# charlesknipp/sequential_monte_carlo

Hardware: AMD Instinct MI355X
Metric: particle-steps/sec (higher is better)
Workload: dtype f64; 1 GPU; LinearGaussian1D bootstrap filter Nx=2^20 T=1000 (BASELINE configs[1]); n_theta_per_gpu=1, n_x=1048576, T=1000, seg=2048, resident_kernel=False, resampler=multinomial

## Files before the change

### include/smc_hip.h

```cpp
#ifndef SMC_HIP_H
#define SMC_HIP_H
#include <stdint.h>

#ifdef __cplusplus
extern "C" {
#endif

#define SMC_MODEL_LG1D 1
#define SMC_MODEL_SV1D 2
#define SMC_MODEL_UCSV3D 3
#define SMC_MODEL_UCSV_RB 4

#define SMC_OK 0
#define SMC_EINVAL (-1)
#define SMC_EHIP (-2)
#define SMC_ESTATE (-3)
#define SMC_ENOMEM (-4)

#define SMC_FLAG_ANCESTORS 1u
#define SMC_FLAG_NO_RESIDENT 2u
#define SMC_FLAG_SYSTEMATIC 4u

typedef struct smc_filter_s* smc_handle;

int smc_create(int model_id, int64_t n_theta, int64_t n_x, int seg, uint64_t seed, int device, uint32_t flags,
               smc_handle* out);
int smc_destroy(smc_handle h);

int smc_set_params(smc_handle h, const double* raw );
int smc_set_streams(smc_handle h, const uint32_t* stream );
int smc_reseed(smc_handle h, uint64_t seed);

#define SMC_PROP_NONE 0
#define SMC_PROP_AFFINE 1
#define SMC_PROP_OPTIMAL 2
#define SMC_PROP_NPAR 4
int smc_set_proposal(smc_handle h, int kind, const double* par );
int smc_host_optimal_proposal(int model_id, const double* raw, double* par );
int smc_host_guided_step(int model_id, const double* raw, int kind, const double* par, const double* xp ,
                         const double* z , double y, double* x , double* logw);
int smc_device_guided_step(int model_id, const double* raw, int kind, const double* par, const double* xp,
                           const double* z, double y, int64_t n, double* x, double* logw, int device);

int smc_host_rb_step(const double* raw , const double* sp , const double* z , double y, int first,
                     double* s , double* logw);
int smc_device_rb_step(const double* raw, const double* sp, const double* z, double y, int first, int64_t n, double* s,
                       double* logw, int device);

int smc_init(smc_handle h, double y1, double* logmu );
int smc_step(smc_handle h, double y_t, double* logmu , double* ess );
int smc_step_window(smc_handle h, const double* y , int k, double* logmu , double* ess );
int smc_step_commit(smc_handle h, int j);
int smc_log_likelihood(smc_handle h, const double* y, int64_t T, double* logZ ,
                       double* logmu_trace, double* ess_trace);
int smc_set_summaries(smc_handle h, int component, const double* p , int np, int moments);
int smc_get_summaries(smc_handle h, int64_t T, double* q , double* mean , double* var );
#define SMC_SUMM_WEIGHTED 0
#define SMC_SUMM_UNWEIGHTED 1
int smc_set_summary_mode(smc_handle h, int mode);
int smc_get_state(smc_handle h, double* x , double* w ,
                  int32_t* anc );
int smc_get_logZ(smc_handle h, double* logZ , double* ess );
int smc_permute(smc_handle h, const int32_t* a );
int smc_copy_from(smc_handle dst, smc_handle src, const uint8_t* mask );

int smc_set_skip(smc_handle h, const uint8_t* skip );

#define SMC_PRIOR_UNIFORM 1
#define SMC_PRIOR_NORMAL 2
#define SMC_PRIOR_TRUNCNORMAL 3
#define SMC_PRIOR_LOGNORMAL 4
#define SMC_PRIOR_NPAR 5
#define SMC_MAX_DTHETA 8
int smc_pmmh_configure(smc_handle prop, int d_theta, const int32_t* prior_family ,
                       const double* prior_par , const int32_t* raw_from ,
                       const double* raw_const );
int smc_pmmh_rejuvenate(smc_handle prop, smc_handle main , const double* y, int64_t T, double xi,
                        const double* chol , const double* scales , int chain,
                        const uint64_t* filter_seeds , uint64_t move_seed, double* theta ,
                        double* logZ , uint8_t* accepted , int64_t* filters_run );
#define SMC_OUTER_SEG 8
int smc_outer_seg(void);
int smc_host_reweight(const double* logw, int64_t n, double* w, double* logmu, double* ess);
int smc_host_outer_records(const double* logw_local, int64_t n_local, uint64_t* rec);
int smc_host_outer_combine(const uint64_t* rec, int64_t nseg, int64_t n_total, double* logmu, double* ess);
int smc_host_outer_window(const double* logw_local, const double* lik , int k, int64_t n_local, uint64_t* rec);
int smc_host_outer_walk(const uint64_t* rec, int k, int64_t nseg, int64_t n_total, double ess_min, double* ess_out , int* j_out);
int smc_host_outer_advance(double* logw, double* logZ, const double* lik , int j, int64_t n);
int smc_host_outer_temper(const double* logZ, int64_t n, double xi, double ess_min, double* xi_new, double* ess, int* resample_flag,
                          double* logw_out);
int smc_host_outer_resample(const double* logw, int64_t n, int64_t m, uint64_t seed, int32_t* a );
int smc_host_rw_factor(const double* theta, int64_t n, int d, double* L , int* univariate);
int smc_host_rw_factor_cov(const double* cov , int d, double* L , int* univariate);
int smc_host_pmmh_propose(int d_theta, uint64_t move_seed, uint32_t stream, uint32_t c, const double* theta,
                          const double* chol, double scale, double* prop);
double smc_host_pmmh_log_uniform(uint64_t move_seed, uint32_t stream, uint32_t c);
double smc_host_prior_logpdf(int family, const double* par , double x);

int smc_slot_bytes(smc_handle h, int64_t* bytes);
int smc_pack_slots(smc_handle h, const int32_t* idx, int64_t k, void* device_buf);
int smc_unpack_slots(smc_handle h, const int32_t* idx, int64_t k, const void* device_buf);

#define SMC_COMM_ID_BYTES 128
typedef struct smc_comm_s* smc_comm;
int smc_comm_unique_id(void* id );
int smc_comm_create(const void* id, int rank, int world, int device, smc_comm* out);
int smc_comm_destroy(smc_comm c);
int smc_comm_rank(smc_comm c, int* rank, int* world);
int smc_comm_all_gather(smc_comm c, const double* local , int64_t n, double* all );
int smc_outer_reweight(smc_comm c, const double* logw_local , int64_t n_local, double* logw_all ,
                       double* w_all , double* logmu, double* ess);
int smc_comm_exchange_slots(smc_comm c, smc_handle h, const int32_t* a , int64_t M);
int smc_comm_plan_exchange(const int32_t* a , int64_t M, int rank, int world, int32_t* send_idx, int64_t* send_cnt ,
                           int64_t* n_send, int32_t* dest_idx, int64_t* recv_cnt );

int smc_get_weights_raw(smc_handle h, uint64_t* C, double* m, uint64_t* S, uint64_t* S2hi, uint64_t* S2lo);
int smc_get_geometry(smc_handle h, int* seg, int* nseg, int* d, int* resident);
int smc_last_elapsed_ms(smc_handle h, double* ms);
int smc_synchronize(smc_handle h);
int smc_time_step_kernel(smc_handle h, const double* y, int64_t T, int nsample, double* avg_ms, double* min_ms);
int smc_event_overhead_ms(smc_handle h, int nsample, double* avg_ms);

int smc_normalize(const double* logw, int64_t n, double* w, double* logmu, double* ess, int device);
int smc_resample(const double* w, int64_t n, int64_t ndraw, uint64_t seed, uint32_t stream, uint32_t t, int32_t* a,
                 int device);

int smc_kalman_log_likelihood(const double* raw, int64_t n_theta, const double* y, int64_t T, int predict_first,
                              double* out , int device);
int smc_ibis_create(int64_t n_theta, uint64_t seed, int device, int predict_first, void* out);
int smc_ibis_destroy(void* h);
int smc_ibis_configure(void* h, int d_theta, const int32_t* prior_family , const double* prior_par ,
                       const int32_t* raw_from , const double* raw_const );
int smc_ibis_set_theta(void* h, const double* theta );
int smc_ibis_window(void* h, const double* y , int k, double* lik , uint64_t* rec );
int smc_ibis_commit(void* h, int j);
int smc_ibis_filter(void* h, const double* y, int64_t T);
int smc_ibis_permute(void* h, const int32_t* a );
int smc_ibis_set_logw(void* h, const double* logw );
int smc_ibis_rejuvenate(void* h, const double* y, int64_t T, double xi, const double* chol ,
                        const double* scales , int chain, uint64_t move_seed, int64_t* accepted ,
                        uint8_t* moved );
int smc_ibis_get(void* h, double* theta, double* x, double* S, double* logZ, double* logw);
int smc_ibis_summary(void* h, int ahead, double* out );
int smc_ibis_set_summaries(void* h, int on, int ahead);
int smc_ibis_get_summaries(void* h, int j, double* out );
int smc_host_ibis_summary(const double* rows, const double* x, const double* S, const double* logw, int64_t M, int ahead, double* out );
int smc_ibis_window_ess(void* h, const double* y , int k, double ess_min, double* ess_out , int* j_out);
int smc_ibis_resample(void* h, uint64_t seed, int32_t* a_out );
int smc_ibis_theta_moments(void* h, int weighted, double* mean , double* cov );
int smc_host_theta_moments(const double* theta, const double* logw, int64_t M, int d, int weighted, double* mean, double* cov);
int smc_ibis_get_moved(void* h, uint8_t* moved );
int smc_get_moments(smc_handle h, double* mean, double* var);

int smc_get_quantiles(smc_handle h, int component, const double* p, int np, double* out);

int smc_simulate(int model_id, const double* raw, int64_t T, uint64_t seed, double* x , double* y );
int smc_simulate_dim(int model_id);
int smc_model_dim(int model_id);
int smc_model_nraw(int model_id);
int smc_auto_seg(int model_id, int64_t n_x);
int smc_device_count(void);
int smc_host_quantile7(const double* x, int64_t n, const double* p, int np, double* out);
int smc_host_sample_moments(const double* x, int64_t n, double* mean, double* var);
double smc_host_exp(double x);
double smc_host_log(double x);
void smc_host_philox4x32_10(const uint32_t ctr[4], const uint32_t key[2], uint32_t out[4]);
void smc_host_box_muller(const uint32_t w[4], double* z0, double* z1);
int smc_sys_targets(uint64_t Dtot, uint32_t n, uint64_t u, uint64_t j0, int nk, uint64_t* out, int device);
int smc_device_math(int which , const double* a, const double* b,
                    int64_t n, double* out, int device);

const char* smc_last_error(void);
const char* smc_version(void);

#ifdef __cplusplus
}
#endif
#endif
```

### sequential_monte_carlo_amd/_lib.py

```python
import ctypes as C
import os

import numpy as np

_HERE = os.path.dirname(os.path.abspath(__file__))
LIB_PATH = os.environ.get("SMC_LIB") or os.path.join(_HERE, "lib", "libsmchip.so")

MODEL_LG1D, MODEL_SV1D, MODEL_UCSV3D, MODEL_UCSV_RB = 1, 2, 3, 4
FLAG_ANCESTORS, FLAG_NO_RESIDENT, FLAG_SYSTEMATIC = 1, 2, 4

EXPORTS = [
    "smc_create", "smc_destroy", "smc_set_params", "smc_set_streams", "smc_reseed", "smc_init", "smc_step",
    "smc_log_likelihood", "smc_get_state", "smc_get_logZ", "smc_permute", "smc_copy_from", "smc_slot_bytes", "smc_pack_slots", "smc_unpack_slots", "smc_get_weights_raw", "smc_get_geometry",
    "smc_last_elapsed_ms", "smc_synchronize", "smc_time_step_kernel", "smc_event_overhead_ms", "smc_normalize", "smc_resample", "smc_kalman_log_likelihood", "smc_get_moments", "smc_get_quantiles", "smc_simulate", "smc_simulate_dim", "smc_model_dim",
    "smc_model_nraw", "smc_auto_seg", "smc_device_count", "smc_host_exp", "smc_host_log", "smc_host_philox4x32_10",
    "smc_host_box_muller", "smc_sys_targets", "smc_device_math", "smc_last_error", "smc_version",
    "smc_set_skip", "smc_pmmh_configure", "smc_pmmh_rejuvenate", "smc_host_pmmh_propose", "smc_host_pmmh_log_uniform",
    "smc_host_prior_logpdf", "smc_step_window", "smc_step_commit",
    "smc_comm_unique_id", "smc_comm_create", "smc_comm_destroy", "smc_comm_rank", "smc_comm_all_gather", "smc_outer_reweight",
    "smc_comm_exchange_slots", "smc_host_reweight", "smc_comm_plan_exchange",
    "smc_outer_seg", "smc_host_outer_records", "smc_host_outer_combine", "smc_host_outer_window", "smc_host_outer_walk",
    "smc_host_outer_advance", "smc_host_outer_temper", "smc_host_outer_resample", "smc_host_rw_factor",
    "smc_set_summaries", "smc_get_summaries", "smc_set_summary_mode", "smc_host_quantile7", "smc_host_sample_moments",
    "smc_set_proposal", "smc_host_optimal_proposal", "smc_host_guided_step", "smc_device_guided_step",
    "smc_host_rb_step", "smc_device_rb_step",
    "smc_ibis_create", "smc_ibis_destroy", "smc_ibis_configure", "smc_ibis_set_theta", "smc_ibis_window", "smc_ibis_commit",
    "smc_ibis_filter", "smc_ibis_permute", "smc_ibis_set_logw", "smc_ibis_rejuvenate", "smc_ibis_get",
    "smc_ibis_summary", "smc_ibis_set_summaries", "smc_ibis_get_summaries", "smc_host_ibis_summary",
    "smc_ibis_window_ess", "smc_ibis_resample", "smc_ibis_theta_moments", "smc_ibis_get_moved", "smc_host_theta_moments",
    "smc_host_rw_factor_cov",
]
PROP_NONE, PROP_AFFINE, PROP_OPTIMAL, PROP_NPAR = 0, 1, 2, 4
SUMM_WEIGHTED, SUMM_UNWEIGHTED = 0, 1
_SUMM_MODES = {"weighted": SUMM_WEIGHTED, "unweighted": SUMM_UNWEIGHTED}
COMM_ID_BYTES = 128
PRIOR_UNIFORM, PRIOR_NORMAL, PRIOR_TRUNCNORMAL, PRIOR_LOGNORMAL, PRIOR_NPAR, MAX_DTHETA = 1, 2, 3, 4, 5, 8

_dp = C.POINTER(C.c_double)
_u64p = C.POINTER(C.c_uint64)
_u32p = C.POINTER(C.c_uint32)
_i32p = C.POINTER(C.c_int32)
_ip = C.POINTER(C.c_int)


class SmcError(RuntimeError):
    pass


_lib = None


def _share_hip_runtime_with_torch():
    if os.environ.get("SMC_HIP_RUNTIME", "") == "system":
        return
    try:
        import importlib.util
        spec = importlib.util.find_spec("torch")
        if spec is None or not spec.submodule_search_locations:
            return
        cand = os.path.join(list(spec.submodule_search_locations)[0], "lib", "libamdhip64.so")
        if os.path.exists(cand):
            C.CDLL(cand, mode=C.RTLD_GLOBAL)
    except Exception:
        pass


def lib():
    global _lib
    if _lib is not None:
        return _lib
    if not os.path.exists(LIB_PATH):
        raise SmcError("HIP extension %s not built: run `python -c 'import __graft_entry__ as g; g.build()'` "
                       "(hipcc --offload-arch=gfx950). There is no CPU fallback." % LIB_PATH)
    _share_hip_runtime_with_torch()
    L = C.CDLL(LIB_PATH)
    h = C.c_void_p
    L.smc_create.argtypes = [C.c_int, C.c_int64, C.c_int64, C.c_int, C.c_uint64, C.c_int, C.c_uint32, C.POINTER(h)]
    L.smc_destroy.argtypes = [h]
    L.smc_set_params.argtypes = [h, _dp]
    L.smc_set_streams.argtypes = [h, _u32p]
    L.smc_reseed.argtypes = [h, C.c_uint64]
    L.smc_init.argtypes = [h, C.c_double, _dp]
    L.smc_step.argtypes = [h, C.c_double, _dp, _dp]
    L.smc_log_likelihood.argtypes = [h, _dp, C.c_int64, _dp, _dp, _dp]
    L.smc_get_state.argtypes = [h, _dp, _dp, _i32p]
    L.smc_get_logZ.argtypes = [h, _dp, _dp]
    L.smc_permute.argtypes = [h, _i32p]
    L.smc_copy_from.argtypes = [h, h, C.POINTER(C.c_uint8)]
    L.smc_slot_bytes.argtypes = [h, C.POINTER(C.c_int64)]
    L.smc_pack_slots.argtypes = [h, _i32p, C.c_int64, C.c_void_p]
    L.smc_unpack_slots.argtypes = [h, _i32p, C.c_int64, C.c_void_p]
    L.smc_get_weights_raw.argtypes = [h, _u64p, _dp, _u64p, _u64p, _u64p]
    L.smc_get_geometry.argtypes = [h, _ip, _ip, _ip, _ip]
    L.smc_last_elapsed_ms.argtypes = [h, _dp]
    L.smc_synchronize.argtypes = [h]
    L.smc_time_step_kernel.argtypes = [h, _dp, C.c_int64, C.c_int, _dp, _dp]
    L.smc_event_overhead_ms.argtypes = [h, C.c_int, _dp]
    L.smc_normalize.argtypes = [_dp, C.c_int64, _dp, _dp, _dp, C.c_int]
    L.smc_resample.argtypes = [_dp, C.c_int64, C.c_int64, C.c_uint64, C.c_uint32, C.c_uint32, _i32p, C.c_int]
    L.smc_kalman_log_likelihood.argtypes = [_dp, C.c_int64, _dp, C.c_int64, C.c_int, _dp, C.c_int]
    L.smc_get_moments.argtypes = [h, _dp, _dp]
    L.smc_get_quantiles.argtypes = [h, C.c_int, _dp, C.c_int, _dp]
    L.smc_set_summaries.argtypes = [h, C.c_int, _dp, C.c_int, C.c_int]
    L.smc_set_summary_mode.argtypes = [h, C.c_int]
    L.smc_host_quantile7.argtypes = [_dp, C.c_int64, _dp, C.c_int, _dp]
    L.smc_host_sample_moments.argtypes = [_dp, C.c_int64, _dp, _dp]
    L.smc_set_proposal.argtypes = [h, C.c_int, _dp]
    L.smc_host_optimal_proposal.argtypes = [C.c_int, _dp, _dp]
    L.smc_host_guided_step.argtypes = [C.c_int, _dp, C.c_int, _dp, _dp, _dp, C.c_double, _dp, _dp]
    L.smc_device_guided_step.argtypes = [C.c_int, _dp, C.c_int, _dp, _dp, _dp, C.c_double, C.c_int64, _dp, _dp, C.c_int]
    L.smc_host_rb_step.argtypes = [_dp, _dp, _dp, C.c_double, C.c_int, _dp, _dp]
    L.smc_device_rb_step.argtypes = [_dp, _dp, _dp, C.c_double, C.c_int, C.c_int64, _dp, _dp, C.c_int]
    L.smc_get_summaries.argtypes = [h, C.c_int64, _dp, _dp, _dp]
    L.smc_sys_targets.argtypes = [C.c_uint64, C.c_uint32, C.c_uint64, C.c_uint64, C.c_int, C.POINTER(C.c_uint64), C.c_int]
    L.smc_simulate.argtypes = [C.c_int, _dp, C.c_int64, C.c_uint64, _dp, _dp]
    L.smc_model_dim.argtypes = [C.c_int]
    L.smc_simulate_dim.argtypes = [C.c_int]
    L.smc_model_nraw.argtypes = [C.c_int]
    L.smc_auto_seg.argtypes = [C.c_int, C.c_int64]
    L.smc_host_exp.restype = C.c_double
    L.smc_host_exp.argtypes = [C.c_double]
    L.smc_host_log.restype = C.c_double
    L.smc_host_log.argtypes = [C.c_double]
    L.smc_host_philox4x32_10.restype = None
    L.smc_host_philox4x32_10.argtypes = [_u32p, _u32p, _u32p]
    L.smc_host_box_muller.restype = None
    L.smc_host_box_muller.argtypes = [_u32p, _dp, _dp]
    L.smc_device_math.argtypes = [C.c_int, _dp, _dp, C.c_int64, _dp, C.c_int]
    L.smc_step_window.argtypes = [h, _dp, C.c_int, _dp, _dp]
    L.smc_step_commit.argtypes = [h, C.c_int]
    L.smc_set_skip.argtypes = [h, C.POINTER(C.c_uint8)]
    L.smc_pmmh_configure.argtypes = [h, C.c_int, _i32p, _dp, _i32p, _dp]
    L.smc_pmmh_rejuvenate.argtypes = [h, h, _dp, C.c_int64, C.c_double, _dp, _dp, C.c_int, _u64p, C.c_uint64, _dp, _dp,
                                      C.POINTER(C.c_uint8), C.POINTER(C.c_int64)]
    L.smc_host_pmmh_propose.argtypes = [C.c_int, C.c_uint64, C.c_uint32, C.c_uint32, _dp, _dp, C.c_double, _dp]
    L.smc_host_pmmh_log_uniform.restype = C.c_double
    L.smc_host_pmmh_log_uniform.argtypes = [C.c_uint64, C.c_uint32, C.c_uint32]
    L.smc_host_prior_logpdf.restype = C.c_double
    L.smc_host_prior_logpdf.argtypes = [C.c_int, _dp, C.c_double]
    L.smc_host_reweight.argtypes = [_dp, C.c_int64, _dp, _dp, _dp]
    L.smc_host_outer_records.argtypes = [_dp, C.c_int64, _u64p]
    L.smc_host_outer_combine.argtypes = [_u64p, C.c_int64, C.c_int64, _dp, _dp]
    L.smc_host_outer_window.argtypes = [_dp, _dp, C.c_int, C.c_int64, _u64p]
    L.smc_host_outer_walk.argtypes = [_u64p, C.c_int, C.c_int64, C.c_int64, C.c_double, _dp, _ip]
    L.smc_host_outer_advance.argtypes = [_dp, _dp, _dp, C.c_int, C.c_int64]
    L.smc_host_outer_temper.argtypes = [_dp, C.c_int64, C.c_double, C.c_double, _dp, _dp, _ip, _dp]
    L.smc_host_outer_resample.argtypes = [_dp, C.c_int64, C.c_int64, C.c_uint64, _i32p]
    L.smc_host_rw_factor.argtypes = [_dp, C.c_int64, C.c_int, _dp, _ip]
    L.smc_comm_unique_id.argtypes = [C.c_void_p]
    L.smc_comm_create.argtypes = [C.c_void_p, C.c_int, C.c_int, C.c_int, C.POINTER(h)]
    L.smc_comm_destroy.argtypes = [h]
    L.smc_comm_rank.argtypes = [h, _ip, _ip]
    L.smc_comm_all_gather.argtypes = [h, _dp, C.c_int64, _dp]
    L.smc_outer_reweight.argtypes = [h, _dp, C.c_int64, _dp, _dp, _dp, _dp]
    L.smc_comm_exchange_slots.argtypes = [h, h, _i32p, C.c_int64]
    L.smc_comm_plan_exchange.argtypes = [_i32p, C.c_int64, C.c_int, C.c_int, _i32p, C.POINTER(C.c_int64), C.POINTER(C.c_int64), _i32p,
                                         C.POINTER(C.c_int64)]
    L.smc_ibis_create.argtypes = [C.c_int64, C.c_uint64, C.c_int, C.c_int, C.POINTER(h)]
    L.smc_ibis_destroy.argtypes = [h]
    L.smc_ibis_configure.argtypes = [h, C.c_int, _i32p, _dp, _i32p, _dp]
    L.smc_ibis_set_theta.argtypes = [h, _dp]
    L.smc_ibis_window.argtypes = [h, _dp, C.c_int, _dp, _u64p]
    L.smc_ibis_commit.argtypes = [h, C.c_int]
    L.smc_ibis_filter.argtypes = [h, _dp, C.c_int64]
    L.smc_ibis_permute.argtypes = [h, _i32p]
    L.smc_ibis_set_logw.argtypes = [h, _dp]
    L.smc_ibis_rejuvenate.argtypes = [h, _dp, C.c_int64, C.c_double, _dp, _dp, C.c_int, C.c_uint64, C.POINTER(C.c_int64),
                                      C.POINTER(C.c_uint8)]
    L.smc_ibis_get.argtypes = [h, _dp, _dp, _dp, _dp, _dp]
    L.smc_ibis_summary.argtypes = [h, C.c_int, _dp]
    L.smc_ibis_set_summaries.argtypes = [h, C.c_int, C.c_int]
    L.smc_ibis_get_summaries.argtypes = [h, C.c_int, _dp]
    L.smc_host_ibis_summary.argtypes = [_dp, _dp, _dp, _dp, C.c_int64, C.c_int, _dp]
    L.smc_ibis_window_ess.argtypes = [h, _dp, C.c_int, C.c_double, _dp, _ip]
    L.smc_ibis_resample.argtypes = [h, C.c_uint64, _i32p]
    L.smc_ibis_theta_moments.argtypes = [h, C.c_int, _dp, _dp]
    L.smc_ibis_get_moved.argtypes = [h, C.POINTER(C.c_uint8)]
    L.smc_host_theta_moments.argtypes = [_dp, _dp, C.c_int64, C.c_int, C.c_int, _dp, _dp]
    L.smc_host_rw_factor_cov.argtypes = [_dp, C.c_int, _dp, _ip]
    L.smc_last_error.restype = C.c_char_p
    L.smc_version.restype = C.c_char_p
    _lib = L
    return L


def check(rc):
    if rc != 0:
        raise SmcError("libsmchip error %d: %s" % (rc, lib().smc_last_error().decode()))


def _d(a):
    return a.ctypes.data_as(_dp) if a is not None else None


def device_count():
    return lib().smc_device_count()


def sys_targets(Dtot, n, u, j0, nk, device=-1):
    out = np.zeros(nk, dtype=np.uint64)
    check(lib().smc_sys_targets(int(Dtot), int(n), int(u), int(j0), int(nk), out.ctypes.data_as(C.POINTER(C.c_uint64)), device))
    return out


def simulate(model_id, raw, T, seed):
    raw = np.ascontiguousarray(raw, dtype=np.float64)
    d = lib().smc_simulate_dim(model_id)
    x = np.zeros((d, T))
    y = np.zeros(T)
    check(lib().smc_simulate(model_id, _d(raw), T, seed, _d(x), _d(y)))
    return x, y


def normalize(logw, device=0):
    logw = np.ascontiguousarray(logw, dtype=np.float64)
    w = np.zeros_like(logw)
    lm, ess = C.c_double(), C.c_double()
    check(lib().smc_normalize(_d(logw), logw.size, _d(w), C.byref(lm), C.byref(ess), device))
    return lm.value, w, ess.value


def resample(w, ndraw=None, seed=0, stream=0, t=0, device=0):
    w = np.ascontiguousarray(w, dtype=np.float64)
    ndraw = w.size if ndraw is None else int(ndraw)
    a = np.zeros(ndraw, dtype=np.int32)
    check(lib().smc_resample(_d(w), w.size, ndraw, seed, stream, t, a.ctypes.data_as(_i32p), device))
    return a


def kalman_log_likelihood(raw, y, predict_first=False, device=0):
    raw = np.ascontiguousarray(raw, dtype=np.float64).reshape(-1, 6)
    y = np.ascontiguousarray(y, dtype=np.float64)
    out = np.zeros((raw.shape[0], 3))
    check(lib().smc_kalman_log_likelihood(_d(raw), raw.shape[0], _d(y), y.size, int(predict_first), _d(out), device))
# ... 124 lines not shown
    k, nseg = rec.shape[0], rec.shape[1]
    ess = np.zeros(k)
    j = C.c_int()
    check(lib().smc_host_outer_walk(rec.ctypes.data_as(_u64p), k, nseg, int(n_total), float(ess_min), _d(ess), C.byref(j)))
    return ess[:j.value], j.value


def host_outer_advance(logw, logZ, lik, j):
    lik = np.ascontiguousarray(lik, dtype=np.float64)
    logw = np.array(logw, dtype=np.float64, order="C")
    logZ = np.array(logZ, dtype=np.float64, order="C")
    assert lik.shape[1] == logw.size == logZ.size and 0 <= j <= lik.shape[0]
    check(lib().smc_host_outer_advance(_d(logw), _d(logZ), _d(lik), int(j), logw.size))
    return logw, logZ


def host_outer_temper(logZ, xi, ess_min):
    logZ = np.ascontiguousarray(logZ, dtype=np.float64)
    lw = np.empty_like(logZ)
    nx, e, flag = C.c_double(), C.c_double(), C.c_int()
    check(lib().smc_host_outer_temper(_d(logZ), logZ.size, float(xi), float(ess_min), C.byref(nx), C.byref(e), C.byref(flag), _d(lw)))
    return nx.value, e.value, bool(flag.value), lw


def host_outer_resample(logw, m, seed):
    logw = np.ascontiguousarray(logw, dtype=np.float64)
    a = np.empty(int(m), dtype=np.int32)
    check(lib().smc_host_outer_resample(_d(logw), logw.size, int(m), int(seed), a.ctypes.data_as(_i32p)))
    return a


def host_rw_factor(theta):
    theta = np.ascontiguousarray(theta, dtype=np.float64)
    n, d = theta.shape
    L = np.zeros((d, d))
    uni = C.c_int()
    check(lib().smc_host_rw_factor(_d(theta), n, d, _d(L), C.byref(uni)))
    return L, bool(uni.value)


def host_rw_factor_cov(cov):
    cov = np.ascontiguousarray(cov, dtype=np.float64)
    d = cov.shape[0]
    assert cov.shape == (d, d)
    L = np.zeros((d, d))
    uni = C.c_int()
    check(lib().smc_host_rw_factor_cov(_d(cov), d, _d(L), C.byref(uni)))
    return L, bool(uni.value)


def host_theta_moments(theta, logw=None, weighted=False):
    theta = np.ascontiguousarray(theta, dtype=np.float64)
    M, d = theta.shape
    if weighted:
        logw = np.ascontiguousarray(logw, dtype=np.float64)
        assert logw.size == M
    mean, cov = np.zeros(d), np.zeros((d, d))
    check(lib().smc_host_theta_moments(_d(theta), _d(logw) if weighted else None, M, d, int(bool(weighted)), _d(mean), _d(cov)))
    return mean, cov


def comm_unique_id():
    buf = C.create_string_buffer(COMM_ID_BYTES)
    check(lib().smc_comm_unique_id(buf))
    return buf.raw


class Comm:

    def __init__(self, unique_id, rank, world, device=0):
        self._c = C.c_void_p()
        self.rank, self.world = int(rank), int(world)
        check(lib().smc_comm_create(C.c_char_p(bytes(unique_id)), self.rank, self.world, int(device), C.byref(self._c)))

    def close(self):
        if getattr(self, "_c", None):
            lib().smc_comm_destroy(self._c)
            self._c = None

    def slice(self, M):
        if M % self.world:
            raise ValueError("n_theta (%d) must be a multiple of the number of ranks (%d)" % (M, self.world))
        per = M // self.world
        return self.rank * per, (self.rank + 1) * per

    def all_gather(self, local):
        local = np.ascontiguousarray(local, dtype=np.float64).ravel()
        out = np.zeros(local.size * self.world)
        check(lib().smc_comm_all_gather(self._c, _d(local), local.size, _d(out)))
        return out

    def outer_reweight(self, logw_local, want_w=True):
        lw = np.ascontiguousarray(logw_local, dtype=np.float64).ravel()
        allw, w = (np.zeros(lw.size * self.world), np.zeros(lw.size * self.world)) if want_w else (None, None)
        lm, ess = C.c_double(), C.c_double()
        check(lib().smc_outer_reweight(self._c, _d(lw), lw.size, _d(allw), _d(w), C.byref(lm), C.byref(ess)))
        return lm.value, w, ess.value, allw

    def exchange_slots(self, h, a, M):
        a = np.ascontiguousarray(a, dtype=np.int32)
        check(lib().smc_comm_exchange_slots(self._c, h._h, a.ctypes.data_as(_i32p), int(M)))


class Handle:

    def __init__(self, model_id, n_theta, n_x, seg=0, seed=1, device=0, flags=0):
        self._h = C.c_void_p()
        self.summary_mode = "weighted"
        self.model_id, self.n_theta, self.n_x = model_id, int(n_theta), int(n_x)
        check(lib().smc_create(model_id, self.n_theta, self.n_x, seg, seed, device, flags, C.byref(self._h)))
        seg_, nseg, d, res = C.c_int(), C.c_int(), C.c_int(), C.c_int()
        check(lib().smc_get_geometry(self._h, C.byref(seg_), C.byref(nseg), C.byref(d), C.byref(res)))
        self.seg, self.nseg, self.d, self.resident = seg_.value, nseg.value, d.value, bool(res.value)
        self.flags = flags

    def close(self):
        if getattr(self, "_h", None):
            lib().smc_destroy(self._h)
            self._h = None

    def __del__(self):
        try:
            self.close()
        except Exception:
            pass

    def set_params(self, raw):
        raw = np.ascontiguousarray(raw, dtype=np.float64).reshape(self.n_theta, -1)
        assert raw.shape[1] == lib().smc_model_nraw(self.model_id)
        check(lib().smc_set_params(self._h, _d(raw)))

    def set_proposal(self, kind, par=None):
        if par is not None:
            par = np.ascontiguousarray(par, dtype=np.float64)
            if par.size == PROP_NPAR and self.n_theta > 1:
                par = np.tile(par.reshape(1, PROP_NPAR), (self.n_theta, 1))
            if par.size != self.n_theta * PROP_NPAR:
                raise ValueError("proposal rows must be [n_theta][4]")
            par = np.ascontiguousarray(par)
        check(lib().smc_set_proposal(self._h, int(kind), _d(par)))
        self.proposal_kind = int(kind)

    def set_streams(self, streams):
        s = np.ascontiguousarray(streams, dtype=np.uint32)
        assert s.size == self.n_theta
        if getattr(self, "_streams_set", None) is not None and np.array_equal(self._streams_set, s):
            return
        check(lib().smc_set_streams(self._h, s.ctypes.data_as(_u32p)))
        self._streams_set = s.copy()

    def reseed(self, seed):
        check(lib().smc_reseed(self._h, seed))

    def init(self, y1):
        lm = np.zeros(self.n_theta)
        check(lib().smc_init(self._h, float(y1), _d(lm)))
        return lm

    def step(self, y):
        lm = np.zeros(self.n_theta)
        ess = np.zeros(self.n_theta)
        check(lib().smc_step(self._h, float(y), _d(lm), _d(ess)))
        return lm, ess

    def step_window(self, y):
        y = np.ascontiguousarray(y, dtype=np.float64)
        lm = np.zeros((y.size, self.n_theta))
        ess = np.zeros((y.size, self.n_theta))
        check(lib().smc_step_window(self._h, _d(y), y.size, _d(lm), _d(ess)))
        return lm, ess

    def step_commit(self, j):
        check(lib().smc_step_commit(self._h, int(j)))

    @property
    def can_window(self):
        return self.nseg == 1 and self.resident

    def log_likelihood(self, y, trace=False):
        y = np.ascontiguousarray(y, dtype=np.float64)
        logZ = np.zeros(self.n_theta)
        if trace:
            lm = np.zeros((y.size, self.n_theta))
            es = np.zeros((y.size, self.n_theta))
            check(lib().smc_log_likelihood(self._h, _d(y), y.size, _d(logZ), _d(lm), _d(es)))
            return logZ, lm, es
        check(lib().smc_log_likelihood(self._h, _d(y), y.size, _d(logZ), None, None))
        return logZ

    def state(self, want_w=True, want_anc=None):
        x = np.zeros((self.d, self.n_theta, self.n_x))
        w = np.zeros((self.n_theta, self.n_x)) if want_w else None
        if want_anc is None:
            want_anc = bool(self.flags & FLAG_ANCESTORS)
        a = np.zeros((self.n_theta, self.n_x), dtype=np.int32) if want_anc else None
        check(lib().smc_get_state(self._h, _d(x), _d(w), a.ctypes.data_as(_i32p) if a is not None else None))
        return x, w, a

    def logZ(self):
        z = np.zeros(self.n_theta)
        e = np.zeros(self.n_theta)
        check(lib().smc_get_logZ(self._h, _d(z), _d(e)))
        return z, e

    def permute(self, a):
        a = np.ascontiguousarray(a, dtype=np.int32)
        assert a.size == self.n_theta
        check(lib().smc_permute(self._h, a.ctypes.data_as(_i32p)))

    def set_summary_mode(self, mode):
        if mode not in _SUMM_MODES:
            raise ValueError("summary mode must be 'weighted' or 'unweighted'")
        check(lib().smc_set_summary_mode(self._h, _SUMM_MODES[mode]))
        self.summary_mode = mode

    def moments(self):
        m = np.zeros((self.d, self.n_theta))
        v = np.zeros((self.d, self.n_theta))
        check(lib().smc_get_moments(self._h, _d(m), _d(v)))
        return m, v

    def quantiles(self, p, component=0):
        p = np.ascontiguousarray(p, dtype=np.float64).ravel()
        out = np.zeros((self.n_theta, p.size))
        check(lib().smc_get_quantiles(self._h, int(component), _d(p), p.size, _d(out)))
        return out

    def set_summaries(self, p=None, component=0, moments=False):
        p = np.ascontiguousarray([] if p is None else p, dtype=np.float64).ravel()
        check(lib().smc_set_summaries(self._h, int(component), _d(p) if p.size else None, p.size, int(bool(moments))))
        self._sum_np, self._sum_mom = int(p.size), bool(moments)

    def get_summaries(self, T):
        nq, mom = getattr(self, "_sum_np", 0), getattr(self, "_sum_mom", False)
        q = np.zeros((T, self.n_theta, nq)) if nq else None
        mean = np.zeros((T, self.d, self.n_theta)) if mom else None
        var = np.zeros((T, self.d, self.n_theta)) if mom else None
        check(lib().smc_get_summaries(self._h, int(T), _d(q), _d(mean), _d(var)))
        return q, mean, var

    def copy_from(self, src, mask):
        m = np.ascontiguousarray(mask, dtype=np.uint8)
        assert m.size == self.n_theta
        check(lib().smc_copy_from(self._h, src._h, m.ctypes.data_as(C.POINTER(C.c_uint8))))

    def set_skip(self, skip):
        if skip is None:
            check(lib().smc_set_skip(self._h, None))
            return
        m = np.ascontiguousarray(skip, dtype=np.uint8)
        assert m.size == self.n_theta
        check(lib().smc_set_skip(self._h, m.ctypes.data_as(C.POINTER(C.c_uint8))))

    def pmmh_configure(self, families, pars, raw_from, raw_const):
        fam = np.ascontiguousarray(families, dtype=np.int32)
        par = np.ascontiguousarray(pars, dtype=np.float64).reshape(fam.size, PRIOR_NPAR)
        rf = np.ascontiguousarray(raw_from, dtype=np.int32)
        rc = np.ascontiguousarray(raw_const, dtype=np.float64)
        assert rf.size == rc.size == lib().smc_model_nraw(self.model_id)
        check(lib().smc_pmmh_configure(self._h, fam.size, fam.ctypes.data_as(_i32p), _d(par), rf.ctypes.data_as(_i32p), _d(rc)))
        self._pmmh_d = int(fam.size)

    def pmmh_rejuvenate(self, main, y, xi, chol, scales, filter_seeds, move_seed, theta, logZ):
        y = np.ascontiguousarray(y, dtype=np.float64)
        d = self._pmmh_d
        theta = np.array(theta, dtype=np.float64, order="C").reshape(self.n_theta, d)
        logZ = np.array(logZ, dtype=np.float64, order="C").reshape(self.n_theta)
        chol = np.ascontiguousarray(chol, dtype=np.float64).reshape(d, d)
        scales = np.ascontiguousarray(scales, dtype=np.float64)
        seeds = np.ascontiguousarray(filter_seeds, dtype=np.uint64)
        assert seeds.size == scales.size
        acc = np.zeros(self.n_theta, dtype=np.uint8)
        nrun = C.c_int64()
        check(lib().smc_pmmh_rejuvenate(self._h, main._h if main is not None else None, _d(y), y.size, float(xi), _d(chol),
                                        _d(scales), scales.size, seeds.ctypes.data_as(_u64p), int(move_seed), _d(theta), _d(logZ),
                                        acc.ctypes.data_as(C.POINTER(C.c_uint8)), C.byref(nrun)))
        return theta, logZ, acc.astype(bool), int(nrun.value)

    def slot_bytes(self):
        b = C.c_int64()
        check(lib().smc_slot_bytes(self._h, C.byref(b)))
        return b.value

    def pack_slots(self, idx, device_ptr):
        idx = np.ascontiguousarray(idx, dtype=np.int32)
        check(lib().smc_pack_slots(self._h, idx.ctypes.data_as(_i32p), idx.size, C.c_void_p(int(device_ptr))))

    def unpack_slots(self, idx, device_ptr):
        idx = np.ascontiguousarray(idx, dtype=np.int32)
        check(lib().smc_unpack_slots(self._h, idx.ctypes.data_as(_i32p), idx.size, C.c_void_p(int(device_ptr))))

    def weights_raw(self):
        npad = self.nseg * self.seg
        Cc = np.zeros((self.n_theta, npad), dtype=np.uint64)
        m = np.zeros((self.n_theta, self.nseg))
        S = np.zeros((self.n_theta, self.nseg), dtype=np.uint64)
        hi = np.zeros_like(S)
        lo = np.zeros_like(S)
        check(lib().smc_get_weights_raw(self._h, Cc.ctypes.data_as(_u64p), _d(m), S.ctypes.data_as(_u64p),
                                        hi.ctypes.data_as(_u64p), lo.ctypes.data_as(_u64p)))
        return Cc, m, S, hi, lo

    def elapsed_ms(self):
        ms = C.c_double()
        check(lib().smc_last_elapsed_ms(self._h, C.byref(ms)))
        return ms.value
# ... 133 lines not shown
```

### sequential_monte_carlo_amd/csrc/smc_capi.hip

```cpp
#include "smc_host.h"
#include "smc_aux_kernels.h"

#include <atomic>
#include <chrono>
#include <cstdlib>
#include <cstring>
#include <mutex>
#include <string>
#include <vector>
#ifdef SMC_ABLATE
#include <algorithm>
#include <cstdio>
#include <map>
#endif

using namespace smc;

static thread_local std::string g_err;
#ifdef SMC_ABLATE
static int h_abl_tmp = 0;
static void abl_report(smc_filter_s* h);
#endif
int fail(int code, const std::string& msg) {
    g_err = msg;
    return code;
}

namespace smc {
bool geo_valid(int seg, int np, Geo& g) {
    if (np != 1 && np != 2 && np != 4) return false;
    const int th = seg / (2 * np);
    if (th * 2 * np != seg) return false;
    if (!(th == 128 || th == 256 || th == 512 || th == 1024 || (th == 64 && np == 2))) return false;
    g = {th, np};
    return true;
}
bool geo_default(int seg, Geo& g) {
    switch (seg) {
    case 256: g = {128, 1}; return true;
    case 512: g = {256, 1}; return true;
    case 1024: g = {512, 1}; return true;
    case 2048: g = {512, 2}; return true;
    case 4096: g = {1024, 2}; return true;
    case 8192: g = {1024, 4}; return true;
    }
    return false;
}
}

constexpr int MAX_NSEG = 16384;
extern "C" int smc_auto_seg(int model_id, int64_t n) {
    const int dm = model_dim_rt(model_id);
    const bool d3 = dm >= 3;
    if (n > (int64_t)MAX_NSEG * 4096) return 8192;
    if (n > (int64_t)MAX_NSEG * 2048) return 4096;
    if (n > (int64_t)MAX_NSEG * 1024) return 2048;
    if (n > ((int64_t)1 << 19)) return d3 ? 1024 : 2048;
    if (n > ((int64_t)1 << 17)) return 1024;
    if (n > ((int64_t)1 << 15)) return 512;
    if (n > (dm > 3 ? 2048 : d3 ? 4096 : MAX_SEG)) return 256;
    int s = 256;
    while (s < n) s <<= 1;
    return s;
}
extern "C" int smc_model_dim(int id) { return model_dim_rt(id); }
extern "C" int smc_model_nraw(int id) { return model_nraw_rt(id); }
extern "C" const char* smc_last_error(void) { return g_err.c_str(); }
extern "C" const char* smc_version(void) { return "smchip 0.1 (gfx950)"; }
extern "C" int smc_device_count(void) {
    int n = 0;
    if (hipGetDeviceCount(&n) != hipSuccess) return 0;
    return n;
}

hipError_t do_init(smc_filter_s* h, double y) {
    return by_model(h->model, [&](auto M) { return launch_init<decltype(M)::value>(h->v, h->geo, h->cur, y, h->stream); });
}
static hipError_t do_table(smc_filter_s* h, int emit, int first_emit, uint32_t t_emit) {
    constexpr int TH = 1024;
    hipLaunchKernelGGL((k_table<TH>), dim3(h->v.ntheta), dim3(TH), 0, h->stream, h->v, h->cur, emit, first_emit, t_emit);
    return hipGetLastError();
}
hipError_t do_step(smc_filter_s* h, uint32_t t, int emit_prev, double y) {
    if (h->v.tabD) {
        hipError_t e = do_table(h, emit_prev, t == 1u ? 1 : 0, t - 1u);
        if (e != hipSuccess) return e;
        emit_prev = 0;
    }
    if (h->v.prop_kind)
        return by_guided_model(h->model, [&](auto M) { return launch_step_g<decltype(M)::value>(h->v, h->geo, h->cur, t, emit_prev, y, h->stream); });
    return by_model(h->model, [&](auto M) { return launch_step<decltype(M)::value>(h->v, h->geo, h->cur, t, emit_prev, y, h->stream); });
}
hipError_t ensure_breaks(smc_filter_s* h, uint32_t t, uint32_t t_end) {
    FilterView& v = h->v;
    if (v.nseg <= 1 || v.systematic) return hipSuccess;
    if (h->brk_count && t >= v.brk_t0 && t < v.brk_t0 + h->brk_count) return hipSuccess;
    const size_t per_step = (size_t)v.ntheta * ((size_t)v.nseg + 1);
    if (!h->d_brk) {
        size_t steps = ((size_t)32 << 20) / (per_step * 8);
        steps = steps < 1 ? 1 : (steps > 1024 ? 1024 : steps);
        hipError_t e = hipMalloc((void**)&h->d_brk, steps * per_step * 8);
        if (e != hipSuccess) return e;
        h->brk_cap = (uint32_t)steps;
        v.brk = h->d_brk;
    }
    uint32_t cnt = t_end > t ? t_end - t : 1;
    cnt = cnt > h->brk_cap ? h->brk_cap : cnt;
    constexpr int TH = 256;
    const size_t lds = ((size_t)v.nseg + 1 + TH / WAVE) * 8;
    static bool raised[16] = {};
    hipError_t e = raise_lds_limit(k_breaks<TH>, lds, raised);
    if (e != hipSuccess) return e;
    hipLaunchKernelGGL((k_breaks<TH>), dim3(cnt, v.ntheta), dim3(TH), lds, h->stream, v, t, h->d_brk);
    v.brk_t0 = t;
    h->brk_count = cnt;
    return hipGetLastError();
}
static hipError_t do_window(smc_filter_s* h, int k, int bout) {
    if (h->v.prop_kind)
        return by_guided_model(h->model, [&](auto M) {
            return launch_window_g<decltype(M)::value>(h->v, k, h->d_recs, (int)h->t, h->cur, bout, h->win.h_out, h->stream);
        });
    return by_model(h->model, [&](auto M) {
        return launch_window<decltype(M)::value>(h->v, k, h->d_recs, (int)h->t, h->cur, bout, h->win.h_out, h->stream);
    });
}

hipError_t do_finalize(smc_filter_s* h, int first_emit, uint32_t t_emit) {
    if (h->v.tabD) return do_table(h, 1, first_emit, t_emit);
    constexpr int TH = 256;
    const size_t lds = table_lds_bytes(h->v.nseg_p2, TH, 1);
    hipLaunchKernelGGL((k_finalize<TH>), dim3(h->v.ntheta), dim3(TH), lds, h->stream, h->v, h->cur, first_emit, t_emit);
    return hipGetLastError();
}

namespace {
struct Bundle {
    int device = -1;
    char* slab = nullptr; size_t slab_bytes = 0;
    double* pin = nullptr; size_t pin_bytes = 0;
    hipStream_t stream = nullptr;
    hipEvent_t ev0 = nullptr, ev1 = nullptr;
    double* d_y = nullptr; int64_t ycap = 0;
    void* d_recs = nullptr; size_t rec_bytes = 0;
    void* h_params = nullptr; size_t params_bytes = 0;
};
struct BundleCache {
    std::mutex mu;
    std::vector<Bundle> free_list;
    size_t bytes = 0;
    static constexpr size_t MAX_BYTES = (size_t)512 << 20, MAX_COUNT = 8;
    bool take(int device, size_t slab_bytes, size_t pin_bytes, Bundle& out) {
        std::lock_guard<std::mutex> g(mu);
        for (size_t i = 0; i < free_list.size(); ++i) {
            const Bundle& b = free_list[i];
            if (b.device == device && b.slab_bytes >= slab_bytes && b.slab_bytes <= 2 * slab_bytes + 4096 && b.pin_bytes >= pin_bytes) {
                out = b;
                bytes -= b.slab_bytes;
                free_list.erase(free_list.begin() + (long)i);
                return true;
            }
        }
        return false;
    }
    bool give(const Bundle& b) {
        std::lock_guard<std::mutex> g(mu);
        if (free_list.size() >= MAX_COUNT || bytes + b.slab_bytes > MAX_BYTES) return false;
        free_list.push_back(b);
        bytes += b.slab_bytes;
        return true;
    }
};
BundleCache& bundle_cache() { static BundleCache* c = new BundleCache(); return *c; }
}

extern "C" int smc_create(int model_id, int64_t n_theta, int64_t n_x, int seg, uint64_t seed, int device, uint32_t flags,
                          smc_handle* out) {
    if (!out) return fail(SMC_EINVAL, "smc_create: out is NULL");
    *out = nullptr;
    const int d = model_dim_rt(model_id);
    if (d < 0) return fail(SMC_EINVAL, "smc_create: unknown model_id " + std::to_string(model_id));
    if (n_theta <= 0 || n_x <= 0) return fail(SMC_EINVAL, "smc_create: n_theta and n_x must be positive");
    if (n_theta > 65535) return fail(SMC_EINVAL, "smc_create: n_theta > 65535 (grid.y limit); shard theta");
    if (seg == 0) seg = smc_auto_seg(model_id, n_x);
    Geo g;
    if (!geo_default(seg, g)) return fail(SMC_EINVAL, "smc_create: seg must be a power of two in [256,8192]");
#ifdef SMC_ABLATE
    if (const char* e = getenv("SMC_ABL")) h_abl_tmp = atoi(e);
#endif
    if (const char* e = getenv("SMC_NP")) {
        Geo g2;
        if (geo_valid(seg, atoi(e), g2)) g = g2;
    }
    const int64_t nseg = (n_x + seg - 1) / seg;
    if (nseg > MAX_NSEG) return fail(SMC_EINVAL, "smc_create: more than 16384 segments; use a larger seg");
    if (n_x > ((int64_t)1 << 31)) return fail(SMC_EINVAL, "smc_create: n_x > 2^31");
    int ndev = 0;
    HIPCHK(hipGetDeviceCount(&ndev));
    if (ndev == 0) return fail(SMC_EHIP, "smc_create: no HIP device; this library has no CPU fallback");
    if (device < 0 || device >= ndev) return fail(SMC_EINVAL, "smc_create: bad device index");
    HIPCHK(hipSetDevice(device));

    smc_filter_s* h = new smc_filter_s();
    h->model = model_id; h->d = d; h->device = device; h->flags = flags;
    h->geo = g;
    FilterView& v = h->v;
    v.n = n_x; v.seg = seg; v.nseg = (int)nseg; v.npad = nseg * seg; v.ntheta = (int)n_theta; v.seed = seed;
    int p2 = 1;
    while (p2 < v.nseg) p2 <<= 1;
    v.nseg_p2 = p2;
    v.SH = table_shift_extra(v.npad);
    v.want_s2 = 1;
#ifdef SMC_ABLATE
    v.abl = h_abl_tmp;
    if (getenv("SMC_DBG")) {
        if (hipMalloc((void**)&v.dbg, (size_t)v.ntheta * v.nseg * 128) != hipSuccess) v.dbg = nullptr;
        else (void)hipMemset(v.dbg, 0, (size_t)v.ntheta * v.nseg * 128);
    }
#endif
    h->resident_ok = (v.nseg == 1) && !(flags & SMC_FLAG_NO_RESIDENT);
    v.systematic = (flags & SMC_FLAG_SYSTEMATIC) ? 1 : 0;
    v.inv_n = 1.0 / (double)n_x;

    const size_t np = (size_t)v.ntheta * (size_t)v.npad, ns = (size_t)v.ntheta * (size_t)v.nseg, nt = (size_t)v.ntheta;
#define TRY(expr)                                       \
    do {                                                \
        hipError_t _e = (expr);                         \
        if (_e != hipSuccess) {                         \
            std::string m = hipGetErrorString(_e);      \
            smc_destroy(h);                             \
            return fail(SMC_ENOMEM, "smc_create: " #expr ": " + m); \
        }                                               \
    } while (0)
    Bundle bun;
    {
        const bool gtab = v.nseg_p2 > 2 * g.threads;
        size_t off = 0;
        auto take = [&](size_t bytes) { const size_t o = off; off += (bytes + 255) & ~(size_t)255; return o; };
        const size_t o_params = take(nt * sizeof(*h->d_params)), o_stream = take(nt * sizeof(*h->d_stream)), o_perm = take(nt * sizeof(*h->d_perm)),
                     o_ztmp = take(nt * 8);
        size_t o_x[2], o_C[2], o_k[2], o_S[2], o_hi[2], o_lo[2];
        for (int b = 0; b < 2; ++b) {
            o_x[b] = take(np * (size_t)d * 8); o_C[b] = take(np * 8);
            o_k[b] = take(ns * 8); o_S[b] = take(ns * 8); o_hi[b] = take(ns * 8); o_lo[b] = take(ns * 8);
        }
        const size_t o_anc = (flags & SMC_FLAG_ANCESTORS) ? take(np * 4) : 0;
        const size_t o_logZ = take(nt * 8), o_lm = take(nt * 8), o_es = take(nt * 8), o_K = take(nt * 8), o_D = take(nt * 8);
        const size_t o_tD = gtab ? take(nt * (size_t)v.nseg_p2 * 8) : 0, o_tsh = gtab ? take(nt * (size_t)v.nseg_p2 * 4) : 0;
        h->slab_bytes = off;
        if (bundle_cache().take(device, off, 4 * nt * 8, bun)) {
            h->d_slab = bun.slab; h->slab_bytes = bun.slab_bytes; h->stream = bun.stream; h->ev0 = bun.ev0; h->ev1 = bun.ev1;
            h->h_pin = bun.pin; h->pin_bytes = bun.pin_bytes;
            h->d_y = bun.d_y; h->ycap = bun.ycap;
            h->d_recs = (decltype(h->d_recs))bun.d_recs; h->reccap = (int64_t)(bun.rec_bytes / (nt * sizeof(*h->d_recs)));
            if (bun.params_bytes >= nt * sizeof(Params)) h->h_params = (Params*)bun.h_params;
            else if (bun.h_params) (void)hipHostFree(bun.h_params);
        } else {
            TRY(hipStreamCreateWithFlags(&h->stream, hipStreamNonBlocking));
            TRY(hipEventCreate(&h->ev0));
            TRY(hipEventCreate(&h->ev1));
            TRY(hipMalloc((void**)&h->d_slab, off));
        }
        TRY(hipMemsetAsync(h->d_slab, 0, off, h->stream));
        char* base = h->d_slab;
        h->d_params = (decltype(h->d_params))(base + o_params); h->d_stream = (decltype(h->d_stream))(base + o_stream);
        h->d_perm = (decltype(h->d_perm))(base + o_perm); h->d_logZ_tmp = (double*)(base + o_ztmp);
        for (int b = 0; b < 2; ++b) {
            v.x[b] = (double*)(base + o_x[b]); v.C[b] = (uint64_t*)(base + o_C[b]);
            v.segk[b] = (double*)(base + o_k[b]); v.segS[b] = (uint64_t*)(base + o_S[b]);
            v.segS2hi[b] = (uint64_t*)(base + o_hi[b]); v.segS2lo[b] = (uint64_t*)(base + o_lo[b]);
        }
        if (flags & SMC_FLAG_ANCESTORS) v.anc = (decltype(v.anc))(base + o_anc);
        v.logZ = (double*)(base + o_logZ); v.last_logmu = (double*)(base + o_lm); v.last_ess = (double*)(base + o_es);
        v.last_K = (double*)(base + o_K); v.last_D = (uint64_t*)(base + o_D);
        if (gtab) { v.tabD = (uint64_t*)(base + o_tD); v.tabsh = (int*)(base + o_tsh); }
    }
    if (!h->h_pin) {
        TRY(hipHostMalloc((void**)&h->h_pin, 4 * nt * 8, hipHostMallocDefault));
        h->pin_bytes = 4 * nt * 8;
    }
    memset(h->h_pin, 0, 4 * nt * 8);
    v.host_out = h->h_pin;
    std::vector<uint32_t> st(nt);
    for (size_t m = 0; m < nt; ++m) st[m] = (uint32_t)m;
    TRY(hipMemcpyAsync(h->d_stream, st.data(), nt * 4, hipMemcpyHostToDevice, h->stream));
    TRY(hipStreamSynchronize(h->stream));
#undef TRY
    v.params = h->d_params;
    v.stream = h->d_stream;
    *out = h;
    return SMC_OK;
}

extern "C" int smc_destroy(smc_handle h) {
    if (!h) return SMC_OK;
    (void)hipSetDevice(h->device);
    if (h->stream) (void)hipStreamSynchronize(h->stream);
#ifdef SMC_ABLATE
    abl_report(h);
#endif
    Bundle bun;
    bun.device = h->device; bun.slab = h->d_slab; bun.slab_bytes = h->slab_bytes; bun.pin = h->h_pin; bun.pin_bytes = h->pin_bytes;
    bun.stream = h->stream; bun.ev0 = h->ev0; bun.ev1 = h->ev1;
    bun.d_y = h->d_y; bun.ycap = h->ycap; bun.d_recs = h->d_recs; bun.rec_bytes = (size_t)h->reccap * (size_t)h->v.ntheta * sizeof(*h->d_recs);
    bun.h_params = h->h_params; bun.params_bytes = h->h_params ? (size_t)h->v.ntheta * sizeof(Params) : 0;
    const bool kept = h->d_slab && h->h_pin && h->stream && h->ev0 && h->ev1 && bundle_cache().give(bun);
    if (!kept) {
        (void)hipFree(h->d_slab);
        if (h->h_pin) (void)hipHostFree(h->h_pin);
    }
    if (h->pm.h_out) (void)hipHostFree(h->pm.h_out);
    if (h->pm.h_in) (void)hipHostFree(h->pm.h_in);
    if (h->h_perm) (void)hipHostFree(h->h_perm);
    if (h->h_params && !kept) (void)hipHostFree(h->h_params);
    if (h->d_prop) (void)hipFree(h->d_prop);
    if (h->h_prop) (void)hipHostFree(h->h_prop);
    (void)hipFree(h->skip.d_mask); (void)hipFree(h->skip.d_order);
    if (h->win.h_out) (void)hipHostFree(h->win.h_out);
    if (h->summ.h_once) (void)hipHostFree(h->summ.h_once);
    (void)hipFree(h->pm.dev.order);
    (void)hipFree(h->pm.d_in);
    (void)hipFree(h->pm.dev.prop); (void)hipFree(h->pm.dev.lp); (void)hipFree(h->pm.dev.skip); (void)hipFree(h->pm.dev.mask);
    if (h->d_brk) (void)hipFree(h->d_brk);
    if (h->summ.d_ms) (void)hipFree(h->summ.d_ms);
    if (!kept) (void)hipFree(h->d_y);
    (void)hipFree(h->d_tr_logmu); (void)hipFree(h->d_tr_ess); (void)hipFree(h->d_wdense); if (!kept) (void)hipFree(h->d_recs);
    (void)hipFree(h->summ.d_q); (void)hipFree(h->summ.d_m); (void)hipFree(h->persist.d_flags);
    if (h->persist.h_err) (void)hipHostFree(h->persist.h_err);
    if (!kept) {
        if (h->ev0) (void)hipEventDestroy(h->ev0);
        if (h->ev1) (void)hipEventDestroy(h->ev1);
        if (h->stream) (void)hipStreamDestroy(h->stream);
    }
    delete h;
    return SMC_OK;
}

static void fill_proposal(smc_handle h, int m) {
    const Params& P = h->h_params[m];
    double* q = h->h_prop[m].p;
    for (int k = 0; k < NPARAM; ++k) q[k] = 0.0;
    if (h->v.prop_kind == PROP_AFFINE)
        for (int k = 0; k < PROP_NPAR; ++k) q[k] = h->prop_par[(size_t)m * PROP_NPAR + k];
    derive_proposal(h->model, h->v.prop_kind, P.raw, P.der, q);
}

extern "C" int smc_set_params(smc_handle h, const double* raw) {
    if (!h || !raw) return fail(SMC_EINVAL, "smc_set_params: NULL argument");
    HIPCHK(hipSetDevice(h->device));
    const int nraw = model_nraw_rt(h->model);
    if (!h->h_params) HIPCHK(hipHostMalloc((void**)&h->h_params, (size_t)h->v.ntheta * sizeof(Params), hipHostMallocDefault));
    else HIPCHK(hipStreamSynchronize(h->stream));
    Params* P = h->h_params;
    for (int m = 0; m < h->v.ntheta; ++m) {
        for (int k = 0; k < NPARAM; ++k) P[m].raw[k] = k < nraw ? raw[(size_t)m * nraw + k] : 0.0;
        derive_params(h->model, P[m].raw, P[m].der);
        if (h->v.prop_kind) fill_proposal(h, m);
    }
    HIPCHK(hipMemcpyAsync(h->d_params, P, (size_t)h->v.ntheta * sizeof(Params), hipMemcpyHostToDevice, h->stream));
    if (h->v.prop_kind)
        HIPCHK(hipMemcpyAsync(h->d_prop, h->h_prop, (size_t)h->v.ntheta * sizeof(PropRow), hipMemcpyHostToDevice, h->stream));
    h->have_params = true;
    return SMC_OK;
}

extern "C" int smc_set_proposal(smc_handle h, int kind, const double* par) {
    if (!h) return fail(SMC_EINVAL, "smc_set_proposal: NULL handle");
    if (kind != PROP_NONE && kind != PROP_AFFINE && kind != PROP_OPTIMAL) return fail(SMC_EINVAL, "smc_set_proposal: unknown kind");
    if (h->model == MODEL_UCSV_RB && kind != PROP_NONE)
        return fail(SMC_EINVAL, "smc_set_proposal: SMC_MODEL_UCSV_RB takes no proposal (its step already conditions on y: the trend is integrated out)");
    if (!proposal_supported(h->model, kind)) return fail(SMC_EINVAL, "smc_set_proposal: this model family has no proposal of that kind");
    if ((kind == PROP_AFFINE) != (par != nullptr)) return fail(SMC_EINVAL, "smc_set_proposal: rows are given with SMC_PROP_AFFINE and only then");
    if (kind == PROP_AFFINE)
        for (int m = 0; m < h->v.ntheta; ++m)
            if (!affine_row_ok(par + (size_t)m * PROP_NPAR)) return fail(SMC_EINVAL, "smc_set_proposal: rows must be finite with s2 > 0");
    HIPCHK(hipSetDevice(h->device));
    HIPCHK(hipStreamSynchronize(h->stream));
    const size_t nt = (size_t)h->v.ntheta;
    if (kind != PROP_NONE && !h->d_prop) {
        HIPCHK(hipMalloc((void**)&h->d_prop, nt * sizeof(PropRow)));
        HIPCHK(hipHostMalloc((void**)&h->h_prop, nt * sizeof(PropRow), hipHostMallocDefault));
    }
    if (kind == PROP_AFFINE) h->prop_par.assign(par, par + nt * PROP_NPAR);
    else h->prop_par.clear();
    h->v.prop_kind = kind;
    h->v.prop = kind != PROP_NONE ? h->d_prop : nullptr;
    h->win.k = 0;
    if (kind == PROP_NONE) return SMC_OK;
    if (!h->h_params) {
        HIPCHK(hipHostMalloc((void**)&h->h_params, nt * sizeof(Params), hipHostMallocDefault));
        memset(h->h_params, 0, nt * sizeof(Params));
    }
    if (h->have_params) HIPCHK(hipMemcpy(h->h_params, h->d_params, nt * sizeof(Params), hipMemcpyDeviceToHost));
    for (int m = 0; m < h->v.ntheta; ++m) fill_proposal(h, m);
    HIPCHK(hipMemcpyAsync(h->d_prop, h->h_prop, nt * sizeof(PropRow), hipMemcpyHostToDevice, h->stream));
    return SMC_OK;
}

extern "C" int smc_set_streams(smc_handle h, const uint32_t* s) {
    if (!h || !s) return fail(SMC_EINVAL, "smc_set_streams: NULL argument");
    HIPCHK(hipSetDevice(h->device));
    HIPCHK(hipMemcpyAsync(h->d_stream, s, (size_t)h->v.ntheta * 4, hipMemcpyHostToDevice, h->stream));
    HIPCHK(hipStreamSynchronize(h->stream));
    h->brk_count = 0;
    return SMC_OK;
}

extern "C" int smc_reseed(smc_handle h, uint64_t seed) {
    if (!h) return fail(SMC_EINVAL, "smc_reseed: NULL handle");
    h->v.seed = seed;
    h->brk_count = 0;
    return SMC_OK;
}

int ensure_y(smc_handle h, int64_t T) {
    if (T > h->ycap) {
        HIPCHK(hipStreamSynchronize(h->stream));
        (void)hipFree(h->d_y);
        h->d_y = nullptr;
        HIPCHK(dalloc(&h->d_y, (size_t)T));
        h->ycap = T;
    }
    return SMC_OK;
}

int ensure_recs(smc_handle h, int64_t T) {
    if (T > h->reccap) {
        HIPCHK(hipStreamSynchronize(h->stream));
        (void)hipFree(h->d_recs);
        h->d_recs = nullptr;
        HIPCHK(dalloc(&h->d_recs, (size_t)T * h->v.ntheta));
        h->reccap = T;
    }
    return SMC_OK;
}

int finish_elapsed(smc_handle h, double* logZ, double* logmu, double* ess) {
    const size_t nt = (size_t)h->v.ntheta;
    HIPCHK(hipEventRecord(h->ev1, h->stream));
    HIPCHK(hipStreamSynchronize(h->stream));
    float ms = 0.f;
    HIPCHK(hipEventElapsedTime(&ms, h->ev0, h->ev1));
    h->last_ms = ms;
    if (logZ) memcpy(logZ, h->h_pin, nt * 8);
    if (logmu) memcpy(logmu, h->h_pin + nt, nt * 8);
    if (ess) memcpy(ess, h->h_pin + 2 * nt, nt * 8);
    return SMC_OK;
}

static int wait_ticket(smc_handle h, uint32_t seq, double* logmu, double* ess) {
    const size_t nt = (size_t)h->v.ntheta;
    const volatile double* tk = h->h_pin + 3 * nt;
    const double want = (double)seq;
    const auto t0 = std::chrono::steady_clock::now();
    bool synced = false;
    unsigned spins = 0;
    for (size_t th = 0; th < nt;) {
        if (tk[th] == want) { ++th; continue; }
        if ((++spins & 0x3ffu) == 0 && std::chrono::steady_clock::now() - t0 > std::chrono::milliseconds(50)) {
            if (synced) return fail(SMC_EHIP, "step API: the launch completed without its result ticket");
            HIPCHK(hipStreamSynchronize(h->stream));
            synced = true;
        }
        __builtin_ia32_pause();
    }
    std::atomic_thread_fence(std::memory_order_acquire);
    if (logmu) memcpy(logmu, h->h_pin + nt, nt * 8);
    if (ess) memcpy(ess, h->h_pin + 2 * nt, nt * 8);
    h->last_ms = std::chrono::duration<float, std::milli>(std::chrono::steady_clock::now() - t0).count();
    return SMC_OK;
}

static uint32_t step_ticket(smc_handle h) {
    if (h->v.ntheta > 64) return 0;
    return ++h->seq ? h->seq : ++h->seq;
}
int emit_if_needed(smc_handle h) {
    if (!h->emitted) {
        HIPCHK(do_finalize(h, h->t == 1 ? 1 : 0, h->t - 1));
        h->emitted = true;
    }
    return SMC_OK;
}

extern "C" int smc_init(smc_handle h, double y1, double* logmu) {
    if (!h) return fail(SMC_EINVAL, "smc_init: NULL handle");
    if (!h->have_params) return fail(SMC_ESTATE, "smc_init: smc_set_params has not been called");
    h->win.k = 0;
    HIPCHK(hipSetDevice(h->device));
    h->v.y = nullptr; h->v.trace_logmu = nullptr; h->v.trace_ess = nullptr;
    h->cur = 0;
    const bool own = h->v.nseg == 1;
    const uint32_t seq = step_ticket(h);
    if (!seq) HIPCHK(hipEventRecord(h->ev0, h->stream));
    h->v.emit_now = own ? 1 : 0;
    h->v.host_seq = seq;
    hipError_t le = do_init(h, y1);
    h->v.emit_now = 0;
    if (le == hipSuccess) { h->t = 1; h->inited = true; h->emitted = own; }
    const int rc = le == hipSuccess ? emit_if_needed(h) : SMC_OK;
    h->v.host_seq = 0;
    HIPCHK(le);
    if (rc) return rc;
    return seq ? wait_ticket(h, seq, logmu, nullptr) : finish_elapsed(h, nullptr, logmu, nullptr);
}

extern "C" int smc_step(smc_handle h, double y_t, double* logmu, double* ess) {
    if (!h) return fail(SMC_EINVAL, "smc_step: NULL handle");
    if (!h->inited) return fail(SMC_ESTATE, "smc_step: call smc_init (bootstrap_filter) first");
    h->win.k = 0;
    HIPCHK(hipSetDevice(h->device));
    h->v.y = nullptr; h->v.trace_logmu = nullptr; h->v.trace_ess = nullptr;
    int rc = emit_if_needed(h);
    if (rc) return rc;
    HIPCHK(ensure_breaks(h, h->t, h->t + 64));
    const bool own = h->v.nseg == 1;
    const uint32_t seq = step_ticket(h);
    if (!seq) HIPCHK(hipEventRecord(h->ev0, h->stream));
    h->v.emit_now = own ? 1 : 0;
    h->v.host_seq = seq;
    hipError_t le = do_step(h, h->t, 0, y_t);
    h->v.emit_now = 0;
    if (le == hipSuccess) { h->cur ^= 1; h->t += 1; h->emitted = own; rc = emit_if_needed(h); }
    h->v.host_seq = 0;
    HIPCHK(le);
    if (rc) return rc;
    return seq ? wait_ticket(h, seq, logmu, ess) : finish_elapsed(h, nullptr, logmu, ess);
}

constexpr int WIN_MAX = 64;
static int launch_window_steps(smc_handle h, int k) {
    HIPCHK(hipEventRecord(h->ev0, h->stream));
    HIPCHK(do_window(h, k, h->cur ^ 1));
    return SMC_OK;
}
extern "C" int smc_step_window(smc_handle h, const double* y, int k, double* logmu, double* ess) {
    if (!h || !y) return fail(SMC_EINVAL, "smc_step_window: NULL argument");
    if (!h->inited) return fail(SMC_ESTATE, "smc_step_window: call smc_init (bootstrap_filter) first");
    if (k < 1 || k > WIN_MAX) return fail(SMC_EINVAL, "smc_step_window: 1 <= k <= 64");
    if (h->v.nseg != 1 || !resident_supported(h->model, h->v.seg))
        return fail(SMC_EINVAL, "smc_step_window: needs filters that fit the LDS-resident kernel (one segment); use smc_step");
    HIPCHK(hipSetDevice(h->device));
    int rc = emit_if_needed(h);
    if (rc) return rc;
    if ((rc = ensure_y(h, WIN_MAX))) return rc;
    if ((rc = ensure_recs(h, WIN_MAX))) return rc;
    const size_t nt = (size_t)h->v.ntheta;
    if (!h->win.h_out) HIPCHK(hipHostMalloc((void**)&h->win.h_out, 2 * (size_t)WIN_MAX * nt * 8, hipHostMallocDefault));
    const bool summ = summaries_on(h);
    if (summ && h->v.systematic) return fail(SMC_EINVAL, "smc_step_window: per-step summaries need the default (multinomial) resampler");
    if (summ && !summaries_fit_lds(h)) return fail(SMC_EINVAL, "smc_step_window: no LDS left for the summaries of filters this long; fewer levels, or smc_step");
    if (summ && (rc = ensure_summaries(h, WIN_MAX))) return rc;
    h->summ.T = 0;
    h->summ.skip.clear();
    HIPCHK(hipMemcpyAsync(h->d_y, y, (size_t)k * 8, hipMemcpyHostToDevice, h->stream));
    h->v.y = h->d_y;
    if (summ) view_summaries(h);
    rc = launch_window_steps(h, k);
    h->v.y = nullptr;
    h->v.sum_np = h->v.sum_mom = 0; h->v.sum_q = h->v.sum_m = nullptr;
    if (rc) return rc;
    if (summ) h->summ.T = k;
    if ((rc = finish_elapsed(h))) return rc;
    if (logmu) memcpy(logmu, h->win.h_out, (size_t)k * nt * 8);
    if (ess) memcpy(ess, h->win.h_out + (size_t)k * nt, (size_t)k * nt * 8);
    h->win.k = k;
    return SMC_OK;
}
extern "C" int smc_step_commit(smc_handle h, int j) {
    if (!h) return fail(SMC_EINVAL, "smc_step_commit: NULL handle");
    if (h->win.k == 0) return fail(SMC_ESTATE, "smc_step_commit: no window pending (smc_step_window)");
    if (j < 0 || j > h->win.k) return fail(SMC_EINVAL, "smc_step_commit: 0 <= j <= steps of the window");
    HIPCHK(hipSetDevice(h->device));
    const int k = h->win.k;
    h->win.k = 0;
    if (j == 0) return SMC_OK;
    if (j < k) {
        h->v.y = h->d_y;
        int rc = launch_window_steps(h, j);
        h->v.y = nullptr;
        if (rc) return rc;
    }
    hipLaunchKernelGGL(k_commit, dim3((unsigned)((h->v.ntheta + 127) / 128)), dim3(128), 0, h->stream, h->v, j, h->d_recs);
    HIPCHK(hipGetLastError());
    h->cur ^= 1; h->t += (uint32_t)j; h->emitted = true;
    return SMC_OK;
}

extern "C" int smc_set_skip(smc_handle h, const uint8_t* skip) {
    if (!h) return fail(SMC_EINVAL, "smc_set_skip: NULL handle");
    HIPCHK(hipSetDevice(h->device));
    if (!skip) { h->skip.on = false; h->skip.h_mask.clear(); return SMC_OK; }
    const int nt = h->v.ntheta;
    if (!h->skip.d_mask) HIPCHK(dalloc(&h->skip.d_mask, (size_t)nt));
    if (!h->skip.d_order) HIPCHK(dalloc(&h->skip.d_order, (size_t)nt + 1));
    std::vector<int32_t> ord((size_t)nt + 1);
    int na = 0, ns = 0;
    for (int m = 0; m < nt; ++m) {
        if (skip[m]) ord[(size_t)nt - 1 - ns++] = m;
        else ord[(size_t)na++] = m;
    }
    ord[(size_t)nt] = na;
    HIPCHK(hipMemcpyAsync(h->skip.d_mask, skip, (size_t)nt, hipMemcpyHostToDevice, h->stream));
    HIPCHK(hipMemcpyAsync(h->skip.d_order, ord.data(), ord.size() * 4, hipMemcpyHostToDevice, h->stream));
    HIPCHK(hipStreamSynchronize(h->stream));
    h->skip.h_mask.assign(skip, skip + nt);
    h->skip.on = true;
    return SMC_OK;
}

extern "C" int smc_get_logZ(smc_handle h, double* logZ, double* ess) {
    if (!h) return fail(SMC_EINVAL, "smc_get_logZ: NULL handle");
    if (!h->inited) return fail(SMC_ESTATE, "smc_get_logZ: filter not initialised");
    HIPCHK(hipSetDevice(h->device));
    int rc = emit_if_needed(h);
    if (rc) return rc;
    HIPCHK(hipStreamSynchronize(h->stream));
    if (logZ) HIPCHK(hipMemcpy(logZ, h->v.logZ, (size_t)h->v.ntheta * 8, hipMemcpyDeviceToHost));
    if (ess) HIPCHK(hipMemcpy(ess, h->v.last_ess, (size_t)h->v.ntheta * 8, hipMemcpyDeviceToHost));
    return SMC_OK;
}

extern "C" int smc_get_geometry(smc_handle h, int* seg, int* nseg, int* d, int* resident) {
    if (!h) return fail(SMC_EINVAL, "smc_get_geometry: NULL handle");
    if (seg) *seg = h->v.seg;
    if (nseg) *nseg = h->v.nseg;
    if (d) *d = h->d;
    if (resident) *resident = (h->resident_ok && resident_supported(h->model, h->v.seg)) ? 1 : 0;
    return SMC_OK;
}

extern "C" int smc_last_elapsed_ms(smc_handle h, double* ms) {
    if (!h || !ms) return fail(SMC_EINVAL, "smc_last_elapsed_ms: NULL argument");
    *ms = h->last_ms;
    return SMC_OK;
}

extern "C" int smc_synchronize(smc_handle h) {
    if (!h) return fail(SMC_EINVAL, "smc_synchronize: NULL handle");
    HIPCHK(hipSetDevice(h->device));
    HIPCHK(hipStreamSynchronize(h->stream));
    return SMC_OK;
}

#ifdef SMC_ABLATE
static void abl_report(smc_filter_s* h) {
    if (h->v.dbg && h->v.nseg == 1) {
        const size_t nwg = (size_t)h->v.ntheta;
        std::vector<unsigned long long> st(nwg * 8);
        (void)hipMemcpy(st.data(), h->v.dbg, nwg * 64, hipMemcpyDeviceToHost);
        unsigned long long t0 = ~0ull, t1 = 0;
        std::map<unsigned long long, std::vector<size_t>> bycu;
        size_t nact = 0;
        for (size_t w = 0; w < nwg; ++w) {
            if (!st[w * 8 + 1]) continue;
            ++nact;
            if (st[w * 8] < t0) t0 = st[w * 8];
            if (st[w * 8 + 1] > t1) t1 = st[w * 8 + 1];
            const unsigned long long hw = st[w * 8 + 2];
            const unsigned long long key = ((hw >> 32) & 0xf) << 16 | ((hw >> 8) & 0xff);
            bycu[key].push_back(w);
        }
        int hist[9] = {0};
        double life[9] = {0};
        for (auto& kv : bycu) {
            const size_t c = kv.second.size() < 8 ? kv.second.size() : 8;
            hist[c]++;
            for (size_t w : kv.second) life[c] += (double)(st[w * 8 + 1] - st[w * 8]) * 0.01;
        }
        fprintf(stderr, "[dbg] k_resident: %zu workgroups ran on %zu CUs, span %.1f us;", nact, bycu.size(), (double)(t1 - t0) * 0.01);
        for (int c = 1; c <= 8; ++c)
            if (hist[c]) fprintf(stderr, "  %d CUs with %d workgroups (mean life %.1f us)", hist[c], c, life[c] / (hist[c] * c));
        fprintf(stderr, "\n");
        {
            int shown = 0;
            for (auto& kv : bycu) {
                if (shown++ >= 4) break;
                fprintf(stderr, "[dbg]   cu %05llx:", kv.first);
                for (size_t w : kv.second) fprintf(stderr, " wg %zu [%.1f, %.1f]", w, (double)(st[w * 8] - t0) * 0.01, (double)(st[w * 8 + 1] - t0) * 0.01);
                fprintf(stderr, "\n");
            }
        }
        (void)hipFree(h->v.dbg);
        h->v.dbg = nullptr;
    }
    if (h->v.dbg) {
        const size_t nwg = (size_t)h->v.ntheta * h->v.nseg;
        std::vector<unsigned long long> st(nwg * 8);
        (void)hipMemcpy(st.data(), h->v.dbg + nwg * 8, nwg * 64, hipMemcpyDeviceToHost);
        if (st[7] == 0x5045525349535421ull) {
            double wait = 0, body = 0, pub = 0, mx_wait = 0;
            for (size_t w = 0; w < nwg; ++w) {
                const double steps = (double)st[w * 8];
                wait += st[w * 8 + 1] * 0.01 / steps; body += st[w * 8 + 2] * 0.01 / steps; pub += st[w * 8 + 3] * 0.01 / steps;
                mx_wait = std::max(mx_wait, st[w * 8 + 1] * 0.01 / steps);
            }
            fprintf(stderr, "[dbg] k_persist, mean over %zu workgroups, us per step: wait (poll + acquire + barrier) %.2f (max %.2f), step body %.2f, "
                            "drain + barrier + publish %.2f\n", nwg, wait / nwg, mx_wait, body / nwg, pub / nwg);
        }
    }
    if (h->v.dbg) {
        const size_t nwg = (size_t)h->v.ntheta * h->v.nseg;
        std::vector<unsigned long long> st(nwg * 8);
        (void)hipMemcpy(st.data(), h->v.dbg, nwg * 64, hipMemcpyDeviceToHost);
        unsigned long long t0 = ~0ull, t7 = 0;
        double ph[8] = {0};
        for (size_t w = 0; w < nwg; ++w) {
            if (st[w * 8] < t0) t0 = st[w * 8];
            if (st[w * 8 + 7] > t7) t7 = st[w * 8 + 7];
            for (int k = 1; k < 8; ++k) ph[k] += (double)(st[w * 8 + k] - st[w * 8 + k - 1]) * 0.01;
        }
        double start_spread = 0, life = 0;
        for (size_t w = 0; w < nwg; ++w) { start_spread += (double)(st[w * 8] - t0) * 0.01; life += (double)(st[w * 8 + 7] - st[w * 8]) * 0.01; }
        fprintf(stderr, "[dbg] k_step span %.2f us; mean start offset %.2f us; mean WG life %.2f us; phases(us):", (double)(t7 - t0) * 0.01,
                start_spread / nwg, life / nwg);
        const char* nm[8] = {"", "table+picks", "targets+range+lookup", "normals", "T2+stage-write+barrier", "search", "gather+model+store", "epilogue"};
        for (int k = 1; k < 8; ++k) fprintf(stderr, " %s=%.2f", nm[k], ph[k] / nwg);
        fprintf(stderr, "\n");
        {
            std::vector<size_t> idx(nwg);
            for (size_t w = 0; w < nwg; ++w) idx[w] = w;
            std::sort(idx.begin(), idx.end(), [&](size_t a, size_t b) { return st[a * 8 + 7] > st[b * 8 + 7]; });
            for (size_t r = 0; r < 6 && r < nwg; ++r) {
                const size_t w = idx[r];
                fprintf(stderr, "[dbg]   late #%zu wg %zu xcd %zu: start %.2f end %.2f phases", r, w, w % 8, (double)(st[w * 8] - t0) * 0.01,
                        (double)(st[w * 8 + 7] - t0) * 0.01);
                for (int k = 1; k < 8; ++k) fprintf(stderr, " %.2f", (double)(st[w * 8 + k] - st[w * 8 + k - 1]) * 0.01);
                fprintf(stderr, "\n");
            }
            double endq[5];
            std::vector<double> ends(nwg);
            for (size_t w = 0; w < nwg; ++w) ends[w] = (double)(st[w * 8 + 7] - t0) * 0.01;
            std::sort(ends.begin(), ends.end());
            const double qs[5] = {0.1, 0.5, 0.9, 0.99, 1.0};
            for (int k = 0; k < 5; ++k) endq[k] = ends[(size_t)((nwg - 1) * qs[k])];
            fprintf(stderr, "[dbg]   end-time quantiles (us) 10%%=%.2f 50%%=%.2f 90%%=%.2f 99%%=%.2f max=%.2f\n", endq[0], endq[1], endq[2], endq[3], endq[4]);
        }
        (void)hipFree(h->v.dbg);
    }
}
#endif
```

### sequential_monte_carlo_amd/csrc/smc_capi_pmmh.hip

```cpp
#include "smc_host.h"
#include "smc_pmmh_kernels.h"

#include <cmath>
#include <cstring>

using namespace smc;

extern "C" int smc_pmmh_configure(smc_handle h, int d_theta, const int32_t* prior_family, const double* prior_par,
                                  const int32_t* raw_from, const double* raw_const) {
    if (!h || !prior_family || !prior_par || !raw_from || !raw_const) return fail(SMC_EINVAL, "smc_pmmh_configure: NULL argument");
    if (d_theta < 1 || d_theta > MAX_DTHETA) return fail(SMC_EINVAL, "smc_pmmh_configure: 1 <= d_theta <= 8");
    PmmhSpec sp{};
    sp.d = d_theta;
    for (int i = 0; i < d_theta; ++i) {
        if (prior_family[i] < PRIOR_UNIFORM || prior_family[i] > PRIOR_LOGNORMAL)
            return fail(SMC_EINVAL, "smc_pmmh_configure: unknown prior family " + std::to_string(prior_family[i]));
        sp.family[i] = prior_family[i];
        for (int k = 0; k < PRIOR_NPAR; ++k) sp.par[i][k] = prior_par[(size_t)i * PRIOR_NPAR + k];
    }
    sp.nraw = model_nraw_rt(h->model);
    for (int k = 0; k < sp.nraw; ++k) {
        if (raw_from[k] >= d_theta) return fail(SMC_EINVAL, "smc_pmmh_configure: raw_from index out of range");
        sp.raw_from[k] = raw_from[k];
        sp.raw_const[k] = raw_const[k];
    }
    HIPCHK(hipSetDevice(h->device));
    const size_t nt = (size_t)h->v.ntheta;
    if (!h->pm.d_in) {
        const size_t w_theta = nt * MAX_DTHETA, w_chol = (size_t)MAX_DTHETA * MAX_DTHETA, w_any = (nt + 7) / 8;
        h->pm.in_words = w_theta + nt + w_chol + 2 + w_any;
        HIPCHK(dalloc(&h->pm.d_in, h->pm.in_words));
        HIPCHK(hipHostMalloc((void**)&h->pm.h_in, h->pm.in_words * 8, hipHostMallocDefault));
        h->pm.dev.theta = h->pm.d_in;
        h->pm.dev.logZ = h->pm.dev.theta + w_theta;
        h->pm.dev.chol = h->pm.dev.logZ + nt;
        h->pm.dev.nrun = (unsigned long long*)(h->pm.dev.chol + w_chol);
        h->pm.dev.counts = (int32_t*)(h->pm.dev.nrun + 1);
        h->pm.dev.any = (unsigned char*)(h->pm.dev.nrun + 2);
        HIPCHK(dalloc(&h->pm.dev.prop, nt * MAX_DTHETA));
        HIPCHK(dalloc(&h->pm.dev.lp, nt * 2));
        HIPCHK(dalloc(&h->pm.dev.skip, nt));
        HIPCHK(dalloc(&h->pm.dev.mask, nt));
        HIPCHK(dalloc(&h->pm.dev.order, nt));
        HIPCHK(hipHostMalloc((void**)&h->pm.h_out, (nt * (MAX_DTHETA + 2) + 1) * 8, hipHostMallocDefault));
    }
    h->pm.spec = sp;
    h->pm.cfg = true;
    return SMC_OK;
}

__global__ void k_pmmh_export(int ntheta, int d, PmmhDev p, double* out) {
    const int m = blockIdx.x * blockDim.x + threadIdx.x;
    if (m >= ntheta) return;
    for (int i = 0; i < d; ++i) out[(size_t)m * d + i] = p.theta[(size_t)m * MAX_DTHETA + i];
    out[(size_t)ntheta * d + m] = p.logZ[m];
    out[(size_t)ntheta * (d + 1) + m] = p.any[m] ? 1.0 : 0.0;
    if (m == 0) out[(size_t)ntheta * (d + 2)] = (double)*p.nrun;
}

extern "C" int smc_pmmh_rejuvenate(smc_handle h, smc_handle main, const double* y, int64_t T, double xi, const double* chol,
                                   const double* scales, int chain, const uint64_t* filter_seeds, uint64_t move_seed,
                                   double* theta, double* logZ, uint8_t* accepted, int64_t* filters_run) {
    if (!h || !y || !chol || !scales || !filter_seeds || !theta || !logZ) return fail(SMC_EINVAL, "smc_pmmh_rejuvenate: NULL argument");
    if (!h->pm.cfg) return fail(SMC_ESTATE, "smc_pmmh_rejuvenate: smc_pmmh_configure has not been called");
    if (T <= 0 || chain < 0) return fail(SMC_EINVAL, "smc_pmmh_rejuvenate: bad T or chain");
    if (main) {
        if (main == h) return fail(SMC_EINVAL, "smc_pmmh_rejuvenate: main and proposal handles are the same");
        const FilterView &a = main->v, &b = h->v;
        if (main->model != h->model || a.n != b.n || a.seg != b.seg || a.ntheta != b.ntheta || main->device != h->device)
            return fail(SMC_EINVAL, "smc_pmmh_rejuvenate: handles differ in model, geometry or device");
        if (!main->inited) return fail(SMC_ESTATE, "smc_pmmh_rejuvenate: main filters not initialised");
        main->win.k = 0;
    }
    h->win.k = 0;
    HIPCHK(hipSetDevice(h->device));
    const PmmhSpec& sp = h->pm.spec;
    const int nt = h->v.ntheta, d = sp.d;
    int rc = ensure_y(h, T);
    if (rc) return rc;
    const bool resident = h->resident_ok && resident_supported(h->model, h->v.seg);
    if (resident && (rc = ensure_recs(h, T))) return rc;
    if (main) {
        if ((rc = emit_if_needed(main))) return rc;
        HIPCHK(hipStreamSynchronize(main->stream));
    }
    {
        double* in = h->pm.h_in;
        memset(in, 0, h->pm.in_words * 8);
        for (int m = 0; m < nt; ++m)
            for (int i = 0; i < d; ++i) in[(size_t)m * MAX_DTHETA + i] = theta[(size_t)m * d + i];
        double* in_logZ = in + (size_t)nt * MAX_DTHETA;
        memcpy(in_logZ, logZ, (size_t)nt * 8);
        double* in_chol = in_logZ + nt;
        for (int i = 0; i < d * d; ++i) in_chol[i] = chol[i];
    }
    HIPCHK(hipEventRecord(h->ev0, h->stream));
    HIPCHK(hipMemcpyAsync(h->d_y, y, (size_t)T * 8, hipMemcpyHostToDevice, h->stream));
    HIPCHK(hipMemcpyAsync(h->pm.d_in, h->pm.h_in, h->pm.in_words * 8, hipMemcpyHostToDevice, h->stream));
    const dim3 grid((unsigned)((nt + 127) / 128)), block(128);
    for (int c = 0; c < chain; ++c) {
        hipLaunchKernelGGL(k_pmmh_propose, grid, block, 0, h->stream, h->v, sp, h->pm.dev, h->model, move_seed, (uint32_t)c,
                           sqrt(scales[c]), h->d_params);
        HIPCHK(hipGetLastError());
        h->have_params = true;
        h->v.seed = filter_seeds[c];
        h->brk_count = 0;
        h->v.skip = h->pm.dev.skip; h->v.order = h->pm.dev.order; h->v.n_active = h->pm.dev.counts;
        rc = enqueue_log_likelihood(h, y[0], T, false);
        h->v.skip = nullptr; h->v.order = nullptr; h->v.n_active = nullptr;
        if (rc) return rc;
        hipLaunchKernelGGL(k_pmmh_accept, grid, block, 0, h->stream, h->v, h->pm.dev, d, move_seed, (uint32_t)c, xi);
        HIPCHK(hipGetLastError());
        if (main) HIPCHK(copy_slots(main->v, main->cur, h->v, h->cur, main->d, h->pm.dev.mask, h->stream));
    }
    hipLaunchKernelGGL(k_pmmh_export, grid, block, 0, h->stream, nt, d, h->pm.dev, h->pm.h_out);
    HIPCHK(hipGetLastError());
    if ((rc = finish_elapsed(h))) return rc;
    if (main && chain > 0) main->t = h->t;
    memcpy(theta, h->pm.h_out, (size_t)nt * d * 8);
    memcpy(logZ, h->pm.h_out + (size_t)nt * d, (size_t)nt * 8);
    if (accepted)
        for (int m = 0; m < nt; ++m) accepted[m] = h->pm.h_out[(size_t)nt * (d + 1) + m] != 0.0 ? 1 : 0;
    if (filters_run) *filters_run = (int64_t)h->pm.h_out[(size_t)nt * (d + 2)];
    return SMC_OK;
}
```

### sequential_monte_carlo_amd/csrc/smc_capi_series.hip

```cpp
#include "smc_host.h"

#include <cstdlib>
#include <cstring>
#include <limits>
#include <vector>

using namespace smc;

static int ensure_trace(smc_handle h, int64_t T) {
    if (T > h->trcap) {
        HIPCHK(hipStreamSynchronize(h->stream));
        (void)hipFree(h->d_tr_logmu); (void)hipFree(h->d_tr_ess);
        h->d_tr_logmu = h->d_tr_ess = nullptr;
        HIPCHK(dalloc(&h->d_tr_logmu, (size_t)T * h->v.ntheta));
        HIPCHK(dalloc(&h->d_tr_ess, (size_t)T * h->v.ntheta));
        h->trcap = T;
    }
    return SMC_OK;
}

struct SeriesScope {
    FilterView& v;
    explicit SeriesScope(FilterView& view) : v(view) {}
    ~SeriesScope() { v.want_s2 = 1; v.y = nullptr; v.trace_logmu = nullptr; v.trace_ess = nullptr; v.sum_np = v.sum_mom = 0; v.sum_q = v.sum_m = nullptr; }
};

static hipError_t do_persist(smc_filter_s* h, uint32_t t0, uint32_t t1, PersistCtl pc) {
    return by_model(h->model, [&](auto M) {
        if constexpr (decltype(M)::value == MODEL_UCSV_RB) return hipErrorCooperativeLaunchTooLarge;
        else return launch_persist<decltype(M)::value>(h->v, h->geo, h->cur, t0, t1, pc, h->stream);
    });
}
static hipError_t do_resident(smc_filter_s* h, int T) {
    if (h->v.prop_kind)
        return by_guided_model(h->model, [&](auto M) { return launch_resident_g<decltype(M)::value>(h->v, T, h->d_recs, h->stream); });
    return by_model(h->model, [&](auto M) { return launch_resident<decltype(M)::value>(h->v, T, h->d_recs, h->stream); });
}
int enqueue_log_likelihood(smc_handle h, double y0, int64_t T, bool want_trace, bool summ) {
    const bool resident = h->resident_ok && resident_supported(h->model, h->v.seg) && !(summ && (h->v.systematic || !summaries_fit_lds(h)));
    SeriesScope scope(h->v);
    h->v.y = h->d_y;
    h->v.trace_logmu = want_trace ? h->d_tr_logmu : nullptr;
    h->v.trace_ess = want_trace ? h->d_tr_ess : nullptr;
    h->cur = 0;
    h->v.want_s2 = want_trace ? 1 : 0;
    int rc = SMC_OK;
    if (summ && resident) view_summaries(h);
    if (summ && !resident) {
        h->v.want_s2 = 1;
        HIPCHK(do_init(h, y0));
        h->t = 1; h->inited = true; h->emitted = false;
        if ((rc = emit_if_needed(h))) return rc;
        if ((rc = enqueue_step_summaries(h, 0))) return rc;
        for (int64_t t = 1; t < T; ++t) {
            HIPCHK(ensure_breaks(h, (uint32_t)t, (uint32_t)T));
            HIPCHK(do_step(h, (uint32_t)t, 0, 0.0));
            h->cur ^= 1; h->t += 1; h->emitted = false;
            if ((rc = emit_if_needed(h))) return rc;
            if ((rc = enqueue_step_summaries(h, t))) return rc;
        }
        return SMC_OK;
    }
    if (resident) {
        HIPCHK(do_resident(h, (int)T));
        h->cur = 0; h->t = (uint32_t)T; h->inited = true; h->emitted = true;
    } else {
        if (T == 1) h->v.want_s2 = 1;
        HIPCHK(do_init(h, y0));
        h->t = 1; h->inited = true; h->emitted = false;
        int64_t t_first = 1;
        if (h->persist.on < 0) { const char* e = getenv("SMC_PERSIST"); h->persist.on = (e && atoi(e) == 1) ? 1 : 0; }
        if (h->persist.on == 1 && !h->v.prop_kind && !want_trace && h->v.nseg > 1 && !h->v.skip && !h->v.anc && T > 3) {
            const size_t nfl = (size_t)h->v.ntheta * h->v.nseg;
            if (!h->persist.d_flags) {
                HIPCHK(dalloc(&h->persist.d_flags, 2 * nfl));
                HIPCHK(hipHostMalloc((void**)&h->persist.h_err, 16, hipHostMallocDefault));
            }
            *h->persist.h_err = 0;
            while (t_first < T - 1) {
                HIPCHK(ensure_breaks(h, (uint32_t)t_first, (uint32_t)T));
                int64_t t_end = (int64_t)h->v.brk_t0 + h->brk_count;
                t_end = t_end > T - 1 ? T - 1 : t_end;
                HIPCHK(hipMemsetAsync(h->persist.d_flags, 0, 2 * nfl * 4, h->stream));
                PersistCtl pc{{h->persist.d_flags, h->persist.d_flags + nfl}, h->persist.h_err};
                const hipError_t pe = do_persist(h, (uint32_t)t_first, (uint32_t)t_end, pc);
                if (pe == hipErrorCooperativeLaunchTooLarge) { h->persist.on = 0; break; }
                HIPCHK(pe);
                if ((t_end - t_first) & 1) h->cur ^= 1;
                h->t += (uint32_t)(t_end - t_first);
                t_first = t_end;
            }
        }
        for (int64_t t = t_first; t < T; ++t) {
            const int emit = h->v.want_s2 ? 1 : 2;
            if (t == T - 1) h->v.want_s2 = 1;
            HIPCHK(ensure_breaks(h, (uint32_t)t, (uint32_t)T));
            HIPCHK(do_step(h, (uint32_t)t, emit, 0.0));
            h->cur ^= 1; h->t += 1;
        }
        h->v.want_s2 = 1;
        rc = emit_if_needed(h);
    }
    return rc;
}

extern "C" int smc_log_likelihood(smc_handle h, const double* y, int64_t T, double* logZ, double* logmu_trace,
                                  double* ess_trace) {
    if (!h || !y) return fail(SMC_EINVAL, "smc_log_likelihood: NULL argument");
    if (T <= 0) return fail(SMC_EINVAL, "smc_log_likelihood: T must be positive");
    if (!h->have_params) return fail(SMC_ESTATE, "smc_log_likelihood: smc_set_params has not been called");
    h->win.k = 0;
    HIPCHK(hipSetDevice(h->device));
    int rc = ensure_y(h, T);
    if (rc) return rc;
    const bool want_trace = logmu_trace || ess_trace;
    if (want_trace && (rc = ensure_trace(h, T))) return rc;
    const bool resident = h->resident_ok && resident_supported(h->model, h->v.seg);
    if (resident && (rc = ensure_recs(h, T))) return rc;
    const bool summ = summaries_on(h);
    if (summ && (rc = ensure_summaries(h, T))) return rc;
    h->summ.T = 0;
    h->summ.skip.clear();
    HIPCHK(hipMemcpyAsync(h->d_y, y, (size_t)T * 8, hipMemcpyHostToDevice, h->stream));
    if (h->skip.on) { h->v.skip = h->skip.d_mask; h->v.order = h->skip.d_order; h->v.n_active = h->skip.d_order + h->v.ntheta; }
    const int cur0 = h->cur;
    HIPCHK(hipEventRecord(h->ev0, h->stream));
    rc = enqueue_log_likelihood(h, y[0], T, want_trace, summ);
    h->v.skip = nullptr; h->v.order = nullptr; h->v.n_active = nullptr;
    if (rc) return rc;
    if (h->skip.on && h->cur != cur0) HIPCHK(copy_slots(h->v, h->cur, h->v, cur0, h->d, h->skip.d_mask, h->stream));
    if (summ) {
        h->summ.T = T;
        if (h->skip.on) h->summ.skip = h->skip.h_mask;
    }
    rc = finish_elapsed(h, logZ);
    if (rc) return rc;
    if (h->persist.h_err && *h->persist.h_err) {
        *h->persist.h_err = 0;
        h->persist.on = 0;
        h->inited = false;
        return fail(SMC_EHIP, "smc_log_likelihood: the persistent step kernel gave up (a workgroup waited 100 ms for the previous step: "
                              "not every workgroup resident?); the handle falls back to one launch per step - call again");
    }
    if (logmu_trace) HIPCHK(hipMemcpy(logmu_trace, h->d_tr_logmu, (size_t)T * h->v.ntheta * 8, hipMemcpyDeviceToHost));
    if (ess_trace) HIPCHK(hipMemcpy(ess_trace, h->d_tr_ess, (size_t)T * h->v.ntheta * 8, hipMemcpyDeviceToHost));
    if (h->skip.on && want_trace) {
        const double nan = std::numeric_limits<double>::quiet_NaN();
        const size_t nt = (size_t)h->v.ntheta;
        for (size_t m = 0; m < nt; ++m) {
            if (!h->skip.h_mask[m]) continue;
            for (int64_t t = 0; t < T; ++t) {
                if (logmu_trace) logmu_trace[(size_t)t * nt + m] = nan;
                if (ess_trace) ess_trace[(size_t)t * nt + m] = nan;
            }
        }
    }
    return SMC_OK;
}

extern "C" int smc_time_step_kernel(smc_handle h, const double* y, int64_t T, int nsample, double* avg_ms,
                                    double* min_ms) {
    if (!h || !y || T < 2 || nsample < 1) return fail(SMC_EINVAL, "smc_time_step_kernel: bad argument");
    if (!h->have_params) return fail(SMC_ESTATE, "smc_time_step_kernel: smc_set_params has not been called");
    HIPCHK(hipSetDevice(h->device));
    int rc = ensure_y(h, T);
    if (rc) return rc;
    const int G = T - 1 >= 512 ? 32 : (T - 1 >= 64 ? 8 : 1);
    if ((int64_t)nsample * G > T - 1) nsample = (int)((T - 1) / G);
    std::vector<hipEvent_t> e0((size_t)nsample), e1((size_t)nsample);
    for (int i = 0; i < nsample; ++i) { HIPCHK(hipEventCreate(&e0[i])); HIPCHK(hipEventCreate(&e1[i])); }
    HIPCHK(hipMemcpyAsync(h->d_y, y, (size_t)T * 8, hipMemcpyHostToDevice, h->stream));
    SeriesScope scope(h->v);
    h->v.y = h->d_y; h->v.trace_logmu = nullptr; h->v.trace_ess = nullptr;
    h->cur = 0;
    h->v.want_s2 = 0;
    HIPCHK(do_init(h, y[0]));
    h->t = 1; h->inited = true; h->emitted = false;
    const int64_t stride = (T - 1) / nsample;
    int k = 0, open_left = 0;
    for (int64_t t = 1; t < T; ++t) {
        const int emit = h->v.want_s2 ? 1 : 2;
        if (t == T - 1) h->v.want_s2 = 1;
        HIPCHK(ensure_breaks(h, (uint32_t)t, (uint32_t)T));
        if (!open_left && k < nsample && ((t - 1) % stride) == (stride - G) / 2) {
            HIPCHK(hipEventRecord(e0[k], h->stream));
            open_left = G;
        }
        HIPCHK(do_step(h, (uint32_t)t, emit, 0.0));
        if (open_left && --open_left == 0) { HIPCHK(hipEventRecord(e1[k], h->stream)); ++k; }
        h->cur ^= 1; h->t += 1;
    }
    if (open_left) { HIPCHK(hipEventRecord(e1[k], h->stream)); }
    h->v.want_s2 = 1;
    rc = emit_if_needed(h);
    if (rc) return rc;
    HIPCHK(hipStreamSynchronize(h->stream));
    double sum = 0.0, mn = 1e30;
    for (int i = 0; i < k; ++i) {
        float ms = 0.f;
        HIPCHK(hipEventElapsedTime(&ms, e0[i], e1[i]));
        sum += ms / G;
        mn = ms / G < mn ? ms / G : mn;
    }
    for (int i = 0; i < nsample; ++i) { (void)hipEventDestroy(e0[i]); (void)hipEventDestroy(e1[i]); }
    if (avg_ms) *avg_ms = k ? sum / k : 0.0;
    if (min_ms) *min_ms = k ? mn : 0.0;
    return SMC_OK;
}

__global__ void k_nop() {}

extern "C" int smc_event_overhead_ms(smc_handle h, int nsample, double* avg_ms) {
    if (!h || !avg_ms || nsample < 1) return fail(SMC_EINVAL, "smc_event_overhead_ms: bad argument");
    HIPCHK(hipSetDevice(h->device));
    std::vector<hipEvent_t> e0((size_t)nsample), e1((size_t)nsample);
    for (int i = 0; i < nsample; ++i) { HIPCHK(hipEventCreate(&e0[i])); HIPCHK(hipEventCreate(&e1[i])); }
    for (int i = 0; i < nsample; ++i) {
        hipLaunchKernelGGL(k_nop, dim3(1), dim3(64), 0, h->stream);
        HIPCHK(hipEventRecord(e0[i], h->stream));
        HIPCHK(hipEventRecord(e1[i], h->stream));
    }
    HIPCHK(hipStreamSynchronize(h->stream));
    double sum = 0.0;
    for (int i = 0; i < nsample; ++i) {
        float ms = 0.f;
        HIPCHK(hipEventElapsedTime(&ms, e0[i], e1[i]));
        sum += ms;
        (void)hipEventDestroy(e0[i]); (void)hipEventDestroy(e1[i]);
    }
    *avg_ms = sum / nsample;
    return SMC_OK;
}
```

### sequential_monte_carlo_amd/csrc/smc_capi_slots.hip

```cpp
#include "smc_host.h"
#include "smc_slot_kernels.h"

#include <cstring>

using namespace smc;

hipError_t copy_slots(const FilterView& dst, int dcur, const FilterView& src, int scur, int d, const unsigned char* mask, hipStream_t s) {
    hipLaunchKernelGGL(k_copy_slots, dim3((unsigned)((dst.npad + 255) / 256), dst.ntheta), dim3(256), 0, s, dst, dcur, src, scur, d, mask);
    return hipGetLastError();
}

extern "C" int smc_get_state(smc_handle h, double* x, double* w, int32_t* anc) {
    if (!h) return fail(SMC_EINVAL, "smc_get_state: NULL handle");
    if (!h->inited) return fail(SMC_ESTATE, "smc_get_state: filter not initialised");
    HIPCHK(hipSetDevice(h->device));
    const FilterView& v = h->v;
    HIPCHK(hipStreamSynchronize(h->stream));
    const size_t rows = (size_t)h->d * v.ntheta;
    if (x)
        HIPCHK(hipMemcpy2D(x, (size_t)v.n * 8, v.x[h->cur], (size_t)v.npad * 8, (size_t)v.n * 8, rows,
                           hipMemcpyDeviceToHost));
    if (anc) {
        if (!v.anc) return fail(SMC_ESTATE, "smc_get_state: handle created without SMC_FLAG_ANCESTORS");
        HIPCHK(hipMemcpy2D(anc, (size_t)v.n * 4, v.anc, (size_t)v.npad * 4, (size_t)v.n * 4, (size_t)v.ntheta,
                           hipMemcpyDeviceToHost));
    }
    if (w) {
        int rc = emit_if_needed(h);
        if (rc) return rc;
        if (!h->d_wdense) HIPCHK(dalloc(&h->d_wdense, (size_t)v.ntheta * v.n + 2 * (size_t)h->d * v.ntheta));
        hipLaunchKernelGGL(k_dense_weights, dim3((unsigned)((v.n + 255) / 256), v.ntheta), dim3(256), 0, h->stream, v,
                           h->cur, h->d_wdense);
        HIPCHK(hipGetLastError());
        HIPCHK(hipStreamSynchronize(h->stream));
        HIPCHK(hipMemcpy(w, h->d_wdense, (size_t)v.ntheta * v.n * 8, hipMemcpyDeviceToHost));
    }
    return SMC_OK;
}

extern "C" int smc_permute(smc_handle h, const int32_t* a) {
    if (!h || !a) return fail(SMC_EINVAL, "smc_permute: NULL argument");
    if (!h->inited) return fail(SMC_ESTATE, "smc_permute: filter not initialised");
    h->win.k = 0;
    for (int m = 0; m < h->v.ntheta; ++m)
        if (a[m] < 0 || a[m] >= h->v.ntheta) return fail(SMC_EINVAL, "smc_permute: index out of range");
    HIPCHK(hipSetDevice(h->device));
    int rc = emit_if_needed(h);
    if (rc) return rc;
    const FilterView& v = h->v;
    if (!h->h_perm) HIPCHK(hipHostMalloc((void**)&h->h_perm, (size_t)v.ntheta * 4, hipHostMallocDefault));
    else HIPCHK(hipStreamSynchronize(h->stream));
    memcpy(h->h_perm, a, (size_t)v.ntheta * 4);
    HIPCHK(hipMemcpyAsync(h->d_perm, h->h_perm, (size_t)v.ntheta * 4, hipMemcpyHostToDevice, h->stream));
    HIPCHK(hipMemcpyAsync(h->d_logZ_tmp, v.logZ, (size_t)v.ntheta * 8, hipMemcpyDeviceToDevice, h->stream));
    hipLaunchKernelGGL(k_permute, dim3((unsigned)((v.npad + 255) / 256), v.ntheta), dim3(256), 0, h->stream, v, h->cur, h->d,
                       h->d_perm, h->d_logZ_tmp);
    HIPCHK(hipGetLastError());
    h->cur ^= 1;
    HIPCHK(hipMemcpyAsync(h->d_logZ_tmp, v.logZ, (size_t)v.ntheta * 8, hipMemcpyDeviceToDevice, h->stream));
    HIPCHK(do_finalize(h, 0, h->t - 1));
    HIPCHK(hipMemcpyAsync(v.logZ, h->d_logZ_tmp, (size_t)v.ntheta * 8, hipMemcpyDeviceToDevice, h->stream));
    return SMC_OK;
}

extern "C" int smc_copy_from(smc_handle dst, smc_handle src, const uint8_t* mask) {
    if (!dst || !src || !mask) return fail(SMC_EINVAL, "smc_copy_from: NULL argument");
    if (dst == src) return fail(SMC_EINVAL, "smc_copy_from: dst and src are the same handle");
    if (!dst->inited || !src->inited) return fail(SMC_ESTATE, "smc_copy_from: filter not initialised");
    dst->win.k = 0;
    const FilterView &a = dst->v, &b = src->v;
    if (dst->model != src->model || a.n != b.n || a.seg != b.seg || a.ntheta != b.ntheta || dst->device != src->device)
        return fail(SMC_EINVAL, "smc_copy_from: handles differ in model, geometry or device");
    HIPCHK(hipSetDevice(dst->device));
    int rc = emit_if_needed(dst);
    if (rc) return rc;
    rc = emit_if_needed(src);
    if (rc) return rc;
    HIPCHK(hipStreamSynchronize(src->stream));
    unsigned char* d_mask = reinterpret_cast<unsigned char*>(dst->d_perm);
    HIPCHK(hipMemcpyAsync(d_mask, mask, (size_t)a.ntheta, hipMemcpyHostToDevice, dst->stream));
    HIPCHK(copy_slots(a, dst->cur, b, src->cur, dst->d, d_mask, dst->stream));
    HIPCHK(hipStreamSynchronize(dst->stream));
    dst->t = src->t;
    return SMC_OK;
}

extern "C" int smc_slot_bytes(smc_handle h, int64_t* bytes) {
    if (!h || !bytes) return fail(SMC_EINVAL, "smc_slot_bytes: NULL argument");
    *bytes = slot_words(h->d, h->v.npad, h->v.nseg) * 8;
    return SMC_OK;
}

static int pack_unpack(smc_handle h, const int32_t* idx, int64_t k, void* buf, bool pack) {
    if (!h || k < 0 || (k > 0 && (!idx || !buf))) return fail(SMC_EINVAL, "smc_pack/unpack_slots: bad argument");
    if (!h->inited) return fail(SMC_ESTATE, "smc_pack/unpack_slots: filter not initialised");
    if (!pack) h->win.k = 0;
    if (k == 0) return SMC_OK;
    for (int64_t i = 0; i < k; ++i)
        if (idx[i] < 0 || idx[i] >= h->v.ntheta) return fail(SMC_EINVAL, "smc_pack/unpack_slots: index out of range");
    HIPCHK(hipSetDevice(h->device));
    int rc = emit_if_needed(h);
    if (rc) return rc;
    const FilterView& v = h->v;
    const int64_t W = slot_words(h->d, v.npad, v.nseg);
    const int64_t span = v.npad > v.nseg ? v.npad : v.nseg;
    for (int64_t k0 = 0; k0 < k; k0 += v.ntheta) {
        const int64_t kc = k - k0 < v.ntheta ? k - k0 : v.ntheta;
        HIPCHK(hipMemcpyAsync(h->d_perm, idx + k0, (size_t)kc * 4, hipMemcpyHostToDevice, h->stream));
        const dim3 grid((unsigned)((span + 255) / 256), (unsigned)kc);
        uint64_t* b = (uint64_t*)buf + (size_t)k0 * W;
        if (pack)
            hipLaunchKernelGGL((k_pack_slots<true>), grid, dim3(256), 0, h->stream, v, h->cur, h->d, h->d_perm, b);
        else
            hipLaunchKernelGGL((k_pack_slots<false>), grid, dim3(256), 0, h->stream, v, h->cur, h->d, h->d_perm, b);
        HIPCHK(hipGetLastError());
        HIPCHK(hipStreamSynchronize(h->stream));
    }
    return SMC_OK;
}
extern "C" int smc_pack_slots(smc_handle h, const int32_t* idx, int64_t k, void* device_buf) {
    return pack_unpack(h, idx, k, device_buf, true);
}
extern "C" int smc_unpack_slots(smc_handle h, const int32_t* idx, int64_t k, const void* device_buf) {
    return pack_unpack(h, idx, k, const_cast<void*>(device_buf), false);
}

extern "C" int smc_get_weights_raw(smc_handle h, uint64_t* C, double* m, uint64_t* S, uint64_t* S2hi, uint64_t* S2lo) {
    if (!h) return fail(SMC_EINVAL, "smc_get_weights_raw: NULL handle");
    if (!h->inited) return fail(SMC_ESTATE, "smc_get_weights_raw: filter not initialised");
    HIPCHK(hipSetDevice(h->device));
    HIPCHK(hipStreamSynchronize(h->stream));
    const FilterView& v = h->v;
    const size_t np = (size_t)v.ntheta * v.npad * 8, ns = (size_t)v.ntheta * v.nseg * 8;
    const int c = h->cur;
    if (C) HIPCHK(hipMemcpy(C, v.C[c], np, hipMemcpyDeviceToHost));
    if (m) HIPCHK(hipMemcpy(m, v.segk[c], ns, hipMemcpyDeviceToHost));
    if (S) HIPCHK(hipMemcpy(S, v.segS[c], ns, hipMemcpyDeviceToHost));
    if (S2hi) HIPCHK(hipMemcpy(S2hi, v.segS2hi[c], ns, hipMemcpyDeviceToHost));
    if (S2lo) HIPCHK(hipMemcpy(S2lo, v.segS2lo[c], ns, hipMemcpyDeviceToHost));
    return SMC_OK;
}
```

### sequential_monte_carlo_amd/csrc/smc_host.h

```cpp
#pragma once
#include "../../include/smc_hip.h"
#include "smc_launch.h"

#include <string>
#include <vector>

#pragma GCC visibility push(hidden)

int fail(int code, const std::string& msg);
#define HIPCHK(expr)                                                                                          \
    do {                                                                                                      \
        hipError_t _e = (expr);                                                                               \
        if (_e != hipSuccess)                                                                                 \
            return fail(SMC_EHIP, std::string(#expr) + ": " + hipGetErrorString(_e) + " (" __FILE__ ":" +      \
                                      std::to_string(__LINE__) + ")");                                        \
    } while (0)

template <class T>
inline hipError_t dalloc(T** p, size_t count) {
    return hipMalloc((void**)p, count * sizeof(T) > 0 ? count * sizeof(T) : 16);
}

namespace smc {
struct PmmhDev {
    double* theta;
    double* prop;
    double* logZ;
    double* lp;
    unsigned char* skip;
    unsigned char* mask;
    unsigned char* any;
    unsigned long long* nrun;
    double* chol;
    int32_t* order;
    int32_t* counts;
};
}

struct smc_filter_s {
    int model = 0, d = 0, device = 0;
    uint32_t flags = 0;
    smc::FilterView v{};
    smc::Params* d_params = nullptr;
    uint32_t* d_stream = nullptr;
    int32_t* d_perm = nullptr;
    double* d_logZ_tmp = nullptr;
    double* d_y = nullptr;
    int64_t ycap = 0;
    double *d_tr_logmu = nullptr, *d_tr_ess = nullptr;
    int64_t trcap = 0;
    double* d_wdense = nullptr;
    smc::StepRec* d_recs = nullptr;
    int64_t reccap = 0;
    double* h_pin = nullptr;
    uint32_t seq = 0;
    size_t slab_bytes = 0, pin_bytes = 0;
    char* d_slab = nullptr;
    uint64_t* d_brk = nullptr;
    uint32_t brk_cap = 0, brk_count = 0;
    int32_t* h_perm = nullptr;
    std::vector<double> prop_par;
    smc::PropRow *d_prop = nullptr, *h_prop = nullptr;
    smc::Params* h_params = nullptr;
    hipStream_t stream = nullptr;
    hipEvent_t ev0 = nullptr, ev1 = nullptr;
    int cur = 0;
    uint32_t t = 0;
    bool inited = false;
    bool emitted = false;
    bool have_params = false;
    bool resident_ok = false;
    smc::Geo geo{0, 0};
    double last_ms = 0.0;

    struct {
        unsigned char* d_mask = nullptr;
        int32_t* d_order = nullptr;
        bool on = false;
        std::vector<uint8_t> h_mask;
    } skip;
    struct {
        int np = 0, comp = 0, mom = 0;
        uint64_t p64[smc::QMAX] = {};
        double p[smc::QMAX] = {};
        int mode = SMC_SUMM_WEIGHTED;
        double *d_q = nullptr, *d_m = nullptr;
        int64_t cap = 0, T = 0;
        std::vector<uint8_t> skip;
        uint64_t* d_ms = nullptr;
        double* h_once = nullptr;
    } summ;
    struct {
        unsigned* d_flags = nullptr;
        int* h_err = nullptr;
        int on = -1;
    } persist;
    struct {
        double* h_out = nullptr;
        int k = 0;
    } win;
    struct {
        smc::PmmhSpec spec{};
        bool cfg = false;
        smc::PmmhDev dev{};
        double* h_out = nullptr;
        double* d_in = nullptr;
        double* h_in = nullptr;
        size_t in_words = 0;
    } pm;
};

inline bool affine_row_ok(const double* par) {
    for (int k = 0; k < smc::PROP_NPAR; ++k)
        if (!smc::finite_d(par[k])) return false;
    return par[3] > 0.0;
}

hipError_t do_init(smc_filter_s* h, double y);
hipError_t do_step(smc_filter_s* h, uint32_t t, int emit_prev, double y);
hipError_t do_finalize(smc_filter_s* h, int first_emit, uint32_t t_emit);
hipError_t ensure_breaks(smc_filter_s* h, uint32_t t, uint32_t t_end);
int ensure_y(smc_handle h, int64_t T);
int ensure_recs(smc_handle h, int64_t T);
int emit_if_needed(smc_handle h);
int finish_elapsed(smc_handle h, double* logZ = nullptr, double* logmu = nullptr, double* ess = nullptr);
int enqueue_log_likelihood(smc_handle h, double y0, int64_t T, bool want_trace, bool summ = false);
inline bool summaries_on(const smc_filter_s* h) { return h->summ.np > 0 || h->summ.mom != 0; }
bool summaries_fit_lds(const smc_filter_s* h);
int ensure_summaries(smc_handle h, int64_t T);
void view_summaries(smc_handle h);
int enqueue_step_summaries(smc_handle h, int64_t row);
hipError_t copy_slots(const smc::FilterView& dst, int dcur, const smc::FilterView& src, int scur, int d, const unsigned char* mask, hipStream_t s);

#pragma GCC visibility pop
```

### sequential_monte_carlo_amd/csrc/smc_kernels.h

```cpp
#pragma once
#include "smc_spec.h"

namespace smc {

constexpr int WAVE = 64;
__host__ __device__ constexpr int lds_pad(int i) { return i + ((i >> 5) << 1); }
__host__ __device__ constexpr int lds_probe_off(int s) { return s >= 32 ? lds_pad(s - 32) + 31 : s - 1; }
__host__ __device__ constexpr int lds_step_inc(int s) { return s >= 32 ? lds_pad(s) : s; }
__host__ __device__ constexpr int lds_unpad(int pp) { return pp - 2 * (pp / 34); }
__host__ __device__ constexpr int lds_padded_len(int n) { return n + (n >> 4) + 8; }

typedef __attribute__((address_space(3))) const char lds_byte;
typedef __attribute__((address_space(3))) const uint64_t lds_u64;
typedef __attribute__((address_space(3))) const double lds_f64;
__device__ __forceinline__ lds_byte* lds_ptr(const void* p) { return (lds_byte*)p; }
__device__ __forceinline__ uint64_t lds_load_u64(lds_byte* p) { return *(lds_u64*)p; }

typedef unsigned long long nt_v2u64 __attribute__((ext_vector_type(2)));
template <bool WT = false, class T>
__device__ __forceinline__ void store_out(T* p, const T& val) {
    static_assert(sizeof(T) == 16, "16-byte stores");
    if (WT) {
        const nt_v2u64 v2 = *reinterpret_cast<const nt_v2u64*>(&val);
        asm volatile("global_store_dwordx4 %0, %1, off sc1\n\ts_nop 1" : : "v"(p), "v"(v2) : "memory");
    } else {
        __builtin_nontemporal_store(*reinterpret_cast<const nt_v2u64*>(&val), reinterpret_cast<nt_v2u64*>(p));
    }
}
template <bool WT, class T>
__device__ __forceinline__ void store_word(T* p, T val) {
    static_assert(sizeof(T) == 8, "8-byte words");
    if (WT) __hip_atomic_store(reinterpret_cast<unsigned long long*>(p), __builtin_bit_cast(unsigned long long, val), __ATOMIC_RELAXED, __HIP_MEMORY_SCOPE_AGENT);
    else *p = val;
}

struct FilterView {
    int64_t n;
    int64_t npad;
    int seg, nseg, nseg_p2, SH;
    int ntheta;
    uint64_t seed;
    const Params* params;
    const uint32_t* stream;
    double* x[2];
    uint64_t* C[2];
    double* segk[2];
    uint64_t* segS[2];
    uint64_t* segS2hi[2];
    uint64_t* segS2lo[2];
    const uint64_t* brk;
    uint32_t brk_t0;
    int32_t* anc;
    double* logZ;
    double* last_logmu;
    double* last_ess;
    double* last_K;
    uint64_t* last_D;
    double* trace_logmu;
    double* trace_ess;
    const double* y;
    uint64_t* tabD;
    int* tabsh;
    uint32_t host_seq;
    double* host_out;
    int systematic;
    double inv_n;
    int emit_now;
    int want_s2;
    const unsigned char* skip;
    const int32_t* order;
    const int32_t* n_active;
    int sum_np, sum_comp, sum_mom, sum_unw;
    uint64_t sum_p64[8];
    double* sum_q;
    double* sum_m;
    int abl;
    int prop_kind;
    unsigned long long* dbg;
    PropRow* prop;
};

#ifdef SMC_ABLATE
#define SMC_ABL(v, bit) (((v).abl >> (bit)) & 1)
#define SMC_STAMP(v, k)                                                                                   \
    do {                                                                                                  \
        if ((v).dbg && threadIdx.x == 0)                                                                  \
            (v).dbg[((size_t)blockIdx.y * gridDim.x + blockIdx.x) * 8 + (k)] = __builtin_amdgcn_s_memrealtime(); \
    } while (0)
#else
#define SMC_ABL(v, bit) 0
#define SMC_STAMP(v, k) do { } while (0)
#endif
template <class VIEW>
__device__ __forceinline__ void host_emit(const VIEW& v, int th, double z, double logmu, double ess) {
    if (!v.host_out) return;
    v.host_out[th] = z;
    v.host_out[(size_t)v.ntheta + th] = logmu;
    v.host_out[2 * (size_t)v.ntheta + th] = ess;
    if (v.host_seq) {
        __threadfence_system();
        __hip_atomic_store(&v.host_out[3 * (size_t)v.ntheta + th], (double)v.host_seq, __ATOMIC_RELEASE, __HIP_MEMORY_SCOPE_SYSTEM);
    }
}
constexpr int QMAX = 8;
__host__ __device__ inline uint64_t order_key(double x) {
    const uint64_t b = d2bits(x);
    return (b >> 63) ? ~b : (b | 0x8000000000000000ULL);
}
__host__ __device__ inline double key_value(uint64_t k) { return bits2d((k >> 63) ? (k & 0x7fffffffffffffffULL) : ~k); }
__host__ __device__ inline uint64_t prob_to_u64(double p) {
    if (!(p > 0.0)) return 0;
    if (p >= 1.0) return ~(uint64_t)0;
    return (uint64_t)(p * TWO_P64);
}
struct Q7Rank { int64_t j; double g; };
__host__ __device__ inline Q7Rank q7_rank(int64_t n, double p) {
    const double h = (double)n * p + (1.0 - p);
    int64_t j = (int64_t)h;
    j = j > n - 1 ? n - 1 : (j < 1 ? 1 : j);
    double g = h - (double)j;
    g = g > 1.0 ? 1.0 : (g < 0.0 ? 0.0 : g);
    Q7Rank r; r.j = j; r.g = g;
    return r;
}
__host__ __device__ inline double q7_interp(double a, double b, double g) {
    const bool fin = (a - a == 0.0) && (b - b == 0.0);
    return fin ? a + g * (b - a) : (1.0 - g) * a + g * b;
}
__host__ __device__ inline double q7_level(double p) { return p > 0.0 ? (p < 1.0 ? p : 1.0) : 0.0; }


#ifndef SMC_NORMALS_EARLY
#define SMC_NORMALS_EARLY 0
#endif
#define SMC_PRIO(ph) __builtin_amdgcn_s_setprio((short)(3 - (ph)))

__device__ __forceinline__ int smc_tid() {
    int t = (int)threadIdx.x;
#if defined(SMC_TID_OPAQUE)
    asm volatile("" : "+v"(t));
#endif
    return t;
}

template <int CTRL, int ROW_MASK>
__device__ __forceinline__ uint32_t dpp_u32(uint32_t old, uint32_t v) {
    return (uint32_t)__builtin_amdgcn_update_dpp((int)old, (int)v, CTRL, ROW_MASK, 0xf, false);
}
template <int CTRL>
__device__ __forceinline__ uint64_t dpp_add_u64(uint64_t v) {
    uint32_t lo = (uint32_t)v, hi = (uint32_t)(v >> 32);
#define SMC_DPP_ADD64(MOD)                                                                                  \
    asm volatile("s_nop 1\n\tv_add_co_u32_dpp %0, vcc, %0, %0 " MOD "\n\ts_nop 1\n\tv_addc_co_u32_dpp %1, vcc, %1, %1, vcc " MOD \
                 : "+v"(lo), "+v"(hi) : : "vcc")
    static_assert(CTRL == 0x111 || CTRL == 0x112 || CTRL == 0x114 || CTRL == 0x118 || CTRL == 0x142 || CTRL == 0x143, "DPP control");
    if (CTRL == 0x111) SMC_DPP_ADD64("row_shr:1 row_mask:0xf bank_mask:0xf bound_ctrl:1");
    if (CTRL == 0x112) SMC_DPP_ADD64("row_shr:2 row_mask:0xf bank_mask:0xf bound_ctrl:1");
    if (CTRL == 0x114) SMC_DPP_ADD64("row_shr:4 row_mask:0xf bank_mask:0xf bound_ctrl:1");
    if (CTRL == 0x118) SMC_DPP_ADD64("row_shr:8 row_mask:0xf bank_mask:0xf bound_ctrl:1");
    if (CTRL == 0x142) SMC_DPP_ADD64("row_bcast:15 row_mask:0xa bank_mask:0xf");
    if (CTRL == 0x143) SMC_DPP_ADD64("row_bcast:31 row_mask:0xc bank_mask:0xf");
#undef SMC_DPP_ADD64
    return ((uint64_t)hi << 32) | lo;
}
__device__ __forceinline__ uint64_t wave_incl_scan(uint64_t v, int ) {
    v = dpp_add_u64<0x111>(v);
    v = dpp_add_u64<0x112>(v);
    v = dpp_add_u64<0x114>(v);
    v = dpp_add_u64<0x118>(v);
    v = dpp_add_u64<0x142>(v);
    v = dpp_add_u64<0x143>(v);
    return v;
}
__device__ __forceinline__ uint32_t wave_incl_scan_u32(uint32_t v) {
    v += dpp_u32<0x111, 0xf>(0u, v);
    v += dpp_u32<0x112, 0xf>(0u, v);
    v += dpp_u32<0x114, 0xf>(0u, v);
    v += dpp_u32<0x118, 0xf>(0u, v);
    v += dpp_u32<0x142, 0xa>(0u, v);
    v += dpp_u32<0x143, 0xc>(0u, v);
    return v;
}
__device__ __forceinline__ uint64_t wave_incl_scan_52(uint64_t v) {
    const uint32_t lo = wave_incl_scan_u32((uint32_t)v & 0x3ffffffu);
    const uint32_t hi = wave_incl_scan_u32((uint32_t)(v >> 26));
    return ((uint64_t)hi << 26) + lo;
}
__device__ __forceinline__ uint64_t readlane_u64(uint64_t v, int l) {
    const uint32_t lo = (uint32_t)__builtin_amdgcn_readlane((int)(uint32_t)v, l);
    const uint32_t hi = (uint32_t)__builtin_amdgcn_readlane((int)(uint32_t)(v >> 32), l);
    return ((uint64_t)hi << 32) | lo;
}
__device__ __forceinline__ uint64_t wave_sum(uint64_t v) { return readlane_u64(wave_incl_scan(v, 0), WAVE - 1); }
template <int NW>
__device__ __forceinline__ void wave_totals(const uint64_t* tot, int lane, int wave, uint64_t& off, uint64_t& all) {
    static_assert(NW >= 1 && NW <= 16 && (NW & (NW - 1)) == 0, "wave count");
    uint64_t t = tot[lane & (NW - 1)];
    if (NW > 1) t = dpp_add_u64<0x111>(t);
    if (NW > 2) t = dpp_add_u64<0x112>(t);
    if (NW > 4) t = dpp_add_u64<0x114>(t);
    if (NW > 8) t = dpp_add_u64<0x118>(t);
    const int ws = __builtin_amdgcn_readfirstlane(wave);
    all = readlane_u64(t, NW - 1);
    const uint64_t prev = readlane_u64(t, ws > 0 ? ws - 1 : 0);
    off = ws > 0 ? prev : 0;
}

struct U128 {
    uint64_t lo, hi;
};
__device__ __forceinline__ U128 add128(U128 a, U128 b) {
    U128 r;
    r.lo = a.lo + b.lo;
    r.hi = a.hi + b.hi + (r.lo < a.lo ? 1u : 0u);
    return r;
}
__device__ __forceinline__ U128 sq128(uint64_t q) {
    U128 r;
    r.hi = __umul64hi(q, q);
    r.lo = q * q;
    return r;
}
template <int CTRL>
__device__ __forceinline__ U128 dpp_add_u128(U128 v) {
    uint32_t w0 = (uint32_t)v.lo, w1 = (uint32_t)(v.lo >> 32), w2 = (uint32_t)v.hi, w3 = (uint32_t)(v.hi >> 32);
#define SMC_DPP_ADD128(MOD)                                                                                       \
    asm volatile("s_nop 1\n\tv_add_co_u32_dpp %0, vcc, %0, %0 " MOD "\n\ts_nop 1\n\tv_addc_co_u32_dpp %1, vcc, %1, %1, vcc " MOD \
                 "\n\ts_nop 1\n\tv_addc_co_u32_dpp %2, vcc, %2, %2, vcc " MOD "\n\ts_nop 1\n\tv_addc_co_u32_dpp %3, vcc, %3, %3, vcc " MOD \
                 : "+v"(w0), "+v"(w1), "+v"(w2), "+v"(w3) : : "vcc")
    static_assert(CTRL == 0x111 || CTRL == 0x112 || CTRL == 0x114 || CTRL == 0x118 || CTRL == 0x142 || CTRL == 0x143, "DPP control");
    if (CTRL == 0x111) SMC_DPP_ADD128("row_shr:1 row_mask:0xf bank_mask:0xf bound_ctrl:1");
    if (CTRL == 0x112) SMC_DPP_ADD128("row_shr:2 row_mask:0xf bank_mask:0xf bound_ctrl:1");
    if (CTRL == 0x114) SMC_DPP_ADD128("row_shr:4 row_mask:0xf bank_mask:0xf bound_ctrl:1");
    if (CTRL == 0x118) SMC_DPP_ADD128("row_shr:8 row_mask:0xf bank_mask:0xf bound_ctrl:1");
    if (CTRL == 0x142) SMC_DPP_ADD128("row_bcast:15 row_mask:0xa bank_mask:0xf");
    if (CTRL == 0x143) SMC_DPP_ADD128("row_bcast:31 row_mask:0xc bank_mask:0xf");
#undef SMC_DPP_ADD128
    return U128{((uint64_t)w1 << 32) | w0, ((uint64_t)w3 << 32) | w2};
}
__device__ __forceinline__ U128 wave_sum128(U128 v) {
    v = dpp_add_u128<0x111>(v);
    v = dpp_add_u128<0x112>(v);
    v = dpp_add_u128<0x114>(v);
    v = dpp_add_u128<0x118>(v);
// ... 334 lines not shown
    uint64_t basek = 0;
    constexpr bool MERGED = NP > 1 && NP * NW <= 16;
    uint64_t tt = 0;
    if (MERGED) {
        tt = wtot[lane & (NP * NW - 1)];
        tt = dpp_add_u64<0x111>(tt);
        if (NP * NW > 2) tt = dpp_add_u64<0x112>(tt);
        if (NP * NW > 4) tt = dpp_add_u64<0x114>(tt);
        if (NP * NW > 8) tt = dpp_add_u64<0x118>(tt);
    }
#pragma unroll
    for (int k = 0; k < NP; ++k) {
        uint64_t off, ktot;
        if (MERGED) {
            const int j = __builtin_amdgcn_readfirstlane(k * NW + wave);
            off = j > 0 ? readlane_u64(tt, j > 0 ? j - 1 : 0) : 0;
            ktot = 0;
        } else {
            wave_totals<NW>(wtot + k * NW, lane, wave, off, ktot);
        }
        const uint64_t excl = basek + off + incl[k] - ps[k];
        ulonglong2 cc;
        cc.x = excl + q[k][0];
        cc.y = cc.x + q[k][1];
        if (PADDED) *reinterpret_cast<ulonglong2*>(Cout + lds_pad(2 * (tid + k * THREADS))) = cc;
        else store_out<WT>(reinterpret_cast<ulonglong2*>(Cout + 2 * (tid + k * THREADS)), cc);
        basek += ktot;
    }
    if (MERGED) basek = readlane_u64(tt, NP * NW - 1);
    SegRec rec;
    rec.kb = kb;
    rec.S = basek;
    rec.hi = rec.lo = 0;
    if (tid == 0) {
        U128 t{0, 0};
#pragma unroll
        for (int w = 0; w < NW; ++w) t = add128(t, U128{w2[w], w2[NW + w]});
        rec.hi = t.hi;
        rec.lo = t.lo;
    }
    return rec;
}

template <int THREADS, int NP, bool WT = false, class VIEW>
__device__ __forceinline__ SegRec segment_epilogue(const VIEW& v, int nxt, int th, int sb, double (&lw)[NP][2],
                                                   uint64_t* scr) {
    uint64_t* Cout = v.C[nxt] + (size_t)th * v.npad + (size_t)sb * v.seg;
    const SegRec rec = segment_normalize<THREADS, NP, false, WT>(lw, scr, Cout, v.want_s2 != 0);
    if (smc_tid() == 0) {
        const size_t r = (size_t)th * v.nseg + sb;
        store_word<WT>(&v.segk[nxt][r], rec.kb);
        store_word<WT>(&v.segS[nxt][r], rec.S);
        store_word<WT>(&v.segS2hi[nxt][r], rec.hi);
        store_word<WT>(&v.segS2lo[nxt][r], rec.lo);
    }
    return rec;
}

template <class VIEW>
__device__ __forceinline__ void emit_own(const VIEW& v, int th, const SegRec& rec, uint32_t t_emit, bool first_emit) {
    const int sh = seg_shift(rec.kb, rec.kb, v.SH);
    const uint64_t D = seg_Q(rec.S, sh), R = seg_R(rec.hi, rec.lo, sh, v.SH);
    double logmu, ess;
    combine_outputs(rec.kb, D, R, v.SH, v.n, logmu, ess);
    v.last_logmu[th] = logmu;
    v.last_ess[th] = ess;
    v.last_K[th] = rec.kb;
    v.last_D[th] = D;
    if (v.trace_logmu) v.trace_logmu[(size_t)t_emit * v.ntheta + th] = logmu;
    if (v.trace_ess) v.trace_ess[(size_t)t_emit * v.ntheta + th] = ess;
    const double z = first_emit ? logmu : v.logZ[th] + logmu;
    v.logZ[th] = z;
    host_emit(v, th, z, logmu, ess);
}

template <class VIEW>
__device__ __forceinline__ void emit_from_totals(const VIEW& v, int th, double K, uint64_t Dtot, bool first_emit, uint32_t t_emit) {
    double logmu, ess;
    combine_outputs(K, Dtot, 0, v.SH, v.n, logmu, ess);
    v.last_logmu[th] = logmu;
    v.last_ess[th] = ess;
    v.last_K[th] = K;
    v.last_D[th] = Dtot;
    if (v.trace_logmu) v.trace_logmu[(size_t)t_emit * v.ntheta + th] = logmu;
    if (v.trace_ess) v.trace_ess[(size_t)t_emit * v.ntheta + th] = ess;
    const double z = first_emit ? logmu : v.logZ[th] + logmu;
    v.logZ[th] = z;
    host_emit(v, th, z, logmu, ess);
}

__device__ __forceinline__ double nan_mask() { return bits2d(0x7ff8000000000000ULL); }

__device__ __forceinline__ int logical_segment(int bid, int nseg) {
    return (nseg & 7) ? bid : (bid & 7) * (nseg >> 3) + (bid >> 3);
}

template <int MODEL, int THREADS, int NP>
__global__ __launch_bounds__(THREADS) void k_init(FilterView v, int nxt, double y) {
    constexpr int D = model_dim<MODEL>::value, NZ = model_nz<MODEL>::value;
    extern __shared__ __attribute__((aligned(16))) char smem[];
    uint64_t* scr = (uint64_t*)smem;
    const int sb = logical_segment(blockIdx.x, v.nseg), th = blockIdx.y, tid = smc_tid();
    if (v.skip && v.skip[th]) return;
    const Params prm = v.params[th];
    const uint32_t stream = v.stream[th];
    const int64_t seg0 = (int64_t)sb * v.seg;
    double lw[NP][2];
#pragma unroll
    for (int k = 0; k < NP; ++k) {
        const int pl = tid + k * THREADS;
        const int64_t i0 = seg0 + 2 * pl;
        const uint32_t pg = (uint32_t)(i0 >> 1);
        double z[NZ][2], xn[2][D];
#pragma unroll
        for (int c = 0; c < NZ; ++c) box_muller(draw(v.seed, pg, stream, 0u, SLOT_NORMAL0 + c), z[c][0], z[c][1]);
#pragma unroll
        for (int j = 0; j < 2; ++j) {
            double zz[NZ];
#pragma unroll
            for (int c = 0; c < NZ; ++c) zz[c] = z[c][j];
            const bool valid = (i0 + j) < v.n;
            if constexpr (model_marginal<MODEL>::value) {
                const double l = model_marginal_step<MODEL>(prm, true, xn[j], zz, y, xn[j]);
                lw[k][j] = valid ? l : nan_mask();
            } else {
                model_initial<MODEL>(prm, zz, xn[j]);
                lw[k][j] = valid ? model_logobs<MODEL>(prm, xn[j], y) : nan_mask();
            }
        }
#pragma unroll
        for (int c = 0; c < D; ++c) {
            double2 o;
            o.x = (i0 < v.n) ? xn[0][c] : 0.0;
            o.y = (i0 + 1 < v.n) ? xn[1][c] : 0.0;
            store_out(reinterpret_cast<double2*>(v.x[nxt] + ((size_t)c * v.ntheta + th) * v.npad + i0), o);
        }
        if (v.anc) {
            int2 o;
            o.x = (int)i0;
            o.y = (int)i0 + 1;
            *reinterpret_cast<int2*>(v.anc + (size_t)th * v.npad + i0) = o;
        }
    }
    const SegRec rec = segment_epilogue<THREADS, NP>(v, nxt, th, sb, lw, scr);
    if (v.emit_now && v.nseg == 1 && tid == 0) emit_own(v, th, rec, 0u, true);
}

__host__ __device__ constexpr int nstage_for(int seg) { return seg >= 8192 ? 1 : (seg >= 4096 ? 2 : 3); }
__host__ __device__ inline size_t step_lds_bytes(int nseg_p2, int threads, int np, bool multi) {
    const size_t base = (size_t)nseg_p2 * 16 + scr_words(threads, np) * 8;
    return base + (size_t)(multi ? nstage_for(2 * np * threads) : 1) * lds_padded_len(2 * np * threads) * 8;
}

template <int MODEL, int THREADS, int NP, bool MULTI, bool SYS, bool PERSIST, class VIEW, bool GTAB = false, int RPT = 1, bool GUIDED = false>
__device__ __forceinline__ void step_body(const VIEW& v, int cur, uint32_t t, int emit_prev, double yval, char* smem) {
    static_assert(!GTAB || (MULTI && !PERSIST), "global table: multi-segment launches");
    static_assert(RPT == 1 || (RPT == 2 && MULTI && !GTAB && !PERSIST), "two records per thread: multi-segment launches");
    constexpr int D = model_dim<MODEL>::value, NZ = model_nz<MODEL>::value;
    static_assert(!(GUIDED && model_marginal<MODEL>::value), "marginal families have no proposals");
    constexpr int SEG = 2 * NP * THREADS;
    constexpr int NQ = 2 * NP;
    constexpr int NSTAGE = nstage_for(SEG);
    constexpr int SEGP = lds_padded_len(SEG);
    int sb_ = logical_segment(blockIdx.x, v.nseg), th_ = blockIdx.y, tid_ = smc_tid();
    if (PERSIST) {
        asm volatile("" : "+v"(tid_));
    }
    const int sb = sb_, th = th_, tid = tid_;
    if (!PERSIST && v.skip && v.skip[th]) return;
    const int nxt = cur ^ 1;
    const Params prm = v.params[th];
    PropRow prw;
    if constexpr (GUIDED) prw = v.prop[th];
    const uint32_t stream = v.stream[th];
    const double y = v.y ? v.y[t] : yval;
    const uint32_t seg0 = (uint32_t)sb * (uint32_t)SEG, n32 = (uint32_t)v.n;
    const uint64_t* Cprev = v.C[cur] + (size_t)th * v.npad;
    const double* xprev = v.x[cur];
    uint64_t* scr;
#ifdef SMC_ABLATE
    if (SMC_ABL(v, 8) && (blockIdx.x & 8)) {
        __builtin_amdgcn_s_sleep(127);
        __builtin_amdgcn_s_sleep(127);
    }
#endif
    SMC_STAMP(v, 0);
    SMC_PRIO(0);

    uint64_t F0 = 0, F1 = 0;
    if (MULTI && !SYS) {
        const uint64_t* Fb = v.brk + ((size_t)(t - v.brk_t0) * v.ntheta + th) * ((size_t)v.nseg + 1) + sb;
        F0 = Fb[0];
        F1 = Fb[1];
    }
    const TablePre tpre = (MULTI && !GTAB) ? table_preload<THREADS, VIEW, RPT>(v, cur, th, emit_prev && sb == 0) : TablePre{-inf(), 0, 0, 0, -inf(), 0};
    uint64_t rr[NQ];
#pragma unroll
    for (int k = 0; k < NP; ++k) {
        if (SYS) { rr[2 * k] = rr[2 * k + 1] = 0; continue; }
        const uint32_t pg = (uint32_t)((seg0 >> 1) + tid + k * THREADS);
        const u32x4 rw = SMC_ABL(v, 3) ? u32x4{{pg * 2654435761u, pg ^ t, pg * 40503u, ~pg}} : draw(v.seed, pg, stream, t, SLOT_RESAMPLE);
        rr[2 * k] = ((uint64_t)rw.v[1] << 32) | rw.v[0];
        rr[2 * k + 1] = ((uint64_t)rw.v[3] << 32) | rw.v[2];
    }
    const uint32_t m_blk = (seg0 + SEG < n32 ? seg0 + SEG : n32) - seg0;
    const bool ragged = seg0 + SEG > n32;
    uint32_t kk[NQ];
#pragma unroll
    for (int i = 0; i < NQ; ++i) kk[i] = 2 * (tid + (i >> 1) * THREADS) + (i & 1);
    if (ragged) {
        asm volatile("; ragged");
#pragma unroll
        for (int i = 0; i < NQ; ++i) kk[i] = (seg0 + kk[i] < n32 ? seg0 + kk[i] : n32 - 1) - seg0;
    }
    uint64_t Tg[NQ];

    constexpr bool SPEC = MULTI && NSTAGE == 3;
    ulonglong2 stg[NSTAGE][NP];
    int spec_lo = 0;
    if (SPEC) {
        spec_lo = sb - 1 < 0 ? 0 : sb - 1;
        spec_lo = spec_lo + NSTAGE > v.nseg ? (v.nseg - NSTAGE < 0 ? 0 : v.nseg - NSTAGE) : spec_lo;
#pragma unroll
        for (int sg = 0; sg < NSTAGE; ++sg) {
#pragma unroll
            for (int k = 0; k < NP; ++k) stg[sg][k] = ulonglong2{0, 0};
            if (spec_lo + sg < v.nseg) {
                const ulonglong2* src = reinterpret_cast<const ulonglong2*>(Cprev + (size_t)(spec_lo + sg) * SEG);
#pragma unroll
                for (int k = 0; k < NP; ++k) stg[sg][k] = src[tid + k * THREADS];
            }
        }
    }

    ulonglong2 stg1[NP];
    constexpr bool EARLY1 = D == 1;
#pragma unroll
    for (int k = 0; k < NP; ++k)
        stg1[k] = (!MULTI && EARLY1) ? reinterpret_cast<const ulonglong2*>(Cprev)[tid + k * THREADS] : ulonglong2{0, 0};

    constexpr bool LATE_Z = D >= 3 && NP >= 2 && !SYS;
    double z[NP][NZ][2];
#pragma unroll
    for (int k = 0; k < NP; ++k) {
        if (LATE_Z) break;
        const uint32_t pg = (uint32_t)((seg0 >> 1) + tid + k * THREADS);
#pragma unroll
        for (int c = 0; c < NZ; ++c) {
            if (SMC_ABL(v, 2)) { z[k][c][0] = 1e-3 * (double)(pg & 1023); z[k][c][1] = -z[k][c][0]; }
            else if (SMC_ABL(v, 6)) { const u32x4 w4 = draw(v.seed, pg, stream, t, SLOT_NORMAL0 + c); z[k][c][0] = 1e-9 * (double)w4.v[0]; z[k][c][1] = 1e-9 * (double)w4.v[2]; }
            else box_muller(draw(v.seed, pg, stream, t, SLOT_NORMAL0 + c), z[k][c][0], z[k][c][1]);
            if (SYS || SMC_NORMALS_EARLY) asm volatile("" : "+v"(z[k][c][0]), "+v"(z[k][c][1]));
        }
    }


    uint64_t alive;
    uint64_t Sseg[NQ];
    int bseg[NQ];
    uint64_t* Cst = nullptr;
    int blo = 0;
    const int tab_p2 = GTAB ? 0 : v.nseg_p2;
    if (MULTI) {
        TableLds L = carve(smem, tab_p2);
        if (GTAB) {
            L.Dcum = v.tabD + (size_t)th * v.nseg_p2;
            L.sh = v.tabsh + (size_t)th * v.nseg_p2;
        }
        scr = L.scr;
        uint64_t* sysw = L.scr + scr_words(THREADS, NP) - 8;
        if (SYS && tid == 0) {
            const u32x4 uw = draw(v.seed, 0u, stream, t, SLOT_SYS);
            sysw[0] = ((uint64_t)uw.v[1] << 32) | uw.v[0];
        }
        const bool emitter = emit_prev && sb == 0;
        const bool emit_totals = emitter && emit_prev == 2;
        const int s_hi = spec_lo + NSTAGE - 1 < v.nseg - 1 ? spec_lo + NSTAGE - 1 : v.nseg - 1;
        const bool use_fast = SPEC && (GTAB || ((!emitter || emit_totals) && v.nseg_p2 <= RPT * THREADS));
        uint64_t P0 = 0, Dc[NSTAGE];
        int shw[NSTAGE];
        if (GTAB) {
            alive = L.Dcum[v.nseg - 1];
            if (SPEC) {
                P0 = spec_lo ? L.Dcum[spec_lo - 1] : 0;
#pragma unroll
                for (int i = 0; i < NSTAGE; ++i) { Dc[i] = L.Dcum[spec_lo + i]; shw[i] = L.sh[spec_lo + i]; }
            }
            if (SYS) __syncthreads();
        } else if (use_fast) {
            double Kw;
            alive = window_prologue<THREADS, NSTAGE, VIEW, RPT>(v, L.scr, tpre, spec_lo, P0, Dc, shw, Kw);
            if (emit_totals && tid == 0) emit_from_totals(v, th, Kw, alive, t == 1u, t - 1u);
        } else {
            alive = table_prologue<THREADS>(v, cur, th, L, emitter, t == 1u, t - 1u, RPT == 1 ? &tpre : nullptr);
        }
        SMC_STAMP(v, 1);
        SMC_PRIO(1);
        SysBase sbase{};
        uint64_t Tfirst, Tlast, lo_ = 0;
        if (SYS) {
            sbase = sys_base(alive, n32, v.inv_n, sysw[0], (uint64_t)seg0);
            Tfirst = sys_target(sbase, 0u);
            Tlast = sys_target(sbase, m_blk - 1);
        } else {
            mul64wide(F0, alive, Tfirst, lo_);
            mul64wide(F1, alive, Tlast, lo_);
        }
        bool fast = false;
        if (use_fast) {
            fast = (spec_lo == 0 || P0 <= Tfirst) && Tlast < Dc[s_hi - spec_lo];
            if (!fast && !GTAB) alive = table_prologue<THREADS>(v, cur, th, L, false, false, 0u, RPT == 1 ? &tpre : nullptr);
        }
        int b_lo = 0, b_hi = 0;
        if (fast || (SPEC && !use_fast && (spec_lo == 0 || L.Dcum[spec_lo - 1] <= Tfirst) && Tlast < L.Dcum[s_hi])) {
            b_lo = spec_lo;
            b_hi = s_hi;
        } else {
            for (int s = v.nseg_p2 >> 1; s >= 1; s >>= 1) {
                b_lo += (L.Dcum[b_lo + s - 1] <= Tfirst) ? s : 0;
                b_hi += (L.Dcum[b_hi + s - 1] <= Tlast) ? s : 0;
            }
            b_lo = b_lo < v.nseg ? b_lo : v.nseg - 1;
            b_hi = b_hi < v.nseg ? b_hi : v.nseg - 1;
            b_hi = b_hi < b_lo ? b_lo : b_hi;
        }
        int w0 = 1;
        while (w0 < b_hi - b_lo + 1) w0 <<= 1;
        Cst = (uint64_t*)(smem + (size_t)tab_p2 * 16 + scr_words(THREADS, NP) * 8);
        const bool spec_ok = SPEC && b_lo >= spec_lo && b_hi < spec_lo + NSTAGE;
        int st_lo = spec_lo;
        if (!spec_ok) {
            st_lo = b_lo;
            const int nst = (b_hi - b_lo + 1) < NSTAGE ? (b_hi - b_lo + 1) : NSTAGE;
#pragma unroll
            for (int sg = 0; sg < NSTAGE; ++sg) {
#pragma unroll
                for (int k = 0; k < NP; ++k) stg[sg][k] = ulonglong2{0, 0};
                if (sg < nst) {
                    const ulonglong2* src = reinterpret_cast<const ulonglong2*>(Cprev + (size_t)(b_lo + sg) * SEG);
#pragma unroll
                    for (int k = 0; k < NP; ++k) stg[sg][k] = src[tid + k * THREADS];
                }
            }
        }
        blo = st_lo;
        int pos[NQ];
#pragma unroll
        for (int i = 0; i < NQ; ++i) {
            if (SYS) {
                Tg[i] = sys_target(sbase, kk[i]);
            } else {
                uint64_t pick;
#if SMC_EXP_PICKF64
                pick = (uint64_t)(fma((double)(uint32_t)(rr[i] >> 32), 0x1p-32, (double)((uint32_t)rr[i] >> 11) * 0x1p-53) * (double)(Tlast - Tfirst));
#else
                mul64wide(rr[i], Tlast - Tfirst, pick, lo_);
#endif
                Tg[i] = kk[i] == m_blk - 1 ? Tlast : Tfirst + pick;
            }
            pos[i] = b_lo;
        }
        if (fast) {
#pragma unroll
            for (int i = 0; i < NQ; ++i) {
                int r = 0;
                uint64_t base = P0;
                int shc = shw[0];
#pragma unroll
                for (int k = 0; k + 1 < NSTAGE; ++k) {
                    const bool up = Dc[k] <= Tg[i];
                    r += up ? 1 : 0;
                    base = up ? Dc[k] : base;
                    shc = up ? shw[k + 1] : shc;
                }
                bseg[i] = spec_lo + r;
                Sseg[i] = 0;
                Tg[i] = ((Tg[i] - base + 1) << shc) - 1;
            }
        } else {
            for (int s = w0 >> 1; s >= 1; s >>= 1) {
#pragma unroll
                for (int i = 0; i < NQ; ++i) {
                    const int c = pos[i] + s;
                    pos[i] = (c <= b_hi && L.Dcum[c - 1] <= Tg[i]) ? c : pos[i];
                }
            }
#pragma unroll
            for (int i = 0; i < NQ; ++i) {
                bseg[i] = pos[i];
                Sseg[i] = 0;
                const uint64_t base = bseg[i] ? L.Dcum[bseg[i] - 1] : 0;
                Tg[i] = sys_threshold(Tg[i] - base, L.sh[bseg[i]]);
            }
        }
    } else {
        const TableLds L = carve(smem, v.nseg_p2);
        scr = L.scr;
        if (emit_prev && sb == 0) table_prologue<THREADS>(v, cur, th, L, true, t == 1u, t - 1u);
        alive = v.segS[cur][(size_t)th * v.nseg];
#pragma unroll
        for (int i = 0; i < NQ; ++i) { bseg[i] = 0; Sseg[i] = alive; }
        if (SYS) {
            const int sh = seg_shift(0.0, 0.0, v.SH);
            const uint64_t Dtot = seg_Q(alive, sh);
            const u32x4 uw = draw(v.seed, 0u, stream, t, SLOT_SYS);
            const SysBase sbase = sys_base(Dtot, n32, v.inv_n, ((uint64_t)uw.v[1] << 32) | uw.v[0], 0u);
#pragma unroll
            for (int i = 0; i < NQ; ++i) Tg[i] = sys_threshold(sys_target(sbase, kk[i]), sh);
            alive = Dtot;
        }
    }

    SMC_STAMP(v, 2);
    SMC_STAMP(v, 3);
    uint64_t T2[NQ];
#pragma unroll
    for (int i = 0; i < NQ; ++i) {
        uint64_t lo;
        if (SYS || MULTI) T2[i] = Tg[i];
        else mul64wide(rr[i], Sseg[i], T2[i], lo);
    }
    if (MULTI) {
#pragma unroll
        for (int sg = 0; sg < NSTAGE; ++sg)
#pragma unroll
            for (int k = 0; k < NP; ++k)
                *reinterpret_cast<ulonglong2*>(Cst + sg * SEGP + lds_pad(2 * (tid + k * THREADS))) = stg[sg][k];
        __syncthreads();
    } else {
        Cst = (uint64_t*)(smem + (size_t)v.nseg_p2 * 16 + scr_words(THREADS, NP) * 8);
#pragma unroll
        for (int k = 0; k < NP; ++k) {
            const ulonglong2 c2 = EARLY1 ? stg1[k] : reinterpret_cast<const ulonglong2*>(Cprev)[tid + k * THREADS];
            *reinterpret_cast<ulonglong2*>(Cst + lds_pad(2 * (tid + k * THREADS))) = c2;
        }
        __syncthreads();
    }
    SMC_STAMP(v, 4);
    SMC_PRIO(2);
    int pos[NQ];
#pragma unroll
    for (int i = 0; i < NQ; ++i) pos[i] = 0;
    if (SMC_ABL(v, 0)) {
#pragma unroll
        for (int i = 0; i < NQ; ++i) pos[i] = (int)(T2[i] & (SEG - 1));
    } else if (MULTI) {
        bool far = false;
        lds_byte* pb[NQ];
        lds_byte* pb0[NQ];
#pragma unroll
        for (int i = 0; i < NQ; ++i) {
            const int r = bseg[i] - blo;
            far |= r >= NSTAGE;
            pb0[i] = lds_ptr(Cst + (r < NSTAGE ? r : 0) * SEGP);
            pb[i] = pb0[i];
        }
#pragma unroll
        for (int s = SEG >> 1; s >= 1; s >>= 1) {
            uint64_t val[NQ];
#pragma unroll
            for (int i = 0; i < NQ; ++i) val[i] = lds_load_u64(pb[i] + 8 * lds_probe_off(s));
#pragma unroll
            for (int i = 0; i < NQ; ++i) pb[i] += (val[i] <= T2[i]) ? 8 * lds_step_inc(s) : 0;
        }
#pragma unroll
        for (int i = 0; i < NQ; ++i) pos[i] = lds_unpad((int)(pb[i] - pb0[i]) >> 3);
        if (__builtin_amdgcn_ballot_w64(far)) {
#pragma unroll
            for (int i = 0; i < NQ; ++i) {
                if (bseg[i] - blo >= NSTAGE) {
                    const uint64_t* Cb = Cprev + (size_t)bseg[i] * SEG;
                    int pp = 0;
                    for (int s = SEG >> 1; s >= 1; s >>= 1) pp += (Cb[pp + s - 1] <= T2[i]) ? s : 0;
                    pos[i] = pp;
                }
            }
        }
    } else {
        lds_byte* pb[NQ];
#pragma unroll
        for (int i = 0; i < NQ; ++i) pb[i] = lds_ptr(Cst);
#pragma unroll
        for (int s = SEG >> 1; s >= 1; s >>= 1) {
            uint64_t val[NQ];
#pragma unroll
            for (int i = 0; i < NQ; ++i) val[i] = lds_load_u64(pb[i] + 8 * lds_probe_off(s));
#pragma unroll
            for (int i = 0; i < NQ; ++i) pb[i] += (val[i] <= T2[i]) ? 8 * lds_step_inc(s) : 0;
        }
#pragma unroll
        for (int i = 0; i < NQ; ++i) pos[i] = lds_unpad((int)(pb[i] - lds_ptr(Cst)) >> 3);
    }
    SMC_STAMP(v, 5);
    uint32_t anc[NQ];
    double xp[NQ][D];
#pragma unroll
    for (int i = 0; i < NQ; ++i) {
        const uint32_t own = seg0 + 2 * (tid + (i >> 1) * THREADS) + (i & 1);
        uint32_t a = (uint32_t)bseg[i] * (uint32_t)SEG + (uint32_t)pos[i];
        if (!alive || ragged) {
            asm volatile("; collapsed or ragged");
            a = alive ? a : own;
            a = a < n32 ? a : n32 - 1;
        }
        anc[i] = a;
#pragma unroll
        for (int c = 0; c < D; ++c) xp[i][c] = SMC_ABL(v, 1) ? 0.25 * (double)(a & 7) : xprev[((size_t)c * v.ntheta + th) * v.npad + a];
    }

    double lw[NP][2];
#pragma unroll
    for (int k = 0; k < NP; ++k) {
        const uint32_t i0 = seg0 + 2 * (tid + k * THREADS);
        double xn[2][D];
        if (LATE_Z) {
            const uint32_t pg = (uint32_t)((seg0 >> 1) + tid + k * THREADS);
#pragma unroll
            for (int c = 0; c < NZ; ++c) box_muller(draw(v.seed, pg, stream, t, SLOT_NORMAL0 + c), z[k][c][0], z[k][c][1]);
        }
#pragma unroll
        for (int j = 0; j < 2; ++j) {
            double zz[NZ];
#pragma unroll
            for (int c = 0; c < NZ; ++c) zz[c] = z[k][c][j];
            if constexpr (model_marginal<MODEL>::value) {
                lw[k][j] = model_marginal_step<MODEL>(prm, false, xp[2 * k + j], zz, y, xn[j]);
            } else if constexpr (GUIDED) {
                lw[k][j] = model_guided<MODEL>(prm, prw, xp[2 * k + j], zz, y, xn[j]);
            } else {
                model_transition<MODEL>(prm, xp[2 * k + j], zz, xn[j]);
                lw[k][j] = model_logobs<MODEL>(prm, xn[j], y);
            }
        }
        if (ragged) {
            asm volatile("; ragged");
#pragma unroll
            for (int j = 0; j < 2; ++j)
                if (i0 + j >= n32) {
                    lw[k][j] = nan_mask();
#pragma unroll
                    for (int c = 0; c < D; ++c) xn[j][c] = 0.0;
                }
        }
#pragma unroll
        for (int c = 0; c < D; ++c) {
            double2 o;
            o.x = xn[0][c];
            o.y = xn[1][c];
            store_out<PERSIST>(reinterpret_cast<double2*>(v.x[nxt] + ((size_t)c * v.ntheta + th) * v.npad + i0), o);
        }
        if (v.anc) {
            int2 o;
            o.x = (int)anc[2 * k];
            o.y = (int)anc[2 * k + 1];
            *reinterpret_cast<int2*>(v.anc + (size_t)th * v.npad + i0) = o;
        }
    }
    SMC_STAMP(v, 6);
    SMC_PRIO(3);
    if (SMC_ABL(v, 4)) {
        double acc = 0;
#pragma unroll
        for (int k = 0; k < NP; ++k) acc += lw[k][0] + lw[k][1];
        if (acc == 1.2345) v.logZ[th] = acc;
        return;
    }
    const SegRec rec = segment_epilogue<THREADS, NP, PERSIST>(v, nxt, th, sb, lw, scr);
    if (!MULTI && v.emit_now && tid == 0) emit_own(v, th, rec, t, false);
    SMC_STAMP(v, 7);
}

template <int MODEL, int THREADS, int NP, bool MULTI, bool SYS = false, bool GTAB = false, int RPT = 1, bool GUIDED = false>
__global__ __launch_bounds__(THREADS) void k_step(FilterView v, int cur, uint32_t t, int emit_prev, double yval) {
    extern __shared__ __attribute__((aligned(16))) char smem[];
    step_body<MODEL, THREADS, NP, MULTI, SYS, false, FilterView, GTAB, RPT, GUIDED>(v, cur, t, emit_prev, yval, smem);
}

struct PersistCtl {
    unsigned* flags[2];
    int* err;
};
template <int MODEL, int THREADS, int NP>
__global__ __launch_bounds__(THREADS, (THREADS >= 512 ? 4 : (THREADS >= 256 ? 4 : 2))) void k_persist(FilterView v_arg, int cur, uint32_t t0, uint32_t t1, PersistCtl pc) {
    extern __shared__ __attribute__((aligned(16))) char smem[];
    const int tid = threadIdx.x;
    typedef __attribute__((address_space(4))) const char karg_byte;
    karg_byte* ka = (karg_byte*)__builtin_amdgcn_kernarg_segment_ptr();
    int* expired_flag = (int*)((uint64_t*)(smem + (size_t)v_arg.nseg_p2 * 16) + scr_words(THREADS, NP) - 1);
    if (tid == 0) *expired_flag = 0;
    unsigned long long* acc = (unsigned long long*)((uint64_t*)(smem + (size_t)v_arg.nseg_p2 * 16) + scr_words(THREADS, NP) - 5);
    if (v_arg.dbg && tid == 0) { acc[0] = acc[1] = acc[2] = 0; acc[3] = __builtin_amdgcn_s_memrealtime(); }
    for (uint32_t t = t0; t < t1; ++t) {
        asm volatile("" : "+s"(ka));
        typedef __attribute__((address_space(4))) const FilterView karg_view;
        karg_view& v = *(karg_view*)ka;
        const int sb = logical_segment(blockIdx.x, v.nseg), th = blockIdx.y;
        if (t > t0) {
            if (tid < v.nseg) {
                const unsigned* f = pc.flags[cur] + (size_t)th * v.nseg + tid;
                const unsigned long long start = __builtin_amdgcn_s_memrealtime();
                while (__hip_atomic_load(f, __ATOMIC_RELAXED, __HIP_MEMORY_SCOPE_AGENT) != t) {
                    if (__builtin_amdgcn_s_memrealtime() - start > 10000000ull) { *expired_flag = 1; break; }
                    __builtin_amdgcn_s_sleep(2);
                }
            }
            if (tid == 0) {
                __builtin_amdgcn_fence(__ATOMIC_ACQUIRE, "agent");
                asm volatile("s_waitcnt vmcnt(0)" ::: "memory");
            }
            __syncthreads();
            if (*expired_flag) {
                if (tid == 0) *pc.err = 1;
                return;
            }
        }
        if (v.dbg && tid == 0) { const unsigned long long now = __builtin_amdgcn_s_memrealtime(); acc[0] += now - acc[3]; acc[3] = now; }
        step_body<MODEL, THREADS, NP, true, false, true>(v, cur, t, 2, 0.0, smem);
        if (v.dbg && tid == 0) { const unsigned long long now = __builtin_amdgcn_s_memrealtime(); acc[1] += now - acc[3]; acc[3] = now; }
        asm volatile("s_waitcnt vmcnt(0)" ::: "memory");
        __syncthreads();
        if (tid == 0) __hip_atomic_store(pc.flags[cur ^ 1] + (size_t)th * v.nseg + sb, t + 1u, __ATOMIC_RELAXED, __HIP_MEMORY_SCOPE_AGENT);
        if (v.dbg && tid == 0) { const unsigned long long now = __builtin_amdgcn_s_memrealtime(); acc[2] += now - acc[3]; acc[3] = now; }
        cur ^= 1;
    }
    if (v_arg.dbg && tid == 0) {
        unsigned long long* d = v_arg.dbg + ((size_t)gridDim.y * gridDim.x + (size_t)blockIdx.y * gridDim.x + blockIdx.x) * 8;
        d[0] = t1 - t0; d[1] = acc[0]; d[2] = acc[1]; d[3] = acc[2]; d[7] = 0x5045525349535421ull;
    }
}

template <int THREADS>
__global__ __launch_bounds__(THREADS) void k_finalize(FilterView v, int cur, int first_emit, uint32_t t_emit) {
    extern __shared__ __attribute__((aligned(16))) char smem[];
    if (v.skip && v.skip[blockIdx.x]) {
        if (threadIdx.x == 0) {
            v.logZ[blockIdx.x] = -inf();
            if (v.host_out) v.host_out[blockIdx.x] = -inf();
        }
        return;
    }
    const TableLds L = carve(smem, v.nseg_p2);
    table_prologue<THREADS>(v, cur, blockIdx.x, L, true, first_emit != 0, t_emit);
}

template <int THREADS>
__global__ __launch_bounds__(THREADS) void k_table(FilterView v, int cur, int emit, int first_emit, uint32_t t_emit) {
    constexpr int NW = THREADS / WAVE;
    constexpr int DEADK = (int)0x80000000;
    __shared__ int redk[NW];
    __shared__ uint64_t wt[NW], wr[NW];
    const int th = blockIdx.x, tid = threadIdx.x, lane = tid & (WAVE - 1), wave = tid / WAVE;
    if (v.skip && v.skip[th]) {
        if (emit != 0 && tid == 0) {
            v.logZ[th] = -inf();
            if (v.host_out) v.host_out[th] = -inf();
        }
        return;
    }
    const size_t base = (size_t)th * v.nseg;
    const double* sk = v.segk[cur] + base;
    const uint64_t* sS = v.segS[cur] + base;
    uint64_t* Dcum = v.tabD + (size_t)th * v.nseg_p2;
    int* shv = v.tabsh + (size_t)th * v.nseg_p2;
    int ki = DEADK;
    for (int b = tid; b < v.nseg; b += THREADS) {
        const double k = sk[b];
        const int kb = k == -inf() ? DEADK : (int)k;
        ki = kb > ki ? kb : ki;
    }
    ki = wave_max_i32(ki);
    if (lane == 0) redk[wave] = ki;
    __syncthreads();
    int km = redk[0];
#pragma unroll
    for (int w = 1; w < NW; ++w) km = redk[w] > km ? redk[w] : km;
    const double K = km == DEADK ? -inf() : (double)km;
    constexpr int EMAX = 16;
    const int E = v.nseg_p2 >= THREADS ? v.nseg_p2 / THREADS : 1, w0 = wave * E * WAVE;
    uint64_t inc[EMAX], carry = 0, rsum = 0;
    int she[EMAX];
#pragma unroll
    for (int i = 0; i < EMAX; ++i) {
        inc[i] = 0; she[i] = 64;
        if (i < E) {
            const int b = w0 + i * WAVE + lane;
            uint64_t Q = 0;
            if (b < v.nseg) {
                she[i] = seg_shift(K, sk[b], v.SH);
                Q = seg_Q(sS[b], she[i]);
                if (emit == 1) rsum += seg_R(v.segS2hi[cur][base + b], v.segS2lo[cur][base + b], she[i], v.SH);
            }
            inc[i] = wave_incl_scan(Q, lane) + carry;
            carry = readlane_u64(inc[i], WAVE - 1);
        }
    }
    if (lane == 0) wt[wave] = carry;
    if (emit == 1) {
        const uint64_t rw = wave_sum(rsum);
        if (lane == 0) wr[wave] = rw;
    }
    __syncthreads();
    uint64_t off = 0, Dtot = 0;
#pragma unroll
    for (int w = 0; w < NW; ++w) { off += w < wave ? wt[w] : 0; Dtot += wt[w]; }
#pragma unroll
    for (int i = 0; i < EMAX; ++i)
        if (i < E) {
            const int b = w0 + i * WAVE + lane;
            if (b < v.nseg_p2) { Dcum[b] = off + inc[i]; shv[b] = she[i]; }
        }
    if (emit == 1 && tid == 0) {
        uint64_t Rtot = 0;
#pragma unroll
        for (int w = 0; w < NW; ++w) Rtot += wr[w];
        double logmu, ess;
        combine_outputs(K, Dtot, Rtot, v.SH, v.n, logmu, ess);
        v.last_logmu[th] = logmu;
        v.last_ess[th] = ess;
        v.last_K[th] = K;
        v.last_D[th] = Dtot;
        if (v.trace_logmu) v.trace_logmu[(size_t)t_emit * v.ntheta + th] = logmu;
        if (v.trace_ess) v.trace_ess[(size_t)t_emit * v.ntheta + th] = ess;
        const double z = first_emit ? logmu : v.logZ[th] + logmu;
        v.logZ[th] = z;
        host_emit(v, th, z, logmu, ess);
    }
    if (emit == 2 && tid == 0) emit_from_totals(v, th, K, Dtot, first_emit != 0, t_emit);
}

}
```

### sequential_monte_carlo_amd/csrc/smc_launch.h

```cpp
#pragma once
#include "smc_kernels.h"
#include "smc_resident.h"
#include <type_traits>

namespace smc {

template <class F>
inline hipError_t by_model(int id, F&& f) {
    switch (id) {
    case MODEL_LG1D: return f(std::integral_constant<int, MODEL_LG1D>{});
    case MODEL_SV1D: return f(std::integral_constant<int, MODEL_SV1D>{});
    case MODEL_UCSV3D: return f(std::integral_constant<int, MODEL_UCSV3D>{});
    case MODEL_UCSV_RB: return f(std::integral_constant<int, MODEL_UCSV_RB>{});
    }
    return hipErrorInvalidValue;
}
template <class F>
inline hipError_t by_guided_model(int id, F&& f) {
    switch (id) {
    case MODEL_LG1D: return f(std::integral_constant<int, MODEL_LG1D>{});
    case MODEL_UCSV3D: return f(std::integral_constant<int, MODEL_UCSV3D>{});
    }
    return hipErrorInvalidValue;
}

template <class K>
inline hipError_t raise_lds_limit(K kernel, size_t lds, bool (&raised)[16]) {
    if (lds <= 64 * 1024) return hipSuccess;
    int dev = 0;
    hipError_t e = hipGetDevice(&dev);
    if (e != hipSuccess) return e;
    if (dev >= 0 && dev < 16 && raised[dev]) return hipSuccess;
    e = hipFuncSetAttribute((const void*)kernel, hipFuncAttributeMaxDynamicSharedMemorySize, 160 * 1024);
    if (e == hipSuccess && dev >= 0 && dev < 16) raised[dev] = true;
    return e;
}

struct Geo {
    int threads, np;
};
bool geo_default(int seg, Geo& g);
bool geo_valid(int seg, int np, Geo& g);

template <int MODEL> hipError_t launch_init(const FilterView& v, Geo g, int nxt, double y, hipStream_t s);
template <int MODEL> hipError_t launch_step(const FilterView& v, Geo g, int cur, uint32_t t, int emit_prev, double y, hipStream_t s);
template <int MODEL> hipError_t launch_resident(const FilterView& v, int T, StepRec* recs, hipStream_t s);
template <int MODEL> hipError_t launch_persist(const FilterView& v, Geo g, int cur, uint32_t t0, uint32_t t1, PersistCtl pc, hipStream_t s);
template <int MODEL> hipError_t launch_summ_once(const FilterView& v, int cur, hipStream_t s);
template <int MODEL> hipError_t launch_window(const FilterView& v, int T, StepRec* recs, int t0, int bin, int bout, double* win, hipStream_t s);
template <int MODEL> hipError_t launch_step_g(const FilterView& v, Geo g, int cur, uint32_t t, int emit_prev, double y, hipStream_t s);
template <int MODEL> hipError_t launch_resident_g(const FilterView& v, int T, StepRec* recs, hipStream_t s);
template <int MODEL> hipError_t launch_window_g(const FilterView& v, int T, StepRec* recs, int t0, int bin, int bout, double* win, hipStream_t s);

}
```

### sequential_monte_carlo_amd/csrc/smc_model.hip

```cpp
#include "smc_launch.h"
#include <cstdlib>

#ifndef SMC_MODEL
#error "compile with -DSMC_MODEL=<model id>"
#endif
#ifndef SMC_GUIDED
#define SMC_GUIDED 0
#endif
#define SMC_G (SMC_GUIDED != 0)

namespace smc {

#if !SMC_G
template <int THREADS, int NP>
static hipError_t init_t(const FilterView& v, int nxt, double y, hipStream_t s) {
    const size_t lds = scr_words(THREADS, NP) * 8;
    hipLaunchKernelGGL((k_init<SMC_MODEL, THREADS, NP>), dim3(v.nseg, v.ntheta), dim3(THREADS), lds, s, v, nxt, y);
    return hipGetLastError();
}
#endif
template <int THREADS, int NP, bool SYS>
static hipError_t step_sys_t(const FilterView& v, int cur, uint32_t t, int emit_prev, double y, hipStream_t s) {
    if (v.tabD) {
        const size_t lds = step_lds_bytes(0, THREADS, NP, true);
        static bool raised[16] = {};
        hipError_t e = raise_lds_limit(k_step<SMC_MODEL, THREADS, NP, true, SYS, true, 1, SMC_G>, lds, raised);
        if (e != hipSuccess) return e;
        hipLaunchKernelGGL((k_step<SMC_MODEL, THREADS, NP, true, SYS, true, 1, SMC_G>), dim3(v.nseg, v.ntheta), dim3(THREADS), lds, s, v, cur, t, 0, y);
        return hipGetLastError();
    }
    const size_t lds = step_lds_bytes(v.nseg_p2, THREADS, NP, v.nseg > 1);
    if (v.nseg_p2 > THREADS) {
        static bool raised[16] = {};
        hipError_t e = raise_lds_limit(k_step<SMC_MODEL, THREADS, NP, true, SYS, false, 2, SMC_G>, lds, raised);
        if (e != hipSuccess) return e;
        hipLaunchKernelGGL((k_step<SMC_MODEL, THREADS, NP, true, SYS, false, 2, SMC_G>), dim3(v.nseg, v.ntheta), dim3(THREADS), lds, s, v, cur, t, emit_prev, y);
        return hipGetLastError();
    }
    {
        static bool raised[2][16] = {};
        hipError_t e = v.nseg > 1 ? raise_lds_limit(k_step<SMC_MODEL, THREADS, NP, true, SYS, false, 1, SMC_G>, lds, raised[1])
                                  : raise_lds_limit(k_step<SMC_MODEL, THREADS, NP, false, SYS, false, 1, SMC_G>, lds, raised[0]);
        if (e != hipSuccess) return e;
    }
    if (v.nseg > 1)
        hipLaunchKernelGGL((k_step<SMC_MODEL, THREADS, NP, true, SYS, false, 1, SMC_G>), dim3(v.nseg, v.ntheta), dim3(THREADS), lds, s, v, cur, t,
                           emit_prev, y);
    else
        hipLaunchKernelGGL((k_step<SMC_MODEL, THREADS, NP, false, SYS, false, 1, SMC_G>), dim3(v.nseg, v.ntheta), dim3(THREADS), lds, s, v, cur, t,
                           emit_prev, y);
    return hipGetLastError();
}
template <int THREADS, int NP>
static hipError_t step_t(const FilterView& v, int cur, uint32_t t, int emit_prev, double y, hipStream_t s) {
    return v.systematic ? step_sys_t<THREADS, NP, true>(v, cur, t, emit_prev, y, s)
                        : step_sys_t<THREADS, NP, false>(v, cur, t, emit_prev, y, s);
}

#define SMC_GEO_SWITCH(FN, ...)                                                   \
    switch (g.threads * 8 + g.np) {                                               \
    case 64 * 8 + 2: return FN<64, 2>(__VA_ARGS__);                               \
    case 128 * 8 + 1: return FN<128, 1>(__VA_ARGS__);                             \
    case 128 * 8 + 2: return FN<128, 2>(__VA_ARGS__);                             \
    case 128 * 8 + 4: return FN<128, 4>(__VA_ARGS__);                             \
    case 256 * 8 + 1: return FN<256, 1>(__VA_ARGS__);                             \
    case 256 * 8 + 2: return FN<256, 2>(__VA_ARGS__);                             \
    case 256 * 8 + 4: return FN<256, 4>(__VA_ARGS__);                             \
    case 512 * 8 + 1: return FN<512, 1>(__VA_ARGS__);                             \
    case 512 * 8 + 2: return FN<512, 2>(__VA_ARGS__);                             \
    case 512 * 8 + 4: return FN<512, 4>(__VA_ARGS__);                             \
    case 1024 * 8 + 1: return FN<1024, 1>(__VA_ARGS__);                           \
    case 1024 * 8 + 2: return FN<1024, 2>(__VA_ARGS__);                           \
    case 1024 * 8 + 4: return FN<1024, 4>(__VA_ARGS__);                           \
    }                                                                             \
    return hipErrorInvalidValue;

#if !SMC_G
template <>
hipError_t launch_init<SMC_MODEL>(const FilterView& v, Geo g, int nxt, double y, hipStream_t s) {
    SMC_GEO_SWITCH(init_t, v, nxt, y, s)
}
#define SMC_LAUNCH_STEP launch_step
#define SMC_LAUNCH_RESIDENT launch_resident
#define SMC_LAUNCH_WINDOW launch_window
#else
#define SMC_LAUNCH_STEP launch_step_g
#define SMC_LAUNCH_RESIDENT launch_resident_g
#define SMC_LAUNCH_WINDOW launch_window_g
#endif
template <>
hipError_t SMC_LAUNCH_STEP<SMC_MODEL>(const FilterView& v, Geo g, int cur, uint32_t t, int emit_prev, double y, hipStream_t s) {
    SMC_GEO_SWITCH(step_t, v, cur, t, emit_prev, y, s)
}

template <int THREADS, int NP, bool SYS, bool WIN, bool SUMM = false, bool UNW = false>
static hipError_t resident_sys_t(const FilterView& v, int T, StepRec* recs, int t0, int bin, int bout, double* win, hipStream_t s) {
    const size_t lds = resident_lds_bytes<SMC_MODEL>(2 * NP * THREADS, THREADS, NP, SUMM ? v.sum_np : -1);
    if (lds > 160 * 1024) return hipErrorInvalidValue;
    static bool raised[16] = {};
    hipError_t e = raise_lds_limit(k_resident<SMC_MODEL, THREADS, NP, SYS, WIN, SUMM, UNW, SMC_G>, lds, raised);
    if (e != hipSuccess) return e;
    hipLaunchKernelGGL((k_resident<SMC_MODEL, THREADS, NP, SYS, WIN, SUMM, UNW, SMC_G>), dim3(v.ntheta), dim3(THREADS), lds, s, v, T, recs, t0, bin, bout, win);
    return hipGetLastError();
}
template <int THREADS, int NP>
static hipError_t resident_t(const FilterView& v, int T, StepRec* recs, hipStream_t s) {
    if ((v.sum_np || v.sum_mom) && v.sum_unw) return resident_sys_t<THREADS, NP, false, false, true, true>(v, T, recs, 0, 0, 0, nullptr, s);
    if (v.sum_np || v.sum_mom) return resident_sys_t<THREADS, NP, false, false, true>(v, T, recs, 0, 0, 0, nullptr, s);
    return v.systematic ? resident_sys_t<THREADS, NP, true, false>(v, T, recs, 0, 0, 0, nullptr, s)
                        : resident_sys_t<THREADS, NP, false, false>(v, T, recs, 0, 0, 0, nullptr, s);
}
template <int THREADS, int NP>
static hipError_t window_t(const FilterView& v, int T, StepRec* recs, int t0, int bin, int bout, double* win, hipStream_t s) {
    if ((v.sum_np || v.sum_mom) && v.sum_unw) return resident_sys_t<THREADS, NP, false, true, true, true>(v, T, recs, t0, bin, bout, win, s);
    if (v.sum_np || v.sum_mom) return resident_sys_t<THREADS, NP, false, true, true>(v, T, recs, t0, bin, bout, win, s);
    return v.systematic ? resident_sys_t<THREADS, NP, true, true>(v, T, recs, t0, bin, bout, win, s)
                        : resident_sys_t<THREADS, NP, false, true>(v, T, recs, t0, bin, bout, win, s);
}

static int resident_np(const FilterView& v) {
    const char* e = getenv("SMC_RES_NP");
    return e ? atoi(e) : (v.seg == 1024 && v.ntheta <= 512) ? 1 : 0;
}

template <>
hipError_t SMC_LAUNCH_RESIDENT<SMC_MODEL>(const FilterView& v, int T, StepRec* recs, hipStream_t s) {
    const int np = resident_np(v);
    switch (v.seg) {
    case 256: return resident_t<128, 1>(v, T, recs, s);
    case 512: return resident_t<256, 1>(v, T, recs, s);
    case 1024: return np == 1 ? resident_t<512, 1>(v, T, recs, s) : np == 4 ? resident_t<128, 4>(v, T, recs, s) : resident_t<256, 2>(v, T, recs, s);
    case 2048: return np == 1 ? resident_t<1024, 1>(v, T, recs, s) : np == 4 ? resident_t<256, 4>(v, T, recs, s) : resident_t<512, 2>(v, T, recs, s);
    case 4096:
        if constexpr (model_dim<SMC_MODEL>::value > 3) return hipErrorInvalidValue;
        else return np == 4 ? resident_t<512, 4>(v, T, recs, s) : resident_t<1024, 2>(v, T, recs, s);
    case 8192:
        if constexpr (model_dim<SMC_MODEL>::value == 1) return resident_t<1024, 4>(v, T, recs, s);
        else return hipErrorInvalidValue;
    }
    return hipErrorInvalidValue;
}

#if !SMC_G
template <int THREADS, int NP, bool UNW>
static hipError_t summ_once_m(const FilterView& v, int cur, hipStream_t s) {
    constexpr int D = model_dim<SMC_MODEL>::value;
    const size_t lds = summ_once_lds_bytes<D>(2 * NP * THREADS, v.sum_np);
    if (lds > 160 * 1024) return hipErrorInvalidValue;
    static bool raised[16] = {};
    hipError_t e = raise_lds_limit(k_summ_once<THREADS, NP, D, UNW>, lds, raised);
    if (e != hipSuccess) return e;
    hipLaunchKernelGGL((k_summ_once<THREADS, NP, D, UNW>), dim3(v.ntheta), dim3(THREADS), lds, s, v, cur);
    return hipGetLastError();
}
template <int THREADS, int NP>
static hipError_t summ_once_t(const FilterView& v, int cur, hipStream_t s) {
    return v.sum_unw ? summ_once_m<THREADS, NP, true>(v, cur, s) : summ_once_m<THREADS, NP, false>(v, cur, s);
}
template <>
hipError_t launch_summ_once<SMC_MODEL>(const FilterView& v, int cur, hipStream_t s) {
    if (v.nseg != 1) return hipErrorInvalidValue;
    switch (v.seg) {
    case 256: return summ_once_t<128, 1>(v, cur, s);
    case 512: return summ_once_t<256, 1>(v, cur, s);
    case 1024: return summ_once_t<512, 1>(v, cur, s);
    case 2048: return summ_once_t<512, 2>(v, cur, s);
    case 4096:
        if constexpr (model_dim<SMC_MODEL>::value > 3) return hipErrorInvalidValue;
        else return summ_once_t<512, 4>(v, cur, s);
    case 8192:
        if constexpr (model_dim<SMC_MODEL>::value > 3) return hipErrorInvalidValue;
        else return summ_once_t<1024, 4>(v, cur, s);
    }
    return hipErrorInvalidValue;
}
#endif

template <>
hipError_t SMC_LAUNCH_WINDOW<SMC_MODEL>(const FilterView& v, int T, StepRec* recs, int t0, int bin, int bout, double* win, hipStream_t s) {
    const int np = resident_np(v);
    switch (v.seg) {
    case 256: return window_t<128, 1>(v, T, recs, t0, bin, bout, win, s);
    case 512: return window_t<256, 1>(v, T, recs, t0, bin, bout, win, s);
    case 1024: return np == 1 ? window_t<512, 1>(v, T, recs, t0, bin, bout, win, s) : window_t<256, 2>(v, T, recs, t0, bin, bout, win, s);
    case 2048: return window_t<512, 2>(v, T, recs, t0, bin, bout, win, s);
    case 4096:
        if constexpr (model_dim<SMC_MODEL>::value > 3) return hipErrorInvalidValue;
        else return np == 4 ? window_t<512, 4>(v, T, recs, t0, bin, bout, win, s) : window_t<1024, 2>(v, T, recs, t0, bin, bout, win, s);
    case 8192:
        if constexpr (model_dim<SMC_MODEL>::value == 1) return window_t<1024, 4>(v, T, recs, t0, bin, bout, win, s);
        else return hipErrorInvalidValue;
    }
    return hipErrorInvalidValue;
}

}
```

Baseline: 83.30 billion particle-steps/s.

## Pass per-step hot scalars and params by value as kernel arguments

Adds a by-value step path for single-theta filters. The seed, stream id, parameters and current observation are handed to k_step as kernel arguments instead of being loaded from device memory at kernel entry. The aim is to shorten each step kernel's start-up latency, which matters when one launch runs per time step. In exchange it needs host-side cache invalidation whenever params, streams or slots change, and it adds another template variant of the kernel. It also adds debug timing of kernel start-up.

```diff
diff --git a/include/smc_hip.h b/include/smc_hip.h
--- a/include/smc_hip.h
+++ b/include/smc_hip.h
@@ -30,6 +30,7 @@
 int smc_set_params(smc_handle h, const double* raw );
 int smc_set_streams(smc_handle h, const uint32_t* stream );
 int smc_reseed(smc_handle h, uint64_t seed);
+int smc_step_by_value(smc_handle h, int* by_value);
 
 #define SMC_PROP_NONE 0
 #define SMC_PROP_AFFINE 1
diff --git a/sequential_monte_carlo_amd/_lib.py b/sequential_monte_carlo_amd/_lib.py
--- a/sequential_monte_carlo_amd/_lib.py
+++ b/sequential_monte_carlo_amd/_lib.py
@@ -10,7 +10,7 @@
 FLAG_ANCESTORS, FLAG_NO_RESIDENT, FLAG_SYSTEMATIC = 1, 2, 4
 
 EXPORTS = [
-    "smc_create", "smc_destroy", "smc_set_params", "smc_set_streams", "smc_reseed", "smc_init", "smc_step",
+    "smc_create", "smc_destroy", "smc_set_params", "smc_set_streams", "smc_reseed", "smc_step_by_value", "smc_init", "smc_step",
     "smc_log_likelihood", "smc_get_state", "smc_get_logZ", "smc_permute", "smc_copy_from", "smc_slot_bytes", "smc_pack_slots", "smc_unpack_slots", "smc_get_weights_raw", "smc_get_geometry",
     "smc_last_elapsed_ms", "smc_synchronize", "smc_time_step_kernel", "smc_event_overhead_ms", "smc_normalize", "smc_resample", "smc_kalman_log_likelihood", "smc_get_moments", "smc_get_quantiles", "smc_simulate", "smc_simulate_dim", "smc_model_dim",
     "smc_model_nraw", "smc_auto_seg", "smc_device_count", "smc_host_exp", "smc_host_log", "smc_host_philox4x32_10",
@@ -80,6 +80,7 @@
     L.smc_set_params.argtypes = [h, _dp]
     L.smc_set_streams.argtypes = [h, _u32p]
     L.smc_reseed.argtypes = [h, C.c_uint64]
+    L.smc_step_by_value.argtypes = [h, C.POINTER(C.c_int)]
     L.smc_init.argtypes = [h, C.c_double, _dp]
     L.smc_step.argtypes = [h, C.c_double, _dp, _dp]
     L.smc_log_likelihood.argtypes = [h, _dp, C.c_int64, _dp, _dp, _dp]
@@ -510,6 +511,12 @@
     def reseed(self, seed):
         check(lib().smc_reseed(self._h, seed))
 
+    @property
+    def step_by_value(self):
+        b = C.c_int()
+        check(lib().smc_step_by_value(self._h, C.byref(b)))
+        return bool(b.value)
+
     def init(self, y1):
         lm = np.zeros(self.n_theta)
         check(lib().smc_init(self._h, float(y1), _d(lm)))
diff --git a/sequential_monte_carlo_amd/csrc/smc_capi.hip b/sequential_monte_carlo_amd/csrc/smc_capi.hip
--- a/sequential_monte_carlo_amd/csrc/smc_capi.hip
+++ b/sequential_monte_carlo_amd/csrc/smc_capi.hip
@@ -81,15 +81,23 @@
     hipLaunchKernelGGL((k_table<TH>), dim3(h->v.ntheta), dim3(TH), 0, h->stream, h->v, h->cur, emit, first_emit, t_emit);
     return hipGetLastError();
 }
-hipError_t do_step(smc_filter_s* h, uint32_t t, int emit_prev, double y) {
+hipError_t do_step(smc_filter_s* h, uint32_t t, int emit_prev, double y, const double* y_host) {
     if (h->v.tabD) {
         hipError_t e = do_table(h, emit_prev, t == 1u ? 1 : 0, t - 1u);
         if (e != hipSuccess) return e;
         emit_prev = 0;
     }
+    StepHot hot{};
+    hot.seed = h->v.seed; hot.t = t; hot.nseg = h->v.nseg; hot.cur = h->cur; hot.emit_prev = emit_prev; hot.yval = y;
+    if (hot_legal(h) && !h->v.skip && (!h->v.y || y_host)) {
+        hot.by_value = 1;
+        hot.stream0 = h->hot.stream0;
+        hot.prm0 = h->hot.prm0;
+        if (h->v.y) hot.yval = y_host[t];
+    }
     if (h->v.prop_kind)
-        return by_guided_model(h->model, [&](auto M) { return launch_step_g<decltype(M)::value>(h->v, h->geo, h->cur, t, emit_prev, y, h->stream); });
-    return by_model(h->model, [&](auto M) { return launch_step<decltype(M)::value>(h->v, h->geo, h->cur, t, emit_prev, y, h->stream); });
+        return by_guided_model(h->model, [&](auto M) { return launch_step_g<decltype(M)::value>(h->v, h->geo, hot, h->stream); });
+    return by_model(h->model, [&](auto M) { return launch_step<decltype(M)::value>(h->v, h->geo, hot, h->stream); });
 }
 hipError_t ensure_breaks(smc_filter_s* h, uint32_t t, uint32_t t_end) {
     FilterView& v = h->v;
@@ -286,6 +294,9 @@
     TRY(hipMemcpyAsync(h->d_stream, st.data(), nt * 4, hipMemcpyHostToDevice, h->stream));
     TRY(hipStreamSynchronize(h->stream));
 #undef TRY
+    h->hot.stream0 = 0u;
+    h->hot.stream_ok = true;
+    if (const char* e = getenv("SMC_STEP_BY_VALUE")) h->hot.allow = atoi(e) != 0;
     v.params = h->d_params;
     v.stream = h->d_stream;
     *out = h;
@@ -358,6 +369,8 @@
         if (h->v.prop_kind) fill_proposal(h, m);
     }
     HIPCHK(hipMemcpyAsync(h->d_params, P, (size_t)h->v.ntheta * sizeof(Params), hipMemcpyHostToDevice, h->stream));
+    h->hot.prm0 = P[0];
+    h->hot.prm_ok = true;
     if (h->v.prop_kind)
         HIPCHK(hipMemcpyAsync(h->d_prop, h->h_prop, (size_t)h->v.ntheta * sizeof(PropRow), hipMemcpyHostToDevice, h->stream));
     h->have_params = true;
@@ -402,7 +415,15 @@
     HIPCHK(hipSetDevice(h->device));
     HIPCHK(hipMemcpyAsync(h->d_stream, s, (size_t)h->v.ntheta * 4, hipMemcpyHostToDevice, h->stream));
     HIPCHK(hipStreamSynchronize(h->stream));
+    h->hot.stream0 = s[0];
+    h->hot.stream_ok = true;
     h->brk_count = 0;
+    return SMC_OK;
+}
+
+extern "C" int smc_step_by_value(smc_handle h, int* by_value) {
+    if (!h || !by_value) return fail(SMC_EINVAL, "smc_step_by_value: NULL argument");
+    *by_value = hot_legal(h) && !h->skip.on ? 1 : 0;
     return SMC_OK;
 }
 
@@ -709,6 +730,21 @@
             if (st[w * 8] < t0) t0 = st[w * 8];
             if (st[w * 8 + 7] > t7) t7 = st[w * 8 + 7];
             for (int k = 1; k < 8; ++k) ph[k] += (double)(st[w * 8 + k] - st[w * 8 + k - 1]) * 0.01;
+        }
+        {
+            std::vector<unsigned long long> sd(nwg * 8);
+            (void)hipMemcpy(sd.data(), h->v.dbg + nwg * 8, nwg * 64, hipMemcpyDeviceToHost);
+            if (sd[7] != 0x5045525349535421ull && sd[0] != 0 && sd[1] != 0) {
+                double sum = 0, mn = 1e30, mx = 0;
+                std::vector<double> all(nwg);
+                for (size_t w = 0; w < nwg; ++w) {
+                    const double us = (double)(sd[w * 8] - sd[w * 8 + 1]) * 0.01;
+                    all[w] = us; sum += us; mn = std::min(mn, us); mx = std::max(mx, us);
+                }
+                std::sort(all.begin(), all.end());
+                fprintf(stderr, "[dbg] k_step start-up, entry -> first pick numbers drawn, over %zu workgroups (us, 10 ns clock): mean %.3f min %.3f "
+                                "median %.3f 90%% %.3f max %.3f\n", nwg, sum / nwg, mn, all[nwg / 2], all[(size_t)((nwg - 1) * 0.9)], mx);
+            }
         }
         double start_spread = 0, life = 0;
         for (size_t w = 0; w < nwg; ++w) { start_spread += (double)(st[w * 8] - t0) * 0.01; life += (double)(st[w * 8 + 7] - st[w * 8]) * 0.01; }
diff --git a/sequential_monte_carlo_amd/csrc/smc_capi_pmmh.hip b/sequential_monte_carlo_amd/csrc/smc_capi_pmmh.hip
--- a/sequential_monte_carlo_amd/csrc/smc_capi_pmmh.hip
+++ b/sequential_monte_carlo_amd/csrc/smc_capi_pmmh.hip
@@ -103,6 +103,7 @@
                            sqrt(scales[c]), h->d_params);
         HIPCHK(hipGetLastError());
         h->have_params = true;
+        hot_invalidate(h);
         h->v.seed = filter_seeds[c];
         h->brk_count = 0;
         h->v.skip = h->pm.dev.skip; h->v.order = h->pm.dev.order; h->v.n_active = h->pm.dev.counts;
@@ -111,7 +112,10 @@
         if (rc) return rc;
         hipLaunchKernelGGL(k_pmmh_accept, grid, block, 0, h->stream, h->v, h->pm.dev, d, move_seed, (uint32_t)c, xi);
         HIPCHK(hipGetLastError());
-        if (main) HIPCHK(copy_slots(main->v, main->cur, h->v, h->cur, main->d, h->pm.dev.mask, h->stream));
+        if (main) {
+            HIPCHK(copy_slots(main->v, main->cur, h->v, h->cur, main->d, h->pm.dev.mask, h->stream));
+            hot_invalidate(main);
+        }
     }
     hipLaunchKernelGGL(k_pmmh_export, grid, block, 0, h->stream, nt, d, h->pm.dev, h->pm.h_out);
     HIPCHK(hipGetLastError());
diff --git a/sequential_monte_carlo_amd/csrc/smc_capi_series.hip b/sequential_monte_carlo_amd/csrc/smc_capi_series.hip
--- a/sequential_monte_carlo_amd/csrc/smc_capi_series.hip
+++ b/sequential_monte_carlo_amd/csrc/smc_capi_series.hip
@@ -36,7 +36,7 @@
         return by_guided_model(h->model, [&](auto M) { return launch_resident_g<decltype(M)::value>(h->v, T, h->d_recs, h->stream); });
     return by_model(h->model, [&](auto M) { return launch_resident<decltype(M)::value>(h->v, T, h->d_recs, h->stream); });
 }
-int enqueue_log_likelihood(smc_handle h, double y0, int64_t T, bool want_trace, bool summ) {
+int enqueue_log_likelihood(smc_handle h, double y0, int64_t T, bool want_trace, bool summ, const double* y_host) {
     const bool resident = h->resident_ok && resident_supported(h->model, h->v.seg) && !(summ && (h->v.systematic || !summaries_fit_lds(h)));
     SeriesScope scope(h->v);
     h->v.y = h->d_y;
@@ -54,7 +54,7 @@
         if ((rc = enqueue_step_summaries(h, 0))) return rc;
         for (int64_t t = 1; t < T; ++t) {
             HIPCHK(ensure_breaks(h, (uint32_t)t, (uint32_t)T));
-            HIPCHK(do_step(h, (uint32_t)t, 0, 0.0));
+            HIPCHK(do_step(h, (uint32_t)t, 0, 0.0, y_host));
             h->cur ^= 1; h->t += 1; h->emitted = false;
             if ((rc = emit_if_needed(h))) return rc;
             if ((rc = enqueue_step_summaries(h, t))) return rc;
@@ -95,7 +95,7 @@
             const int emit = h->v.want_s2 ? 1 : 2;
             if (t == T - 1) h->v.want_s2 = 1;
             HIPCHK(ensure_breaks(h, (uint32_t)t, (uint32_t)T));
-            HIPCHK(do_step(h, (uint32_t)t, emit, 0.0));
+            HIPCHK(do_step(h, (uint32_t)t, emit, 0.0, y_host));
             h->cur ^= 1; h->t += 1;
         }
         h->v.want_s2 = 1;
@@ -125,7 +125,7 @@
     if (h->skip.on) { h->v.skip = h->skip.d_mask; h->v.order = h->skip.d_order; h->v.n_active = h->skip.d_order + h->v.ntheta; }
     const int cur0 = h->cur;
     HIPCHK(hipEventRecord(h->ev0, h->stream));
-    rc = enqueue_log_likelihood(h, y[0], T, want_trace, summ);
+    rc = enqueue_log_likelihood(h, y[0], T, want_trace, summ, y);
     h->v.skip = nullptr; h->v.order = nullptr; h->v.n_active = nullptr;
     if (rc) return rc;
     if (h->skip.on && h->cur != cur0) HIPCHK(copy_slots(h->v, h->cur, h->v, cur0, h->d, h->skip.d_mask, h->stream));
@@ -186,7 +186,7 @@
             HIPCHK(hipEventRecord(e0[k], h->stream));
             open_left = G;
         }
-        HIPCHK(do_step(h, (uint32_t)t, emit, 0.0));
+        HIPCHK(do_step(h, (uint32_t)t, emit, 0.0, y));
         if (open_left && --open_left == 0) { HIPCHK(hipEventRecord(e1[k], h->stream)); ++k; }
         h->cur ^= 1; h->t += 1;
     }
diff --git a/sequential_monte_carlo_amd/csrc/smc_capi_slots.hip b/sequential_monte_carlo_amd/csrc/smc_capi_slots.hip
--- a/sequential_monte_carlo_amd/csrc/smc_capi_slots.hip
+++ b/sequential_monte_carlo_amd/csrc/smc_capi_slots.hip
@@ -56,6 +56,7 @@
     hipLaunchKernelGGL(k_permute, dim3((unsigned)((v.npad + 255) / 256), v.ntheta), dim3(256), 0, h->stream, v, h->cur, h->d,
                        h->d_perm, h->d_logZ_tmp);
     HIPCHK(hipGetLastError());
+    hot_invalidate(h);
     h->cur ^= 1;
     HIPCHK(hipMemcpyAsync(h->d_logZ_tmp, v.logZ, (size_t)v.ntheta * 8, hipMemcpyDeviceToDevice, h->stream));
     HIPCHK(do_finalize(h, 0, h->t - 1));
@@ -80,6 +81,7 @@
     unsigned char* d_mask = reinterpret_cast<unsigned char*>(dst->d_perm);
     HIPCHK(hipMemcpyAsync(d_mask, mask, (size_t)a.ntheta, hipMemcpyHostToDevice, dst->stream));
     HIPCHK(copy_slots(a, dst->cur, b, src->cur, dst->d, d_mask, dst->stream));
+    hot_invalidate(dst);
     HIPCHK(hipStreamSynchronize(dst->stream));
     dst->t = src->t;
     return SMC_OK;
@@ -96,6 +98,7 @@
     if (!h->inited) return fail(SMC_ESTATE, "smc_pack/unpack_slots: filter not initialised");
     if (!pack) h->win.k = 0;
     if (k == 0) return SMC_OK;
+    if (!pack) hot_invalidate(h);
     for (int64_t i = 0; i < k; ++i)
         if (idx[i] < 0 || idx[i] >= h->v.ntheta) return fail(SMC_EINVAL, "smc_pack/unpack_slots: index out of range");
     HIPCHK(hipSetDevice(h->device));
diff --git a/sequential_monte_carlo_amd/csrc/smc_host.h b/sequential_monte_carlo_amd/csrc/smc_host.h
--- a/sequential_monte_carlo_amd/csrc/smc_host.h
+++ b/sequential_monte_carlo_amd/csrc/smc_host.h
@@ -72,6 +72,12 @@
     bool resident_ok = false;
     smc::Geo geo{0, 0};
     double last_ms = 0.0;
+    struct {
+        smc::Params prm0{};
+        uint32_t stream0 = 0;
+        bool prm_ok = false, stream_ok = false;
+        bool allow = true;
+    } hot;
 
     struct {
         unsigned char* d_mask = nullptr;
@@ -117,14 +123,16 @@
 }
 
 hipError_t do_init(smc_filter_s* h, double y);
-hipError_t do_step(smc_filter_s* h, uint32_t t, int emit_prev, double y);
+hipError_t do_step(smc_filter_s* h, uint32_t t, int emit_prev, double y, const double* y_host = nullptr);
+inline void hot_invalidate(smc_filter_s* h) { h->hot.prm_ok = h->hot.stream_ok = false; }
+inline bool hot_legal(const smc_filter_s* h) { return h->hot.allow && h->hot.prm_ok && h->hot.stream_ok && h->v.ntheta == 1; }
 hipError_t do_finalize(smc_filter_s* h, int first_emit, uint32_t t_emit);
 hipError_t ensure_breaks(smc_filter_s* h, uint32_t t, uint32_t t_end);
 int ensure_y(smc_handle h, int64_t T);
 int ensure_recs(smc_handle h, int64_t T);
 int emit_if_needed(smc_handle h);
 int finish_elapsed(smc_handle h, double* logZ = nullptr, double* logmu = nullptr, double* ess = nullptr);
-int enqueue_log_likelihood(smc_handle h, double y0, int64_t T, bool want_trace, bool summ = false);
+int enqueue_log_likelihood(smc_handle h, double y0, int64_t T, bool want_trace, bool summ = false, const double* y_host = nullptr);
 inline bool summaries_on(const smc_filter_s* h) { return h->summ.np > 0 || h->summ.mom != 0; }
 bool summaries_fit_lds(const smc_filter_s* h);
 int ensure_summaries(smc_handle h, int64_t T);
diff --git a/sequential_monte_carlo_amd/csrc/smc_kernels.h b/sequential_monte_carlo_amd/csrc/smc_kernels.h
--- a/sequential_monte_carlo_amd/csrc/smc_kernels.h
+++ b/sequential_monte_carlo_amd/csrc/smc_kernels.h
@@ -1,5 +1,6 @@
 #pragma once
 #include "smc_spec.h"
+#include <type_traits>
 
 namespace smc {
 
@@ -87,9 +88,21 @@
         if ((v).dbg && threadIdx.x == 0)                                                                  \
             (v).dbg[((size_t)blockIdx.y * gridDim.x + blockIdx.x) * 8 + (k)] = __builtin_amdgcn_s_memrealtime(); \
     } while (0)
+#define SMC_CLOCK() __builtin_amdgcn_s_memrealtime()
+#define SMC_STAMP_START(v, t_draw, t_entry)                                                               \
+    do {                                                                                                  \
+        if ((v).dbg && threadIdx.x == 0) {                                                                \
+            unsigned long long* d_ = (v).dbg + ((size_t)gridDim.y * gridDim.x + (size_t)blockIdx.y * gridDim.x + blockIdx.x) * 8; \
+            d_[0] = (t_draw); d_[1] = (t_entry);                                                          \
+        }                                                                                                 \
+    } while (0)
+#define SMC_ORDER_AFTER(x) asm volatile("" : : "v"(x))
 #else
+#define SMC_ORDER_AFTER(x) do { } while (0)
 #define SMC_ABL(v, bit) 0
 #define SMC_STAMP(v, k) do { } while (0)
+#define SMC_CLOCK() 0ull
+#define SMC_STAMP_START(v, t_draw, t_entry) do { (void)(t_draw); (void)(t_entry); } while (0)
 #endif
 template <class VIEW>
 __device__ __forceinline__ void host_emit(const VIEW& v, int th, double z, double logmu, double ess) {
@@ -730,8 +743,11 @@
     return base + (size_t)(multi ? nstage_for(2 * np * threads) : 1) * lds_padded_len(2 * np * threads) * 8;
 }
 
-template <int MODEL, int THREADS, int NP, bool MULTI, bool SYS, bool PERSIST, class VIEW, bool GTAB = false, int RPT = 1, bool GUIDED = false>
-__device__ __forceinline__ void step_body(const VIEW& v, int cur, uint32_t t, int emit_prev, double yval, char* smem) {
+template <int MODEL, int THREADS, int NP, bool MULTI, bool SYS, bool PERSIST, class VIEW, bool GTAB = false, int RPT = 1, bool GUIDED = false, bool BYV = false>
+__device__ __forceinline__ void step_body(const VIEW& v, uint64_t seed, uint32_t t, uint32_t stream0, int nseg, int cur, int emit_prev,
+                                          double yval, const Params* prm0, char* smem) {
+    static_assert(!(BYV && PERSIST), "by value: one launch per step");
+    const unsigned long long t_entry = SMC_CLOCK();
     static_assert(!GTAB || (MULTI && !PERSIST), "global table: multi-segment launches");
     static_assert(RPT == 1 || (RPT == 2 && MULTI && !GTAB && !PERSIST), "two records per thread: multi-segment launches");
     constexpr int D = model_dim<MODEL>::value, NZ = model_nz<MODEL>::value;
@@ -740,19 +756,26 @@
     constexpr int NQ = 2 * NP;
     constexpr int NSTAGE = nstage_for(SEG);
     constexpr int SEGP = lds_padded_len(SEG);
-    int sb_ = logical_segment(blockIdx.x, v.nseg), th_ = blockIdx.y, tid_ = smc_tid();
+    int sb_ = logical_segment(blockIdx.x, nseg), th_ = blockIdx.y, tid_ = smc_tid();
     if (PERSIST) {
         asm volatile("" : "+v"(tid_));
     }
     const int sb = sb_, th = th_, tid = tid_;
-    if (!PERSIST && v.skip && v.skip[th]) return;
+    if (!PERSIST && !BYV && v.skip && v.skip[th]) return;
     const int nxt = cur ^ 1;
-    const Params prm = v.params[th];
+    uint32_t stream;
+    if constexpr (BYV) stream = stream0;
+    else stream = v.stream[th];
+    const uint32_t seg0 = (uint32_t)sb * (uint32_t)SEG;
+    uint64_t rr[NQ];
+    u32x4 rw[NP] = {};
+    Params prm;
+    double y;
+    if constexpr (BYV) { prm = *prm0; y = yval; }
+    else { prm = v.params[th]; y = v.y ? v.y[t] : yval; }
     PropRow prw;
     if constexpr (GUIDED) prw = v.prop[th];
-    const uint32_t stream = v.stream[th];
-    const double y = v.y ? v.y[t] : yval;
-    const uint32_t seg0 = (uint32_t)sb * (uint32_t)SEG, n32 = (uint32_t)v.n;
+    const uint32_t n32 = (uint32_t)v.n;
     const uint64_t* Cprev = v.C[cur] + (size_t)th * v.npad;
     const double* xprev = v.x[cur];
     uint64_t* scr;
@@ -772,14 +795,19 @@
         F1 = Fb[1];
     }
     const TablePre tpre = (MULTI && !GTAB) ? table_preload<THREADS, VIEW, RPT>(v, cur, th, emit_prev && sb == 0) : TablePre{-inf(), 0, 0, 0, -inf(), 0};
-    uint64_t rr[NQ];
+    unsigned long long t_draw = 0;
 #pragma unroll
     for (int k = 0; k < NP; ++k) {
         if (SYS) { rr[2 * k] = rr[2 * k + 1] = 0; continue; }
         const uint32_t pg = (uint32_t)((seg0 >> 1) + tid + k * THREADS);
-        const u32x4 rw = SMC_ABL(v, 3) ? u32x4{{pg * 2654435761u, pg ^ t, pg * 40503u, ~pg}} : draw(v.seed, pg, stream, t, SLOT_RESAMPLE);
-        rr[2 * k] = ((uint64_t)rw.v[1] << 32) | rw.v[0];
-        rr[2 * k + 1] = ((uint64_t)rw.v[3] << 32) | rw.v[2];
+        rw[k] = draw(seed, pg, stream, t, SLOT_RESAMPLE);
+        if (k == 0) {
+            SMC_ORDER_AFTER(rw[0].v[3]);
+            t_draw = SMC_CLOCK();
+        }
+        if (SMC_ABL(v, 3)) rw[k] = u32x4{{pg * 2654435761u, pg ^ t, pg * 40503u, ~pg}};
+        rr[2 * k] = ((uint64_t)rw[k].v[1] << 32) | rw[k].v[0];
+        rr[2 * k + 1] = ((uint64_t)rw[k].v[3] << 32) | rw[k].v[2];
     }
     const uint32_t m_blk = (seg0 + SEG < n32 ? seg0 + SEG : n32) - seg0;
     const bool ragged = seg0 + SEG > n32;
@@ -826,8 +854,8 @@
 #pragma unroll
         for (int c = 0; c < NZ; ++c) {
             if (SMC_ABL(v, 2)) { z[k][c][0] = 1e-3 * (double)(pg & 1023); z[k][c][1] = -z[k][c][0]; }
-            else if (SMC_ABL(v, 6)) { const u32x4 w4 = draw(v.seed, pg, stream, t, SLOT_NORMAL0 + c); z[k][c][0] = 1e-9 * (double)w4.v[0]; z[k][c][1] = 1e-9 * (double)w4.v[2]; }
-            else box_muller(draw(v.seed, pg, stream, t, SLOT_NORMAL0 + c), z[k][c][0], z[k][c][1]);
+            else if (SMC_ABL(v, 6)) { const u32x4 w4 = draw(seed, pg, stream, t, SLOT_NORMAL0 + c); z[k][c][0] = 1e-9 * (double)w4.v[0]; z[k][c][1] = 1e-9 * (double)w4.v[2]; }
+            else box_muller(draw(seed, pg, stream, t, SLOT_NORMAL0 + c), z[k][c][0], z[k][c][1]);
             if (SYS || SMC_NORMALS_EARLY) asm volatile("" : "+v"(z[k][c][0]), "+v"(z[k][c][1]));
         }
     }
@@ -848,7 +876,7 @@
         scr = L.scr;
         uint64_t* sysw = L.scr + scr_words(THREADS, NP) - 8;
         if (SYS && tid == 0) {
-            const u32x4 uw = draw(v.seed, 0u, stream, t, SLOT_SYS);
+            const u32x4 uw = draw(seed, 0u, stream, t, SLOT_SYS);
             sysw[0] = ((uint64_t)uw.v[1] << 32) | uw.v[0];
         }
         const bool emitter = emit_prev && sb == 0;
@@ -981,7 +1009,7 @@
         if (SYS) {
             const int sh = seg_shift(0.0, 0.0, v.SH);
             const uint64_t Dtot = seg_Q(alive, sh);
-            const u32x4 uw = draw(v.seed, 0u, stream, t, SLOT_SYS);
+            const u32x4 uw = draw(seed, 0u, stream, t, SLOT_SYS);
             const SysBase sbase = sys_base(Dtot, n32, v.inv_n, ((uint64_t)uw.v[1] << 32) | uw.v[0], 0u);
 #pragma unroll
             for (int i = 0; i < NQ; ++i) Tg[i] = sys_threshold(sys_target(sbase, kk[i]), sh);
@@ -990,6 +1018,7 @@
     }
 
     SMC_STAMP(v, 2);
+    SMC_STAMP_START(v, t_draw, t_entry);
     SMC_STAMP(v, 3);
     uint64_t T2[NQ];
 #pragma unroll
@@ -1094,7 +1123,7 @@
         if (LATE_Z) {
             const uint32_t pg = (uint32_t)((seg0 >> 1) + tid + k * THREADS);
 #pragma unroll
-            for (int c = 0; c < NZ; ++c) box_muller(draw(v.seed, pg, stream, t, SLOT_NORMAL0 + c), z[k][c][0], z[k][c][1]);
+            for (int c = 0; c < NZ; ++c) box_muller(draw(seed, pg, stream, t, SLOT_NORMAL0 + c), z[k][c][0], z[k][c][1]);
         }
 #pragma unroll
         for (int j = 0; j < 2; ++j) {
@@ -1148,10 +1177,23 @@
     SMC_STAMP(v, 7);
 }
 
-template <int MODEL, int THREADS, int NP, bool MULTI, bool SYS = false, bool GTAB = false, int RPT = 1, bool GUIDED = false>
-__global__ __launch_bounds__(THREADS) void k_step(FilterView v, int cur, uint32_t t, int emit_prev, double yval) {
+struct StepHot {
+    uint64_t seed;
+    uint32_t t;
+    uint32_t stream0;
+    int nseg;
+    int cur, emit_prev;
+    int by_value;
+    double yval;
+    Params prm0;
+};
+static_assert(std::is_trivially_copyable<StepHot>::value, "passed by value");
+
+template <int MODEL, int THREADS, int NP, bool MULTI, bool SYS = false, bool GTAB = false, int RPT = 1, bool GUIDED = false, bool BYV = false>
+__global__ __launch_bounds__(THREADS) void k_step(uint64_t seed, uint32_t t, uint32_t stream0, int nseg, int cur, int emit_prev, double yval,
+                                                  Params prm0, FilterView v) {
     extern __shared__ __attribute__((aligned(16))) char smem[];
-    step_body<MODEL, THREADS, NP, MULTI, SYS, false, FilterView, GTAB, RPT, GUIDED>(v, cur, t, emit_prev, yval, smem);
+    step_body<MODEL, THREADS, NP, MULTI, SYS, false, FilterView, GTAB, RPT, GUIDED, BYV>(v, seed, t, stream0, nseg, cur, emit_prev, yval, &prm0, smem);
 }
 
 struct PersistCtl {
@@ -1193,7 +1235,7 @@
             }
         }
         if (v.dbg && tid == 0) { const unsigned long long now = __builtin_amdgcn_s_memrealtime(); acc[0] += now - acc[3]; acc[3] = now; }
-        step_body<MODEL, THREADS, NP, true, false, true>(v, cur, t, 2, 0.0, smem);
+        step_body<MODEL, THREADS, NP, true, false, true>(v, v.seed, t, 0u, v.nseg, cur, 2, 0.0, (const Params*)nullptr, smem);
         if (v.dbg && tid == 0) { const unsigned long long now = __builtin_amdgcn_s_memrealtime(); acc[1] += now - acc[3]; acc[3] = now; }
         asm volatile("s_waitcnt vmcnt(0)" ::: "memory");
         __syncthreads();
diff --git a/sequential_monte_carlo_amd/csrc/smc_launch.h b/sequential_monte_carlo_amd/csrc/smc_launch.h
--- a/sequential_monte_carlo_amd/csrc/smc_launch.h
+++ b/sequential_monte_carlo_amd/csrc/smc_launch.h
@@ -43,12 +43,12 @@
 bool geo_valid(int seg, int np, Geo& g);
 
 template <int MODEL> hipError_t launch_init(const FilterView& v, Geo g, int nxt, double y, hipStream_t s);
-template <int MODEL> hipError_t launch_step(const FilterView& v, Geo g, int cur, uint32_t t, int emit_prev, double y, hipStream_t s);
+template <int MODEL> hipError_t launch_step(const FilterView& v, Geo g, const StepHot& hot, hipStream_t s);
 template <int MODEL> hipError_t launch_resident(const FilterView& v, int T, StepRec* recs, hipStream_t s);
 template <int MODEL> hipError_t launch_persist(const FilterView& v, Geo g, int cur, uint32_t t0, uint32_t t1, PersistCtl pc, hipStream_t s);
 template <int MODEL> hipError_t launch_summ_once(const FilterView& v, int cur, hipStream_t s);
 template <int MODEL> hipError_t launch_window(const FilterView& v, int T, StepRec* recs, int t0, int bin, int bout, double* win, hipStream_t s);
-template <int MODEL> hipError_t launch_step_g(const FilterView& v, Geo g, int cur, uint32_t t, int emit_prev, double y, hipStream_t s);
+template <int MODEL> hipError_t launch_step_g(const FilterView& v, Geo g, const StepHot& hot, hipStream_t s);
 template <int MODEL> hipError_t launch_resident_g(const FilterView& v, int T, StepRec* recs, hipStream_t s);
 template <int MODEL> hipError_t launch_window_g(const FilterView& v, int T, StepRec* recs, int t0, int bin, int bout, double* win, hipStream_t s);
 
diff --git a/sequential_monte_carlo_amd/csrc/smc_model.hip b/sequential_monte_carlo_amd/csrc/smc_model.hip
--- a/sequential_monte_carlo_amd/csrc/smc_model.hip
+++ b/sequential_monte_carlo_amd/csrc/smc_model.hip
@@ -19,42 +19,29 @@
     return hipGetLastError();
 }
 #endif
-template <int THREADS, int NP, bool SYS>
-static hipError_t step_sys_t(const FilterView& v, int cur, uint32_t t, int emit_prev, double y, hipStream_t s) {
-    if (v.tabD) {
-        const size_t lds = step_lds_bytes(0, THREADS, NP, true);
-        static bool raised[16] = {};
-        hipError_t e = raise_lds_limit(k_step<SMC_MODEL, THREADS, NP, true, SYS, true, 1, SMC_G>, lds, raised);
-        if (e != hipSuccess) return e;
-        hipLaunchKernelGGL((k_step<SMC_MODEL, THREADS, NP, true, SYS, true, 1, SMC_G>), dim3(v.nseg, v.ntheta), dim3(THREADS), lds, s, v, cur, t, 0, y);
-        return hipGetLastError();
-    }
-    const size_t lds = step_lds_bytes(v.nseg_p2, THREADS, NP, v.nseg > 1);
-    if (v.nseg_p2 > THREADS) {
-        static bool raised[16] = {};
-        hipError_t e = raise_lds_limit(k_step<SMC_MODEL, THREADS, NP, true, SYS, false, 2, SMC_G>, lds, raised);
-        if (e != hipSuccess) return e;
-        hipLaunchKernelGGL((k_step<SMC_MODEL, THREADS, NP, true, SYS, false, 2, SMC_G>), dim3(v.nseg, v.ntheta), dim3(THREADS), lds, s, v, cur, t, emit_prev, y);
-        return hipGetLastError();
-    }
-    {
-        static bool raised[2][16] = {};
-        hipError_t e = v.nseg > 1 ? raise_lds_limit(k_step<SMC_MODEL, THREADS, NP, true, SYS, false, 1, SMC_G>, lds, raised[1])
-                                  : raise_lds_limit(k_step<SMC_MODEL, THREADS, NP, false, SYS, false, 1, SMC_G>, lds, raised[0]);
-        if (e != hipSuccess) return e;
-    }
-    if (v.nseg > 1)
-        hipLaunchKernelGGL((k_step<SMC_MODEL, THREADS, NP, true, SYS, false, 1, SMC_G>), dim3(v.nseg, v.ntheta), dim3(THREADS), lds, s, v, cur, t,
-                           emit_prev, y);
-    else
-        hipLaunchKernelGGL((k_step<SMC_MODEL, THREADS, NP, false, SYS, false, 1, SMC_G>), dim3(v.nseg, v.ntheta), dim3(THREADS), lds, s, v, cur, t,
-                           emit_prev, y);
+template <int THREADS, int NP, bool MULTI, bool SYS, bool GTAB, int RPT, bool BYV>
+static hipError_t step_launch(const FilterView& v, const StepHot& hot, int emit_prev, size_t lds, hipStream_t s) {
+    static bool raised[16] = {};
+    hipError_t e = raise_lds_limit(k_step<SMC_MODEL, THREADS, NP, MULTI, SYS, GTAB, RPT, SMC_G, BYV>, lds, raised);
+    if (e != hipSuccess) return e;
+    hipLaunchKernelGGL((k_step<SMC_MODEL, THREADS, NP, MULTI, SYS, GTAB, RPT, SMC_G, BYV>), dim3(v.nseg, v.ntheta), dim3(THREADS), lds, s, hot.seed, hot.t,
+                       hot.stream0, hot.nseg, hot.cur, emit_prev, hot.yval, hot.prm0, v);
     return hipGetLastError();
 }
+template <int THREADS, int NP, bool SYS, bool BYV>
+static hipError_t step_sys_t(const FilterView& v, const StepHot& hot, hipStream_t s) {
+    if (v.tabD)
+        return step_launch<THREADS, NP, true, SYS, true, 1, BYV>(v, hot, 0, step_lds_bytes(0, THREADS, NP, true), s);
+    const size_t lds = step_lds_bytes(v.nseg_p2, THREADS, NP, v.nseg > 1);
+    if (v.nseg_p2 > THREADS)
+        return step_launch<THREADS, NP, true, SYS, false, 2, BYV>(v, hot, hot.emit_prev, lds, s);
+    return v.nseg > 1 ? step_launch<THREADS, NP, true, SYS, false, 1, BYV>(v, hot, hot.emit_prev, lds, s)
+                      : step_launch<THREADS, NP, false, SYS, false, 1, BYV>(v, hot, hot.emit_prev, lds, s);
+}
 template <int THREADS, int NP>
-static hipError_t step_t(const FilterView& v, int cur, uint32_t t, int emit_prev, double y, hipStream_t s) {
-    return v.systematic ? step_sys_t<THREADS, NP, true>(v, cur, t, emit_prev, y, s)
-                        : step_sys_t<THREADS, NP, false>(v, cur, t, emit_prev, y, s);
+static hipError_t step_t(const FilterView& v, const StepHot& hot, hipStream_t s) {
+    if (hot.by_value) return v.systematic ? step_sys_t<THREADS, NP, true, true>(v, hot, s) : step_sys_t<THREADS, NP, false, true>(v, hot, s);
+    return v.systematic ? step_sys_t<THREADS, NP, true, false>(v, hot, s) : step_sys_t<THREADS, NP, false, false>(v, hot, s);
 }
 
 #define SMC_GEO_SWITCH(FN, ...)                                                   \
@@ -89,8 +76,9 @@
 #define SMC_LAUNCH_WINDOW launch_window_g
 #endif
 template <>
-hipError_t SMC_LAUNCH_STEP<SMC_MODEL>(const FilterView& v, Geo g, int cur, uint32_t t, int emit_prev, double y, hipStream_t s) {
-    SMC_GEO_SWITCH(step_t, v, cur, t, emit_prev, y, s)
+hipError_t SMC_LAUNCH_STEP<SMC_MODEL>(const FilterView& v, Geo g, const StepHot& hot, hipStream_t s) {
+    if (hot.by_value && v.ntheta != 1) return hipErrorInvalidValue;
+    SMC_GEO_SWITCH(step_t, v, hot, s)
 }
 
 template <int THREADS, int NP, bool SYS, bool WIN, bool SUMM = false, bool UNW = false>
```

Measured after the change: 89.68 billion particle-steps/s (median of 6 runs). 7.7% higher.
